# iamgiddyaboutgit/globalign

Hardware: AMD Instinct MI355X
Metric: DP cells/s (matrix fill) + alignment score bit-exact vs ref (higher is better)
Workload: dtype int32; 1 GPU; C3: 100k x 100k DNA (SplitMix64 seeds 1,2), match 2 / mismatch -3 / open -5 / ext -1, full traceback; m=100000, n=100000, traceback=True, parallelism=single GPU, cost=245432, oracle_cost=245432, cost_matches_oracle=True

## Files before the change

globalign_amd/csrc/ga_host.cpp:

```cpp
#include <hip/hip_runtime.h>
#include <unistd.h>

#include <algorithm>
#include <condition_variable>
#include <map>
#include <mutex>
#include <thread>
#include <chrono>
#include <cstdint>
#include <cstdio>
#include <cstring>
#include <string>
#include <vector>

#include "../../include/globalign_amd.h"
#include "ga_device.h"
#include "ga_lane.h"
#include "ga_check.h"
#include "ga_rng.h"

namespace {

thread_local std::string g_err;

// ... 333 lines not shown
#ifdef GA_EXPERIMENTS
constexpr bool kRcJumpDefault = false;
#endif
inline size_t rc_cache_bytes(bool jump, int TD, int CB) {
    return jump ? (size_t)ga::RC_CACHE_I * ga::RC_CACHE_S * 4 * TD * 6144 + 65536
                : (size_t)ga::RC_CACHE_I * ga::RC_CACHE_S * TD * 64 * 64 * CB + (size_t)64 * 64 * 4 * 4;
}
inline bool rc_jump_requested(const ga_ctx* c) {
#ifdef GA_EXPERIMENTS
    const char* e = c->xknob("GA_RC_JUMP");
    return e ? atoi(e) != 0 : kRcJumpDefault;
#else
    (void)c;
    return false;
#endif
}

int enqueue_fill(ga_ctx* c, int32_t flags, const Band& bd = Band()) {
    int every = bd.rc_every > 0 ? bd.rc_every : 64;
    if (!c->loaded) return fail(GA_E_STATE, "no problem loaded");
    const bool tb = (flags & (GA_FILL_TRACEBACK | GA_FILL_FULL)) != 0;
    const bool full = (flags & GA_FILL_FULL) != 0;
    const int64_t m = bd.band ? bd.mb : c->m, n = bd.band && bd.nc > 0 ? bd.nc : c->n;
    c->TC = (int)((m + ga::FROWS - 1) / ga::FROWS) * c->CB;
    int qrows = c->qrows;
    c->diag = false;
    c->lane = false;
    if (bd.rc) {
        if (tb || full || !lane_geometry(c, n, &qrows, false)) return fail(GA_E_STATE, "recompute fill needs the lane kernel");
        if (c->nwc == 8 && c->T == 8 && !lane_geometry(c, n, &qrows, false, 8, 4)) return fail(GA_E_STATE, "recompute fill geometry");
        constexpr int kRcLds = 256 * 256 * 2;
        if (!c->lane_T_req) {
            const char* nw = c->knob("GA_RC_NARROW");
            const bool td2 = nw && atoi(nw) && !c->slab && c->K <= 8 && (n + 127) / 128 <= 4 * (int64_t)c->num_cu;
            if (td2 && lane_geometry(c, n, &qrows, false, 2, 4)) {
            } else if (c->T > 4) {
                if (!lane_geometry(c, n, &qrows, false, 4, 4)) return fail(GA_E_STATE, "recompute fill geometry");
            } else if (c->T < 4) {
                (void)lane_geometry(c, n, &qrows, false, 4, 4);
            }
        }
        int64_t budget = (int64_t)96 << 30;
        if (const char* e = c->knob("GA_RC_BUDGET_MB")) budget = atoll(e) << 20;
        const int64_t dev_avail = dev_avail_bytes(c, (int64_t)c->stck.cap + (int64_t)c->colck.cap + (int64_t)c->rc_tb.cap);
        auto ck_bytes = [&](int e) {
            const int64_t nck = std::max<int64_t>((m - 1) / e, 1);
            return nck * c->nstripes * (c->T + 1) * 512;
        };
        auto other_bytes = [&]() {
            return (int64_t)c->nstripes * (m + 1) * 8 +
                   (int64_t)rc_cache_bytes(rc_jump_requested(c) && c->T <= 4, c->T, c->CB) +
                   ((int64_t)64 << 20);
        };
        auto fits = [&](int e) {
            return ck_bytes(e) <= std::min(budget, dev_avail - other_bytes()) &&
                   1024 + ga::rc_worker_bytes(c->T, c->CB, e) <= kRcLds;
        };
        for (;;) {
            if (bd.rc_every > 0) every = bd.rc_every;
            else
                for (every = 64; every < 4096 && !fits(every); every *= 2) {}
            if (1024 + ga::rc_worker_bytes(c->T, c->CB, every) <= kRcLds) break;
            if (c->T == 1) {
                if (1024 + ga::rc_worker_bytes(1, c->CB, 64) <= kRcLds)
                    return fail(GA_E_NOMEM, "recompute walk: the checkpoints do not fit the budget / free device memory");
                return fail(GA_E_RANGE, "recompute walk: a block's codes do not fit LDS");
            }
// ... 1998 lines not shown
```

globalign_amd/csrc/ga_lane.hip:

```cpp
#include <hip/hip_runtime.h>
#include <stdint.h>

#include <algorithm>
#include <cstdlib>
#include <type_traits>

#include "ga_device.h"
#include "ga_lane.h"
#include "ga_lane_asm.h"
#include "ga_sync.h"

#ifndef GA_LANE_LE
#define GA_LANE_LE 13
#endif

namespace ga {

__device__ unsigned lane_slab(const FillArgs& p) {
    unsigned* F = p.ticket;
    if (!p.xcd_map) return atomicAdd(F, 1u);
    const unsigned x = (unsigned)__builtin_amdgcn_s_getreg((15 << 11) | 20) & 7u;
    const unsigned rk = __hip_atomic_fetch_add(F + 4 + x, 1u, __ATOMIC_RELAXED, AGENT);
    const unsigned arr = __hip_atomic_fetch_add(F, 1u, __ATOMIC_ACQ_REL, AGENT);
    unsigned mode = 0;
// ... 349 lines not shown
    auto dbg_rows = [&](int r0) {
        if (r0 == 64) t_rows[4] = __builtin_amdgcn_s_memrealtime();
        if (r0 == 128) t_rows[5] = __builtin_amdgcn_s_memrealtime();
        if (r0 == 256) t_rows[0] = __builtin_amdgcn_s_memrealtime();
        if (r0 == 1024) t_rows[1] = __builtin_amdgcn_s_memrealtime();
        if (r0 == 4096) t_rows[2] = __builtin_amdgcn_s_memrealtime();
        if (r0 == 16384) t_rows[3] = __builtin_amdgcn_s_memrealtime();
    };
    auto wait_ge = [&](unsigned* ctr, unsigned add, unsigned& cached, int target, int kind) {
        unsigned spins = 0;
        cached = sgpr_u(cached);
        unsigned long long t0 = 0;
        if (DBG && (int)cached < target) t0 = __builtin_amdgcn_s_memtime();
        while ((int)cached < target && !aborted) {
            cached = lds_ldu(ctr) + add;
            if ((int)cached >= target) break;
            if (!spin_ok_lds(spins, p.spin_limit, abort_sh)) aborted = true;
        }
        if (DBG && t0) wcyc[kind] += __builtin_amdgcn_s_memtime() - t0;
        __atomic_signal_fence(__ATOMIC_SEQ_CST);
    };
    constexpr int NE = SUB / 2;
    constexpr int NQ = SUB / 4;
    int4 A[NE], B[NE];
    uint32_t qA[TD][NQ], qB[TD][NQ];
    wait_ge(prod_in, 0, avail, SUB, 0);
    unsigned long long w_first = 0, t_first = 0;
    if (DBG) {
        w_first = wcyc[0];
        t_first = __builtin_amdgcn_s_memrealtime();
    }
    const int4* const ezero = reinterpret_cast<const int4*>(smem + LK_ZERO_OFF);
    const unsigned ca_lds = lds_addr(prod_in);
    const unsigned pq_lds = lds_addr(pq);
    const unsigned scr_lds = lds_addr(smem + LK_SCR_OFF);
    unsigned q4[TD], ea_m, ea_b, wa_m, wa_b, wb_m, wb_b;
    {
#pragma unroll
        for (int k = 0; k < TD; k++) q4[k] = pq_lds + 4u * qb[k];
        const unsigned scr = scr_lds + 8u * (unsigned)lane, rout_l = lds_addr(rin + RING);
        const bool hi = lane >= 48;
        ea_m = lane == 0 ? ~0u : 0u;
        ea_b = lane == 0 ? 0u : lds_addr(ezero);
        wa_m = hi && (lane & 4) ? 8u * RMASK : 0u;
        wa_b = hi && (lane & 4) ? rout_l : scr;
        wb_m = hi && !(lane & 4) ? 8u * RMASK : 0u;
        wb_b = hi && !(lane & 4) ? rout_l : scr;
    }
    {
        const int4* src = lane == 0 ? reinterpret_cast<const int4*>(rin) : ezero;
#pragma unroll
        for (int k = 0; k < NE; k++) A[k] = src[k];
    }
    wait_ge(&cnt[LK_PRODQ], 0, qavail, SUB, 1);
    {
        const unsigned idx = (unsigned)(-lane) & qmask;
#pragma unroll
        for (int k = 0; k < TD; k++)
#pragma unroll
            for (int d = 0; d < NQ; d++) qA[k][d] = pq[qb[k] + idx + 4 * d];
    }
    unsigned pnext = *prod_in;
    int next_ck = CKP ? p.ckpt_rows : 0x7fffffff;
    constexpr int LE = (CB == 0 && !CKP && SUB == 16 && LATE) ? GA_LANE_LE : 0;

    auto sub_chunk = [&](int r0, int4 (&C)[NE], int4 (&Nx)[NE], uint32_t (&qc)[TD][NQ], uint32_t (&qx)[TD][NQ],
                         auto HALF, auto LEANT) {
        constexpr int HB = decltype(HALF)::value * SUB;
        constexpr bool LEAN = decltype(LEANT)::value;
        if (!LE) {
            avail = sgpr_u(max(avail, pnext));
            if ((int)avail < r0 + 2 * SUB) wait_ge(prod_in, 0, avail, r0 + 2 * SUB, 0);
        }
        if ((int)qavail < r0 + 2 * SUB) wait_ge(&cnt[LK_PRODQ], 0, qavail, r0 + 2 * SUB, 1);
        int eh[SUB], ex[SUB];
#pragma unroll
        for (int k = 0; k < NE; k++) {
            eh[2 * k] = C[k].x; ex[2 * k] = C[k].y; eh[2 * k + 1] = C[k].z; ex[2 * k + 1] = C[k].w;
        }
        auto qloads = [&]() {
            asm volatile("" ::: "memory");
            const unsigned idx = (unsigned)(r0 + SUB - lane) & qmask;
#pragma unroll
            for (int k = 0; k < TD; k++)
#pragma unroll
                for (int d = 0; d < NQ; d++) qx[k][d] = pq[qb[k] + idx + 4 * d];
            asm volatile("" ::: "memory");
        };
        auto eloads = [&]() {
            asm volatile("" ::: "memory");
            if (LE) {
                avail = sgpr_u(max(avail, pnext));
                if ((int)avail < r0 + 2 * SUB) wait_ge(prod_in, 0, avail, r0 + 2 * SUB, 0);
            }
            {
                const int4* src = lane == 0 ? reinterpret_cast<const int4*>(rin + ((r0 + SUB) & RMASK)) : ezero;
#pragma unroll
                for (int k = 0; k < NE; k++) Nx[k] = src[k];
            }
            pnext = __hip_atomic_load(prod_in, RLX, WGS);
            asm volatile("" ::: "memory");
        };
        const int row0 = r0 - lane + 1;
        const bool capl = lane == cn / TD;
        int cku = -1;
        int2* ckr = nullptr;
        auto ck_find = [&]() {
// ... 20 lines not shown
                            if (jl + k + 1 <= p.n) ckr[jl + k + 1] = make_int2(H[k], Y[k]);
                    }
                }
            };
            one(std::integral_constant<int, 0>{});
            qloads();
            if constexpr (LE > 0) {
                LkUnroll<1, LE>::run(one);
                eloads();
                LkUnroll<LE, SUB>::run(one);
            } else {
                eloads();
                LkUnroll<1, SUB>::run(one);
            }
        };
        const bool ckw = CKP && next_ck <= r0 + SUB;
        if (ckw) ck_find();
        if (CKP && next_ck < r0 + SUB - 62) next_ck += p.ckpt_rows;
        if constexpr (CKP) {
            if (r0 < 64 || (unsigned)(tm - r0) < (unsigned)SUB) {
                if (ckw) steps(std::true_type{}, std::true_type{});
                else steps(std::true_type{}, std::false_type{});
            } else if (ckw) {
                steps(std::false_type{}, std::true_type{});
            } else {
                steps(std::false_type{}, std::false_type{});
            }
        } else {
            const bool masked = !LEAN && ((r0 < 64 && !(p.lean0 && use_asm)) || (unsigned)(tm - r0) < (unsigned)SUB);
            if constexpr (ASMOK) {
                if (LEAN || (use_asm && !masked && !hand_direct)) {
                    const int rlo = r0 - 62;
                    outfree = sgpr_u(outfree);
                    if ((int)outfree < rlo + SUB - 1) wait_ge(cons_out, RING, outfree, rlo + SUB - 1, 2);
                    lk_v4i Ev[NE];
#pragma unroll
                    for (int k = 0; k < NE; k++) Ev[k] = lk_v4i{C[k].x, C[k].y, C[k].z, C[k].w};
                    unsigned ea, qi4, wt, wa, wb, qbv[TD];
                    const unsigned ea_s = lds_addr(rin) + 8u * ((unsigned)(r0 + SUB) & RMASK);
                    asm volatile("v_and_or_b32 %0, %1, %2, %3" : "=v"(ea) : "s"(ea_s), "v"(ea_m), "v"(ea_b));
                    asm volatile("v_sub_u32 %0, %1, %2" : "=v"(qi4) : "s"(4u * (unsigned)(r0 + SUB)), "v"(4u * (unsigned)lane));
                    qi4 &= 4u * qmask;
#pragma unroll
                    for (int k = 0; k < TD; k++) asm volatile("v_add_u32 %0, %1, %2" : "=v"(qbv[k]) : "v"(q4[k]), "v"(qi4));
                    asm volatile("v_add_u32 %0, %1, %2" : "=v"(wt) : "s"(8u * (unsigned)(rlo - 49)), "v"(8u * (unsigned)lane));
                    wa = (wt & wa_m) + wa_b;
                    wb = (wt & wb_m) + wb_b;
                    const unsigned wc = lane == 0 ? pc_lds : scr_lds + 8u * (unsigned)lane;
                    const bool hi = lane >= 48;
                    const lk_v2u cp = {(unsigned)(r0 + 2 * SUB), (unsigned)max(rlo + SUB - 1, 0)};
                    unsigned cv;
                    lk_v4i En[NE];
                    lk_v2u qn[TD][2];
                    int R[4];
                    LaneSub<TD, LE ? 12 : 0>::run(H, Y, Xl, HLp, Ev, qc, o, ca_lds, ea, qbv, wa, wb, wc, cp, cv, En, qn, R);
                    Hl = H[TD - 1];
                    if (DBG && rlo <= m / 2 && m / 2 < rlo + SUB) t_pub = __builtin_amdgcn_s_memrealtime();
                    const int need = min(r0 + 2 * SUB, m);
                    if ((int)sgpr_u(cv) < need) {
                        wait_ge(prod_in, 0, avail, need, 0);
                        asm volatile("" ::: "memory");
                        const int4* src = lane == 0 ? reinterpret_cast<const int4*>(rin + ((r0 + SUB) & RMASK)) : ezero;
#pragma unroll
                        for (int k = 0; k < NE; k++) Nx[k] = src[k];
#pragma unroll
                        for (int k = 0; k < NE; k++) asm volatile("" ::"v"(Nx[k].x), "v"(Nx[k].y), "v"(Nx[k].z), "v"(Nx[k].w));
                    } else {
#pragma unroll
                        for (int k = 0; k < NE; k++) Nx[k] = make_int4(En[k].x, En[k].y, En[k].z, En[k].w);
                    }
                    if (DBG && r0 + SUB < m / 2 && m / 2 <= r0 + 2 * SUB) t_avail = __builtin_amdgcn_s_memrealtime();
#pragma unroll
                    for (int k = 0; k < TD; k++) {
                        qx[k][0] = qn[k][0].x;
                        qx[k][1] = qn[k][0].y;
                        qx[k][2] = qn[k][1].x;
                        qx[k][3] = qn[k][1].y;
                    }
                    if (RC && LEAN) {
                        const lk_v2u vv = (lane & 4) ? lk_v2u{(unsigned)R[0], (unsigned)R[1]} : lk_v2u{(unsigned)R[2], (unsigned)R[3]};
                        const unsigned off = ck_cb + sgpr_u(8u * (unsigned)rlo);
                        asm volatile("buffer_store_dwordx2 %1, %0, %2, 0 offen" ::"v"(off), "v"(vv), "s"(ck_rsrc) : "memory");
                    } else if (RC && p.colck != nullptr) {
                        const int row = rlo + lane - 48;
                        const int2 v = (lane & 4) ? make_int2(R[0], R[1]) : make_int2(R[2], R[3]);
                        int2* const cdst = hi && row <= m ? colck_s + row : colck_x;
                        const lk_v2u vv = {(unsigned)v.x, (unsigned)v.y};
                        asm volatile("global_store_dwordx2 %0, %1, off" ::"v"(cdst), "v"(vv) : "memory");
                    }
                    return;
                }
            }
// ... 240 lines not shown
```

globalign_amd/csrc/ga_lane_asm.h:

```cpp
#pragma once
#include <hip/hip_runtime.h>
#include <stdint.h>

#include "ga_lane.h"

namespace ga {

template <int TD, int U0, int N>
struct LaneAsm;
typedef int lk_v4i __attribute__((ext_vector_type(4)));
template <int TD, int RS>
struct LaneSub;

template <>
struct LaneAsm<1, 0, 1> {
    __device__ __forceinline__ static void run(int (&H)[1], int (&Y)[1], int& Xl, int& HLp, const int* eh,
                                               const int* ex, const uint32_t (&q)[1], int o, int* oh, int* ox) {
        int X[1], HLn[1], hn[1], T, M[1];
        asm volatile(
        "v_add_u32_sdwa %[M0], sext(%[q0]), %[HLp] dst_sel:DWORD dst_unused:UNUSED_PAD src0_sel:BYTE_0 src1_sel:DWORD\n\t"
        "s_nop 0\n\t"
        "v_add_u32_dpp %[X0], %[Xl], %[ex0] wave_shr:1 row_mask:0xf bank_mask:0xf bound_ctrl:1\n\t"
        "v_add_u32_dpp %[HLn0], %[Hlast], %[eh0] wave_shr:1 row_mask:0xf bank_mask:0xf bound_ctrl:1\n\t"
        "v_min3_i32 %[hn0], %[M0], %[X0], %[Y0]\n\t"
// ... 2393 lines not shown
        "v_min_i32 %[Y4], %[Y4], %[T]\n\t"
        "v_min3_i32 %[H5], %[M5], %[X0], %[Y5]\n\t"
        "v_add_u32 %[T], %[o], %[H5]\n\t"
        "v_min_i32 %[X0], %[X0], %[T]\n\t"
        "v_min_i32 %[Y5], %[Y5], %[T]\n\t"
        "v_min3_i32 %[H6], %[M6], %[X0], %[Y6]\n\t"
        "v_add_u32 %[T], %[o], %[H6]\n\t"
        "v_min_i32 %[X0], %[X0], %[T]\n\t"
        "v_min_i32 %[Y6], %[Y6], %[T]\n\t"
        "v_min3_i32 %[hn0], %[M7], %[X0], %[Y7]\n\t"
        "v_add_u32 %[T], %[o], %[hn0]\n\t"
        "v_min_i32 %[X0], %[X0], %[T]\n\t"
        "v_min_i32 %[Y7], %[Y7], %[T]"
        : [X0] "=&v"(X[0]), [HLn0] "=&v"(HLn[0]), [hn0] "=&v"(hn[0]), [H0] "+v"(H[0]), [H1] "+v"(H[1]), [H2] "+v"(H[2]), [H3] "+v"(H[3]), [H4] "+v"(H[4]), [H5] "+v"(H[5]), [H6] "+v"(H[6]), [Y0] "+v"(Y[0]), [Y1] "+v"(Y[1]), [Y2] "+v"(Y[2]), [Y3] "+v"(Y[3]), [Y4] "+v"(Y[4]), [Y5] "+v"(Y[5]), [Y6] "+v"(Y[6]), [Y7] "+v"(Y[7]), [T] "=&v"(T), [M0] "=&v"(M[0]), [M1] "=&v"(M[1]), [M2] "=&v"(M[2]), [M3] "=&v"(M[3]), [M4] "=&v"(M[4]), [M5] "=&v"(M[5]), [M6] "=&v"(M[6]), [M7] "=&v"(M[7])
        : [Xl] "v"(Xl), [HLp] "v"(HLp), [Hlast] "v"(H[7]), [ex0] "v"(ex[0]), [eh0] "v"(eh[0]), [q0] "v"(q[0]), [q1] "v"(q[1]), [q2] "v"(q[2]), [q3] "v"(q[3]), [q4] "v"(q[4]), [q5] "v"(q[5]), [q6] "v"(q[6]), [q7] "v"(q[7]), [o] "s"(o));
        H[7] = hn[0];
        Xl = X[0];
        HLp = HLn[0];
#pragma unroll
        for (int s = 0; s < 1; s++) {
            oh[s] = hn[s];
            ox[s] = X[s];
        }
    }
};

template <>
struct LaneSub<1, 0> {
    __device__ __forceinline__ static void run(int (&H)[1], int (&Y)[1], int& Xl, int& HLp, const lk_v4i (&E)[8],
                                               const uint32_t (&q)[1][4], int o, unsigned ca, unsigned ea,
                                               const unsigned (&qb)[1], unsigned wa, unsigned wb, unsigned wc, lk_v2u cp,
                                               unsigned& cv, lk_v4i (&En)[8], lk_v2u (&qn)[1][2], int (&R)[4]) {
        int X[16], hn[16], HLn[2], T, M[1];
        asm volatile(
        "v_add_u32_sdwa %[M0], sext(%[q0_0]), %[HLp] dst_sel:DWORD dst_unused:UNUSED_PAD src0_sel:BYTE_0 src1_sel:DWORD\n\t"
        "s_nop 1\n\t"
        "v_add_u32_dpp %[X0], %[Xl], %[ex0] wave_shr:1 row_mask:0xf bank_mask:0xf bound_ctrl:1\n\t"
        "v_add_u32_dpp %[HLn0], %[Hlast], %[eh0] wave_shr:1 row_mask:0xf bank_mask:0xf bound_ctrl:1\n\t"
        "v_min3_i32 %[hn0], %[M0], %[X0], %[Y0]\n\t"
        "v_add_u32 %[T], %[o], %[hn0]\n\t"
        "v_min_i32 %[X0], %[X0], %[T]\n\t"
        "v_min_i32 %[Y0], %[Y0], %[T]\n\t"
        "ds_read_b32 %[cv], %[ca]\n\t"
        "ds_read_b128 %[E0], %[ea] offset:0\n\t"
        "ds_read_b128 %[E1], %[ea] offset:16\n\t"
        "ds_read_b128 %[E2], %[ea] offset:32\n\t"
        "ds_read_b128 %[E3], %[ea] offset:48\n\t"
        "ds_read_b128 %[E4], %[ea] offset:64\n\t"
        "ds_read_b128 %[E5], %[ea] offset:80\n\t"
        "ds_read_b128 %[E6], %[ea] offset:96\n\t"
        "ds_read_b128 %[E7], %[ea] offset:112\n\t"
        "v_add_u32_sdwa %[M0], sext(%[q0_0]), %[HLn0] dst_sel:DWORD dst_unused:UNUSED_PAD src0_sel:BYTE_1 src1_sel:DWORD\n\t"
        "v_add_u32_dpp %[X1], %[X0], %[ex1] wave_shr:1 row_mask:0xf bank_mask:0xf bound_ctrl:1\n\t"
        "v_add_u32_dpp %[HLn1], %[hn0], %[eh1] wave_shr:1 row_mask:0xf bank_mask:0xf bound_ctrl:1\n\t"
        "v_min3_i32 %[hn1], %[M0], %[X1], %[Y0]\n\t"
        "v_add_u32 %[T], %[o], %[hn1]\n\t"
        "v_min_i32 %[X1], %[X1], %[T]\n\t"
        "v_min_i32 %[Y0], %[Y0], %[T]\n\t"
        "ds_read2_b32 %[qa0], %[qb0] offset0:0 offset1:4\n\t"
        "ds_read2_b32 %[qc0], %[qb0] offset0:8 offset1:12\n\t"
        "v_add_u32_sdwa %[M0], sext(%[q0_0]), %[HLn1] dst_sel:DWORD dst_unused:UNUSED_PAD src0_sel:BYTE_2 src1_sel:DWORD\n\t"
        "v_add_u32_dpp %[X2], %[X1], %[ex2] wave_shr:1 row_mask:0xf bank_mask:0xf bound_ctrl:1\n\t"
        "v_add_u32_dpp %[HLn0], %[hn1], %[eh2] wave_shr:1 row_mask:0xf bank_mask:0xf bound_ctrl:1\n\t"
        "v_min3_i32 %[hn2], %[M0], %[X2], %[Y0]\n\t"
        "v_add_u32 %[T], %[o], %[hn2]\n\t"
        "v_min_i32 %[X2], %[X2], %[T]\n\t"
// ... 75 lines not shown
        "v_add_u32_dpp %[HLn1], %[hn10], %[eh11] wave_shr:1 row_mask:0xf bank_mask:0xf bound_ctrl:1\n\t"
        "v_min3_i32 %[hn11], %[M0], %[X11], %[Y0]\n\t"
        "v_add_u32 %[T], %[o], %[hn11]\n\t"
        "v_min_i32 %[X11], %[X11], %[T]\n\t"
        "v_min_i32 %[Y0], %[Y0], %[T]\n\t"
        "v_add_u32_sdwa %[M0], sext(%[q0_3]), %[HLn1] dst_sel:DWORD dst_unused:UNUSED_PAD src0_sel:BYTE_0 src1_sel:DWORD\n\t"
        "v_add_u32_dpp %[X12], %[X11], %[ex12] wave_shr:1 row_mask:0xf bank_mask:0xf bound_ctrl:1\n\t"
        "v_add_u32_dpp %[HLn0], %[hn11], %[eh12] wave_shr:1 row_mask:0xf bank_mask:0xf bound_ctrl:1\n\t"
        "v_min3_i32 %[hn12], %[M0], %[X12], %[Y0]\n\t"
        "v_add_u32 %[T], %[o], %[hn12]\n\t"
        "v_min_i32 %[X12], %[X12], %[T]\n\t"
        "v_min_i32 %[Y0], %[Y0], %[T]\n\t"
        "v_add_u32_sdwa %[M0], sext(%[q0_3]), %[HLn0] dst_sel:DWORD dst_unused:UNUSED_PAD src0_sel:BYTE_1 src1_sel:DWORD\n\t"
        "v_add_u32_dpp %[X13], %[X12], %[ex13] wave_shr:1 row_mask:0xf bank_mask:0xf bound_ctrl:1\n\t"
        "v_add_u32_dpp %[HLn1], %[hn12], %[eh13] wave_shr:1 row_mask:0xf bank_mask:0xf bound_ctrl:1\n\t"
        "v_min3_i32 %[hn13], %[M0], %[X13], %[Y0]\n\t"
        "v_add_u32 %[T], %[o], %[hn13]\n\t"
        "v_min_i32 %[X13], %[X13], %[T]\n\t"
        "v_min_i32 %[Y0], %[Y0], %[T]\n\t"
        "v_add_u32_sdwa %[M0], sext(%[q0_3]), %[HLn1] dst_sel:DWORD dst_unused:UNUSED_PAD src0_sel:BYTE_2 src1_sel:DWORD\n\t"
        "v_add_u32_dpp %[X14], %[X13], %[ex14] wave_shr:1 row_mask:0xf bank_mask:0xf bound_ctrl:1\n\t"
        "v_add_u32_dpp %[HLn0], %[hn13], %[eh14] wave_shr:1 row_mask:0xf bank_mask:0xf bound_ctrl:1\n\t"
        "v_min3_i32 %[hn14], %[M0], %[X14], %[Y0]\n\t"
        "v_add_u32 %[T], %[o], %[hn14]\n\t"
        "v_min_i32 %[X14], %[X14], %[T]\n\t"
        "v_min_i32 %[Y0], %[Y0], %[T]\n\t"
        "v_add_u32_sdwa %[M0], sext(%[q0_3]), %[HLn0] dst_sel:DWORD dst_unused:UNUSED_PAD src0_sel:BYTE_3 src1_sel:DWORD\n\t"
        "v_add_u32_dpp %[X15], %[X14], %[ex15] wave_shr:1 row_mask:0xf bank_mask:0xf bound_ctrl:1\n\t"
        "v_add_u32_dpp %[HLn1], %[hn14], %[eh15] wave_shr:1 row_mask:0xf bank_mask:0xf bound_ctrl:1\n\t"
        "v_min3_i32 %[hn15], %[M0], %[X15], %[Y0]\n\t"
        "v_add_u32 %[T], %[o], %[hn15]\n\t"
        "v_min_i32 %[X15], %[X15], %[T]\n\t"
        "v_min_i32 %[Y0], %[Y0], %[T]\n\t"
        "v_mov_b32_dpp %[Rhb], %[hn11] row_shl:4 row_mask:0x8 bank_mask:0x4\n\t"
        "v_mov_b32_dpp %[Rha], %[hn15] quad_perm:[0,1,2,3] row_mask:0x8 bank_mask:0x8\n\t"
        "v_mov_b32_dpp %[Rxb], %[X11] row_shl:4 row_mask:0x8 bank_mask:0x4\n\t"
        "v_mov_b32_dpp %[Rxa], %[X15] quad_perm:[0,1,2,3] row_mask:0x8 bank_mask:0x8\n\t"
        "v_mov_b32_dpp %[Rhb], %[hn10] row_shl:5 row_mask:0x8 bank_mask:0x4\n\t"
        "v_mov_b32_dpp %[Rha], %[hn14] row_shl:1 row_mask:0x8 bank_mask:0x8\n\t"
        "v_mov_b32_dpp %[Rxb], %[X10] row_shl:5 row_mask:0x8 bank_mask:0x4\n\t"
        "v_mov_b32_dpp %[Rxa], %[X14] row_shl:1 row_mask:0x8 bank_mask:0x8\n\t"
        "v_mov_b32_dpp %[Rhb], %[hn9] row_shl:6 row_mask:0x8 bank_mask:0x4\n\t"
        "v_mov_b32_dpp %[Rha], %[hn13] row_shl:2 row_mask:0x8 bank_mask:0x8\n\t"
        "v_mov_b32_dpp %[Rxb], %[X9] row_shl:6 row_mask:0x8 bank_mask:0x4\n\t"
        "v_mov_b32_dpp %[Rxa], %[X13] row_shl:2 row_mask:0x8 bank_mask:0x8\n\t"
        "v_mov_b32_dpp %[Rhb], %[hn8] row_shl:7 row_mask:0x8 bank_mask:0x4\n\t"
        "v_mov_b32_dpp %[Rha], %[hn12] row_shl:3 row_mask:0x8 bank_mask:0x8\n\t"
        "v_mov_b32_dpp %[Rxb], %[X8] row_shl:7 row_mask:0x8 bank_mask:0x4\n\t"
        "v_mov_b32_dpp %[Rxa], %[X12] row_shl:3 row_mask:0x8 bank_mask:0x8\n\t"
        "ds_write2_b32 %[wa], %[Rha], %[Rxa] offset1:1\n\t"
        "ds_write2_b32 %[wb], %[Rhb], %[Rxb] offset1:1\n\t"
        "ds_write_b64 %[wc], %[cp]\n\t"
        "s_waitcnt lgkmcnt(3)"
        : [X0] "=&v"(X[0]), [X1] "=&v"(X[1]), [X2] "=&v"(X[2]), [X3] "=&v"(X[3]), [X4] "=&v"(X[4]), [X5] "=&v"(X[5]), [X6] "=&v"(X[6]), [X7] "=&v"(X[7]), [X8] "=&v"(X[8]), [X9] "=&v"(X[9]), [X10] "=&v"(X[10]), [X11] "=&v"(X[11]), [X12] "=&v"(X[12]), [X13] "=&v"(X[13]), [X14] "=&v"(X[14]), [X15] "=&v"(X[15]), [hn0] "=&v"(hn[0]), [hn1] "=&v"(hn[1]), [hn2] "=&v"(hn[2]), [hn3] "=&v"(hn[3]), [hn4] "=&v"(hn[4]), [hn5] "=&v"(hn[5]), [hn6] "=&v"(hn[6]), [hn7] "=&v"(hn[7]), [hn8] "=&v"(hn[8]), [hn9] "=&v"(hn[9]), [hn10] "=&v"(hn[10]), [hn11] "=&v"(hn[11]), [hn12] "=&v"(hn[12]), [hn13] "=&v"(hn[13]), [hn14] "=&v"(hn[14]), [hn15] "=&v"(hn[15]), [HLn0] "=&v"(HLn[0]), [HLn1] "=&v"(HLn[1]), [Y0] "+v"(Y[0]), [T] "=&v"(T), [M0] "=&v"(M[0]), [Rha] "=&v"(R[0]), [Rxa] "=&v"(R[1]), [Rhb] "=&v"(R[2]), [Rxb] "=&v"(R[3]), [cv] "=&v"(cv), [E0] "=&v"(En[0]), [E1] "=&v"(En[1]), [E2] "=&v"(En[2]), [E3] "=&v"(En[3]), [E4] "=&v"(En[4]), [E5] "=&v"(En[5]), [E6] "=&v"(En[6]), [E7] "=&v"(En[7]), [qa0] "=&v"(qn[0][0]), [qc0] "=&v"(qn[0][1])
        : [Xl] "v"(Xl), [HLp] "v"(HLp), [Hlast] "v"(H[0]), [o] "s"(o), [ex0] "v"(E[0][1]), [ex1] "v"(E[0][3]), [ex2] "v"(E[1][1]), [ex3] "v"(E[1][3]), [ex4] "v"(E[2][1]), [ex5] "v"(E[2][3]), [ex6] "v"(E[3][1]), [ex7] "v"(E[3][3]), [ex8] "v"(E[4][1]), [ex9] "v"(E[4][3]), [ex10] "v"(E[5][1]), [ex11] "v"(E[5][3]), [ex12] "v"(E[6][1]), [ex13] "v"(E[6][3]), [ex14] "v"(E[7][1]), [ex15] "v"(E[7][3]), [eh0] "v"(E[0][0]), [eh1] "v"(E[0][2]), [eh2] "v"(E[1][0]), [eh3] "v"(E[1][2]), [eh4] "v"(E[2][0]), [eh5] "v"(E[2][2]), [eh6] "v"(E[3][0]), [eh7] "v"(E[3][2]), [eh8] "v"(E[4][0]), [eh9] "v"(E[4][2]), [eh10] "v"(E[5][0]), [eh11] "v"(E[5][2]), [eh12] "v"(E[6][0]), [eh13] "v"(E[6][2]), [eh14] "v"(E[7][0]), [eh15] "v"(E[7][2]), [q0_0] "v"(q[0][0]), [q0_1] "v"(q[0][1]), [q0_2] "v"(q[0][2]), [q0_3] "v"(q[0][3]), [ca] "v"(ca), [ea] "v"(ea), [wa] "v"(wa), [wb] "v"(wb), [wc] "v"(wc), [cp] "v"(cp), [qb0] "v"(qb[0])
        : "memory");
        H[0] = hn[15];
        Xl = X[15];
        HLp = HLn[1];
    }
};

template <>
struct LaneSub<1, 12> {
    __device__ __forceinline__ static void run(int (&H)[1], int (&Y)[1], int& Xl, int& HLp, const lk_v4i (&E)[8],
                                               const uint32_t (&q)[1][4], int o, unsigned ca, unsigned ea,
                                               const unsigned (&qb)[1], unsigned wa, unsigned wb, unsigned wc, lk_v2u cp,
                                               unsigned& cv, lk_v4i (&En)[8], lk_v2u (&qn)[1][2], int (&R)[4]) {
        int X[16], hn[16], HLn[2], T, M[1];
        asm volatile(
        "v_add_u32_sdwa %[M0], sext(%[q0_0]), %[HLp] dst_sel:DWORD dst_unused:UNUSED_PAD src0_sel:BYTE_0 src1_sel:DWORD\n\t"
        "s_nop 1\n\t"
        "v_add_u32_dpp %[X0], %[Xl], %[ex0] wave_shr:1 row_mask:0xf bank_mask:0xf bound_ctrl:1\n\t"
        "v_add_u32_dpp %[HLn0], %[Hlast], %[eh0] wave_shr:1 row_mask:0xf bank_mask:0xf bound_ctrl:1\n\t"
        "v_min3_i32 %[hn0], %[M0], %[X0], %[Y0]\n\t"
        "v_add_u32 %[T], %[o], %[hn0]\n\t"
        "v_min_i32 %[X0], %[X0], %[T]\n\t"
        "v_min_i32 %[Y0], %[Y0], %[T]\n\t"
        "v_add_u32_sdwa %[M0], sext(%[q0_0]), %[HLn0] dst_sel:DWORD dst_unused:UNUSED_PAD src0_sel:BYTE_1 src1_sel:DWORD\n\t"
        "v_add_u32_dpp %[X1], %[X0], %[ex1] wave_shr:1 row_mask:0xf bank_mask:0xf bound_ctrl:1\n\t"
        "v_add_u32_dpp %[HLn1], %[hn0], %[eh1] wave_shr:1 row_mask:0xf bank_mask:0xf bound_ctrl:1\n\t"
        "v_min3_i32 %[hn1], %[M0], %[X1], %[Y0]\n\t"
        "v_add_u32 %[T], %[o], %[hn1]\n\t"
        "v_min_i32 %[X1], %[X1], %[T]\n\t"
        "v_min_i32 %[Y0], %[Y0], %[T]\n\t"
        "ds_read2_b32 %[qa0], %[qb0] offset0:0 offset1:4\n\t"
        "ds_read2_b32 %[qc0], %[qb0] offset0:8 offset1:12\n\t"
        "v_add_u32_sdwa %[M0], sext(%[q0_0]), %[HLn1] dst_sel:DWORD dst_unused:UNUSED_PAD src0_sel:BYTE_2 src1_sel:DWORD\n\t"
        "v_add_u32_dpp %[X2], %[X1], %[ex2] wave_shr:1 row_mask:0xf bank_mask:0xf bound_ctrl:1\n\t"
        "v_add_u32_dpp %[HLn0], %[hn1], %[eh2] wave_shr:1 row_mask:0xf bank_mask:0xf bound_ctrl:1\n\t"
        "v_min3_i32 %[hn2], %[M0], %[X2], %[Y0]\n\t"
        "v_add_u32 %[T], %[o], %[hn2]\n\t"
        "v_min_i32 %[X2], %[X2], %[T]\n\t"
        "v_min_i32 %[Y0], %[Y0], %[T]\n\t"
        "v_add_u32_sdwa %[M0], sext(%[q0_0]), %[HLn0] dst_sel:DWORD dst_unused:UNUSED_PAD src0_sel:BYTE_3 src1_sel:DWORD\n\t"
        "v_add_u32_dpp %[X3], %[X2], %[ex3] wave_shr:1 row_mask:0xf bank_mask:0xf bound_ctrl:1\n\t"
        "v_add_u32_dpp %[HLn1], %[hn2], %[eh3] wave_shr:1 row_mask:0xf bank_mask:0xf bound_ctrl:1\n\t"
        "v_min3_i32 %[hn3], %[M0], %[X3], %[Y0]\n\t"
        "v_add_u32 %[T], %[o], %[hn3]\n\t"
        "v_min_i32 %[X3], %[X3], %[T]\n\t"
        "v_min_i32 %[Y0], %[Y0], %[T]\n\t"
        "v_add_u32_sdwa %[M0], sext(%[q0_1]), %[HLn1] dst_sel:DWORD dst_unused:UNUSED_PAD src0_sel:BYTE_0 src1_sel:DWORD\n\t"
// ... 75 lines not shown
        "v_add_u32 %[T], %[o], %[hn12]\n\t"
        "v_min_i32 %[X12], %[X12], %[T]\n\t"
        "v_min_i32 %[Y0], %[Y0], %[T]\n\t"
        "ds_read_b32 %[cv], %[ca]\n\t"
        "ds_read_b128 %[E0], %[ea] offset:0\n\t"
        "ds_read_b128 %[E1], %[ea] offset:16\n\t"
        "ds_read_b128 %[E2], %[ea] offset:32\n\t"
        "ds_read_b128 %[E3], %[ea] offset:48\n\t"
        "ds_read_b128 %[E4], %[ea] offset:64\n\t"
        "ds_read_b128 %[E5], %[ea] offset:80\n\t"
        "ds_read_b128 %[E6], %[ea] offset:96\n\t"
        "ds_read_b128 %[E7], %[ea] offset:112\n\t"
        "v_add_u32_sdwa %[M0], sext(%[q0_3]), %[HLn0] dst_sel:DWORD dst_unused:UNUSED_PAD src0_sel:BYTE_1 src1_sel:DWORD\n\t"
        "v_add_u32_dpp %[X13], %[X12], %[ex13] wave_shr:1 row_mask:0xf bank_mask:0xf bound_ctrl:1\n\t"
        "v_add_u32_dpp %[HLn1], %[hn12], %[eh13] wave_shr:1 row_mask:0xf bank_mask:0xf bound_ctrl:1\n\t"
        "v_min3_i32 %[hn13], %[M0], %[X13], %[Y0]\n\t"
        "v_add_u32 %[T], %[o], %[hn13]\n\t"
        "v_min_i32 %[X13], %[X13], %[T]\n\t"
        "v_min_i32 %[Y0], %[Y0], %[T]\n\t"
        "v_add_u32_sdwa %[M0], sext(%[q0_3]), %[HLn1] dst_sel:DWORD dst_unused:UNUSED_PAD src0_sel:BYTE_2 src1_sel:DWORD\n\t"
        "v_add_u32_dpp %[X14], %[X13], %[ex14] wave_shr:1 row_mask:0xf bank_mask:0xf bound_ctrl:1\n\t"
        "v_add_u32_dpp %[HLn0], %[hn13], %[eh14] wave_shr:1 row_mask:0xf bank_mask:0xf bound_ctrl:1\n\t"
        "v_min3_i32 %[hn14], %[M0], %[X14], %[Y0]\n\t"
        "v_add_u32 %[T], %[o], %[hn14]\n\t"
        "v_min_i32 %[X14], %[X14], %[T]\n\t"
        "v_min_i32 %[Y0], %[Y0], %[T]\n\t"
        "v_add_u32_sdwa %[M0], sext(%[q0_3]), %[HLn0] dst_sel:DWORD dst_unused:UNUSED_PAD src0_sel:BYTE_3 src1_sel:DWORD\n\t"
        "v_add_u32_dpp %[X15], %[X14], %[ex15] wave_shr:1 row_mask:0xf bank_mask:0xf bound_ctrl:1\n\t"
        "v_add_u32_dpp %[HLn1], %[hn14], %[eh15] wave_shr:1 row_mask:0xf bank_mask:0xf bound_ctrl:1\n\t"
        "v_min3_i32 %[hn15], %[M0], %[X15], %[Y0]\n\t"
        "v_add_u32 %[T], %[o], %[hn15]\n\t"
        "v_min_i32 %[X15], %[X15], %[T]\n\t"
        "v_min_i32 %[Y0], %[Y0], %[T]\n\t"
        "v_mov_b32_dpp %[Rhb], %[hn11] row_shl:4 row_mask:0x8 bank_mask:0x4\n\t"
        "v_mov_b32_dpp %[Rha], %[hn15] quad_perm:[0,1,2,3] row_mask:0x8 bank_mask:0x8\n\t"
        "v_mov_b32_dpp %[Rxb], %[X11] row_shl:4 row_mask:0x8 bank_mask:0x4\n\t"
        "v_mov_b32_dpp %[Rxa], %[X15] quad_perm:[0,1,2,3] row_mask:0x8 bank_mask:0x8\n\t"
        "v_mov_b32_dpp %[Rhb], %[hn10] row_shl:5 row_mask:0x8 bank_mask:0x4\n\t"
        "v_mov_b32_dpp %[Rha], %[hn14] row_shl:1 row_mask:0x8 bank_mask:0x8\n\t"
        "v_mov_b32_dpp %[Rxb], %[X10] row_shl:5 row_mask:0x8 bank_mask:0x4\n\t"
        "v_mov_b32_dpp %[Rxa], %[X14] row_shl:1 row_mask:0x8 bank_mask:0x8\n\t"
        "v_mov_b32_dpp %[Rhb], %[hn9] row_shl:6 row_mask:0x8 bank_mask:0x4\n\t"
        "v_mov_b32_dpp %[Rha], %[hn13] row_shl:2 row_mask:0x8 bank_mask:0x8\n\t"
        "v_mov_b32_dpp %[Rxb], %[X9] row_shl:6 row_mask:0x8 bank_mask:0x4\n\t"
        "v_mov_b32_dpp %[Rxa], %[X13] row_shl:2 row_mask:0x8 bank_mask:0x8\n\t"
        "v_mov_b32_dpp %[Rhb], %[hn8] row_shl:7 row_mask:0x8 bank_mask:0x4\n\t"
        "v_mov_b32_dpp %[Rha], %[hn12] row_shl:3 row_mask:0x8 bank_mask:0x8\n\t"
        "v_mov_b32_dpp %[Rxb], %[X8] row_shl:7 row_mask:0x8 bank_mask:0x4\n\t"
        "v_mov_b32_dpp %[Rxa], %[X12] row_shl:3 row_mask:0x8 bank_mask:0x8\n\t"
        "ds_write2_b32 %[wa], %[Rha], %[Rxa] offset1:1\n\t"
        "ds_write2_b32 %[wb], %[Rhb], %[Rxb] offset1:1\n\t"
        "ds_write_b64 %[wc], %[cp]\n\t"
        "s_waitcnt lgkmcnt(3)"
        : [X0] "=&v"(X[0]), [X1] "=&v"(X[1]), [X2] "=&v"(X[2]), [X3] "=&v"(X[3]), [X4] "=&v"(X[4]), [X5] "=&v"(X[5]), [X6] "=&v"(X[6]), [X7] "=&v"(X[7]), [X8] "=&v"(X[8]), [X9] "=&v"(X[9]), [X10] "=&v"(X[10]), [X11] "=&v"(X[11]), [X12] "=&v"(X[12]), [X13] "=&v"(X[13]), [X14] "=&v"(X[14]), [X15] "=&v"(X[15]), [hn0] "=&v"(hn[0]), [hn1] "=&v"(hn[1]), [hn2] "=&v"(hn[2]), [hn3] "=&v"(hn[3]), [hn4] "=&v"(hn[4]), [hn5] "=&v"(hn[5]), [hn6] "=&v"(hn[6]), [hn7] "=&v"(hn[7]), [hn8] "=&v"(hn[8]), [hn9] "=&v"(hn[9]), [hn10] "=&v"(hn[10]), [hn11] "=&v"(hn[11]), [hn12] "=&v"(hn[12]), [hn13] "=&v"(hn[13]), [hn14] "=&v"(hn[14]), [hn15] "=&v"(hn[15]), [HLn0] "=&v"(HLn[0]), [HLn1] "=&v"(HLn[1]), [Y0] "+v"(Y[0]), [T] "=&v"(T), [M0] "=&v"(M[0]), [Rha] "=&v"(R[0]), [Rxa] "=&v"(R[1]), [Rhb] "=&v"(R[2]), [Rxb] "=&v"(R[3]), [cv] "=&v"(cv), [E0] "=&v"(En[0]), [E1] "=&v"(En[1]), [E2] "=&v"(En[2]), [E3] "=&v"(En[3]), [E4] "=&v"(En[4]), [E5] "=&v"(En[5]), [E6] "=&v"(En[6]), [E7] "=&v"(En[7]), [qa0] "=&v"(qn[0][0]), [qc0] "=&v"(qn[0][1])
        : [Xl] "v"(Xl), [HLp] "v"(HLp), [Hlast] "v"(H[0]), [o] "s"(o), [ex0] "v"(E[0][1]), [ex1] "v"(E[0][3]), [ex2] "v"(E[1][1]), [ex3] "v"(E[1][3]), [ex4] "v"(E[2][1]), [ex5] "v"(E[2][3]), [ex6] "v"(E[3][1]), [ex7] "v"(E[3][3]), [ex8] "v"(E[4][1]), [ex9] "v"(E[4][3]), [ex10] "v"(E[5][1]), [ex11] "v"(E[5][3]), [ex12] "v"(E[6][1]), [ex13] "v"(E[6][3]), [ex14] "v"(E[7][1]), [ex15] "v"(E[7][3]), [eh0] "v"(E[0][0]), [eh1] "v"(E[0][2]), [eh2] "v"(E[1][0]), [eh3] "v"(E[1][2]), [eh4] "v"(E[2][0]), [eh5] "v"(E[2][2]), [eh6] "v"(E[3][0]), [eh7] "v"(E[3][2]), [eh8] "v"(E[4][0]), [eh9] "v"(E[4][2]), [eh10] "v"(E[5][0]), [eh11] "v"(E[5][2]), [eh12] "v"(E[6][0]), [eh13] "v"(E[6][2]), [eh14] "v"(E[7][0]), [eh15] "v"(E[7][2]), [q0_0] "v"(q[0][0]), [q0_1] "v"(q[0][1]), [q0_2] "v"(q[0][2]), [q0_3] "v"(q[0][3]), [ca] "v"(ca), [ea] "v"(ea), [wa] "v"(wa), [wb] "v"(wb), [wc] "v"(wc), [cp] "v"(cp), [qb0] "v"(qb[0])
        : "memory");
        H[0] = hn[15];
        Xl = X[15];
        HLp = HLn[1];
    }
};

template <>
struct LaneSub<2, 0> {
    __device__ __forceinline__ static void run(int (&H)[2], int (&Y)[2], int& Xl, int& HLp, const lk_v4i (&E)[8],
                                               const uint32_t (&q)[2][4], int o, unsigned ca, unsigned ea,
                                               const unsigned (&qb)[2], unsigned wa, unsigned wb, unsigned wc, lk_v2u cp,
                                               unsigned& cv, lk_v4i (&En)[8], lk_v2u (&qn)[2][2], int (&R)[4]) {
        int X[16], hn[16], HLn[2], T, M[2];
        asm volatile(
        "v_add_u32_sdwa %[M0], sext(%[q0_0]), %[HLp] dst_sel:DWORD dst_unused:UNUSED_PAD src0_sel:BYTE_0 src1_sel:DWORD\n\t"
        "v_add_u32_sdwa %[M1], sext(%[q1_0]), %[H0] dst_sel:DWORD dst_unused:UNUSED_PAD src0_sel:BYTE_0 src1_sel:DWORD\n\t"
        "v_add_u32_dpp %[X0], %[Xl], %[ex0] wave_shr:1 row_mask:0xf bank_mask:0xf bound_ctrl:1\n\t"
        "v_add_u32_dpp %[HLn0], %[Hlast], %[eh0] wave_shr:1 row_mask:0xf bank_mask:0xf bound_ctrl:1\n\t"
        "v_min3_i32 %[H0], %[M0], %[X0], %[Y0]\n\t"
        "v_add_u32 %[T], %[o], %[H0]\n\t"
        "v_min_i32 %[X0], %[X0], %[T]\n\t"
        "v_min_i32 %[Y0], %[Y0], %[T]\n\t"
        "v_min3_i32 %[hn0], %[M1], %[X0], %[Y1]\n\t"
        "v_add_u32 %[T], %[o], %[hn0]\n\t"
        "v_min_i32 %[X0], %[X0], %[T]\n\t"
        "v_min_i32 %[Y1], %[Y1], %[T]\n\t"
        "ds_read_b32 %[cv], %[ca]\n\t"
        "ds_read_b128 %[E0], %[ea] offset:0\n\t"
        "ds_read_b128 %[E1], %[ea] offset:16\n\t"
        "ds_read_b128 %[E2], %[ea] offset:32\n\t"
        "ds_read_b128 %[E3], %[ea] offset:48\n\t"
        "ds_read_b128 %[E4], %[ea] offset:64\n\t"
        "ds_read_b128 %[E5], %[ea] offset:80\n\t"
        "ds_read_b128 %[E6], %[ea] offset:96\n\t"
        "ds_read_b128 %[E7], %[ea] offset:112\n\t"
        "v_add_u32_sdwa %[M0], sext(%[q0_0]), %[HLn0] dst_sel:DWORD dst_unused:UNUSED_PAD src0_sel:BYTE_1 src1_sel:DWORD\n\t"
        "v_add_u32_sdwa %[M1], sext(%[q1_0]), %[H0] dst_sel:DWORD dst_unused:UNUSED_PAD src0_sel:BYTE_1 src1_sel:DWORD\n\t"
        "v_add_u32_dpp %[X1], %[X0], %[ex1] wave_shr:1 row_mask:0xf bank_mask:0xf bound_ctrl:1\n\t"
        "v_add_u32_dpp %[HLn1], %[hn0], %[eh1] wave_shr:1 row_mask:0xf bank_mask:0xf bound_ctrl:1\n\t"
        "v_min3_i32 %[H0], %[M0], %[X1], %[Y0]\n\t"
        "v_add_u32 %[T], %[o], %[H0]\n\t"
        "v_min_i32 %[X1], %[X1], %[T]\n\t"
        "v_min_i32 %[Y0], %[Y0], %[T]\n\t"
        "v_min3_i32 %[hn1], %[M1], %[X1], %[Y1]\n\t"
        "v_add_u32 %[T], %[o], %[hn1]\n\t"
        "v_min_i32 %[X1], %[X1], %[T]\n\t"
// ... 156 lines not shown
        "v_add_u32_dpp %[HLn1], %[hn12], %[eh13] wave_shr:1 row_mask:0xf bank_mask:0xf bound_ctrl:1\n\t"
        "v_min3_i32 %[H0], %[M0], %[X13], %[Y0]\n\t"
        "v_add_u32 %[T], %[o], %[H0]\n\t"
        "v_min_i32 %[X13], %[X13], %[T]\n\t"
        "v_min_i32 %[Y0], %[Y0], %[T]\n\t"
        "v_min3_i32 %[hn13], %[M1], %[X13], %[Y1]\n\t"
        "v_add_u32 %[T], %[o], %[hn13]\n\t"
        "v_min_i32 %[X13], %[X13], %[T]\n\t"
        "v_min_i32 %[Y1], %[Y1], %[T]\n\t"
        "v_add_u32_sdwa %[M0], sext(%[q0_3]), %[HLn1] dst_sel:DWORD dst_unused:UNUSED_PAD src0_sel:BYTE_2 src1_sel:DWORD\n\t"
        "v_add_u32_sdwa %[M1], sext(%[q1_3]), %[H0] dst_sel:DWORD dst_unused:UNUSED_PAD src0_sel:BYTE_2 src1_sel:DWORD\n\t"
        "v_add_u32_dpp %[X14], %[X13], %[ex14] wave_shr:1 row_mask:0xf bank_mask:0xf bound_ctrl:1\n\t"
        "v_add_u32_dpp %[HLn0], %[hn13], %[eh14] wave_shr:1 row_mask:0xf bank_mask:0xf bound_ctrl:1\n\t"
        "v_min3_i32 %[H0], %[M0], %[X14], %[Y0]\n\t"
        "v_add_u32 %[T], %[o], %[H0]\n\t"
        "v_min_i32 %[X14], %[X14], %[T]\n\t"
        "v_min_i32 %[Y0], %[Y0], %[T]\n\t"
        "v_min3_i32 %[hn14], %[M1], %[X14], %[Y1]\n\t"
        "v_add_u32 %[T], %[o], %[hn14]\n\t"
        "v_min_i32 %[X14], %[X14], %[T]\n\t"
        "v_min_i32 %[Y1], %[Y1], %[T]\n\t"
        "v_add_u32_sdwa %[M0], sext(%[q0_3]), %[HLn0] dst_sel:DWORD dst_unused:UNUSED_PAD src0_sel:BYTE_3 src1_sel:DWORD\n\t"
        "v_add_u32_sdwa %[M1], sext(%[q1_3]), %[H0] dst_sel:DWORD dst_unused:UNUSED_PAD src0_sel:BYTE_3 src1_sel:DWORD\n\t"
        "v_add_u32_dpp %[X15], %[X14], %[ex15] wave_shr:1 row_mask:0xf bank_mask:0xf bound_ctrl:1\n\t"
        "v_add_u32_dpp %[HLn1], %[hn14], %[eh15] wave_shr:1 row_mask:0xf bank_mask:0xf bound_ctrl:1\n\t"
        "v_min3_i32 %[H0], %[M0], %[X15], %[Y0]\n\t"
        "v_add_u32 %[T], %[o], %[H0]\n\t"
        "v_min_i32 %[X15], %[X15], %[T]\n\t"
        "v_min_i32 %[Y0], %[Y0], %[T]\n\t"
        "v_min3_i32 %[hn15], %[M1], %[X15], %[Y1]\n\t"
        "v_add_u32 %[T], %[o], %[hn15]\n\t"
        "v_min_i32 %[X15], %[X15], %[T]\n\t"
        "v_min_i32 %[Y1], %[Y1], %[T]\n\t"
        "v_mov_b32_dpp %[Rhb], %[hn11] row_shl:4 row_mask:0x8 bank_mask:0x4\n\t"
        "v_mov_b32_dpp %[Rha], %[hn15] quad_perm:[0,1,2,3] row_mask:0x8 bank_mask:0x8\n\t"
        "v_mov_b32_dpp %[Rxb], %[X11] row_shl:4 row_mask:0x8 bank_mask:0x4\n\t"
        "v_mov_b32_dpp %[Rxa], %[X15] quad_perm:[0,1,2,3] row_mask:0x8 bank_mask:0x8\n\t"
        "v_mov_b32_dpp %[Rhb], %[hn10] row_shl:5 row_mask:0x8 bank_mask:0x4\n\t"
        "v_mov_b32_dpp %[Rha], %[hn14] row_shl:1 row_mask:0x8 bank_mask:0x8\n\t"
        "v_mov_b32_dpp %[Rxb], %[X10] row_shl:5 row_mask:0x8 bank_mask:0x4\n\t"
        "v_mov_b32_dpp %[Rxa], %[X14] row_shl:1 row_mask:0x8 bank_mask:0x8\n\t"
        "v_mov_b32_dpp %[Rhb], %[hn9] row_shl:6 row_mask:0x8 bank_mask:0x4\n\t"
        "v_mov_b32_dpp %[Rha], %[hn13] row_shl:2 row_mask:0x8 bank_mask:0x8\n\t"
        "v_mov_b32_dpp %[Rxb], %[X9] row_shl:6 row_mask:0x8 bank_mask:0x4\n\t"
        "v_mov_b32_dpp %[Rxa], %[X13] row_shl:2 row_mask:0x8 bank_mask:0x8\n\t"
        "v_mov_b32_dpp %[Rhb], %[hn8] row_shl:7 row_mask:0x8 bank_mask:0x4\n\t"
        "v_mov_b32_dpp %[Rha], %[hn12] row_shl:3 row_mask:0x8 bank_mask:0x8\n\t"
        "v_mov_b32_dpp %[Rxb], %[X8] row_shl:7 row_mask:0x8 bank_mask:0x4\n\t"
        "v_mov_b32_dpp %[Rxa], %[X12] row_shl:3 row_mask:0x8 bank_mask:0x8\n\t"
        "ds_write2_b32 %[wa], %[Rha], %[Rxa] offset1:1\n\t"
        "ds_write2_b32 %[wb], %[Rhb], %[Rxb] offset1:1\n\t"
        "ds_write_b64 %[wc], %[cp]\n\t"
        "s_waitcnt lgkmcnt(3)"
        : [X0] "=&v"(X[0]), [X1] "=&v"(X[1]), [X2] "=&v"(X[2]), [X3] "=&v"(X[3]), [X4] "=&v"(X[4]), [X5] "=&v"(X[5]), [X6] "=&v"(X[6]), [X7] "=&v"(X[7]), [X8] "=&v"(X[8]), [X9] "=&v"(X[9]), [X10] "=&v"(X[10]), [X11] "=&v"(X[11]), [X12] "=&v"(X[12]), [X13] "=&v"(X[13]), [X14] "=&v"(X[14]), [X15] "=&v"(X[15]), [hn0] "=&v"(hn[0]), [hn1] "=&v"(hn[1]), [hn2] "=&v"(hn[2]), [hn3] "=&v"(hn[3]), [hn4] "=&v"(hn[4]), [hn5] "=&v"(hn[5]), [hn6] "=&v"(hn[6]), [hn7] "=&v"(hn[7]), [hn8] "=&v"(hn[8]), [hn9] "=&v"(hn[9]), [hn10] "=&v"(hn[10]), [hn11] "=&v"(hn[11]), [hn12] "=&v"(hn[12]), [hn13] "=&v"(hn[13]), [hn14] "=&v"(hn[14]), [hn15] "=&v"(hn[15]), [HLn0] "=&v"(HLn[0]), [HLn1] "=&v"(HLn[1]), [H0] "+v"(H[0]), [Y0] "+v"(Y[0]), [Y1] "+v"(Y[1]), [T] "=&v"(T), [M0] "=&v"(M[0]), [M1] "=&v"(M[1]), [Rha] "=&v"(R[0]), [Rxa] "=&v"(R[1]), [Rhb] "=&v"(R[2]), [Rxb] "=&v"(R[3]), [cv] "=&v"(cv), [E0] "=&v"(En[0]), [E1] "=&v"(En[1]), [E2] "=&v"(En[2]), [E3] "=&v"(En[3]), [E4] "=&v"(En[4]), [E5] "=&v"(En[5]), [E6] "=&v"(En[6]), [E7] "=&v"(En[7]), [qa0] "=&v"(qn[0][0]), [qa1] "=&v"(qn[1][0]), [qc0] "=&v"(qn[0][1]), [qc1] "=&v"(qn[1][1])
        : [Xl] "v"(Xl), [HLp] "v"(HLp), [Hlast] "v"(H[1]), [o] "s"(o), [ex0] "v"(E[0][1]), [ex1] "v"(E[0][3]), [ex2] "v"(E[1][1]), [ex3] "v"(E[1][3]), [ex4] "v"(E[2][1]), [ex5] "v"(E[2][3]), [ex6] "v"(E[3][1]), [ex7] "v"(E[3][3]), [ex8] "v"(E[4][1]), [ex9] "v"(E[4][3]), [ex10] "v"(E[5][1]), [ex11] "v"(E[5][3]), [ex12] "v"(E[6][1]), [ex13] "v"(E[6][3]), [ex14] "v"(E[7][1]), [ex15] "v"(E[7][3]), [eh0] "v"(E[0][0]), [eh1] "v"(E[0][2]), [eh2] "v"(E[1][0]), [eh3] "v"(E[1][2]), [eh4] "v"(E[2][0]), [eh5] "v"(E[2][2]), [eh6] "v"(E[3][0]), [eh7] "v"(E[3][2]), [eh8] "v"(E[4][0]), [eh9] "v"(E[4][2]), [eh10] "v"(E[5][0]), [eh11] "v"(E[5][2]), [eh12] "v"(E[6][0]), [eh13] "v"(E[6][2]), [eh14] "v"(E[7][0]), [eh15] "v"(E[7][2]), [q0_0] "v"(q[0][0]), [q0_1] "v"(q[0][1]), [q0_2] "v"(q[0][2]), [q0_3] "v"(q[0][3]), [q1_0] "v"(q[1][0]), [q1_1] "v"(q[1][1]), [q1_2] "v"(q[1][2]), [q1_3] "v"(q[1][3]), [ca] "v"(ca), [ea] "v"(ea), [wa] "v"(wa), [wb] "v"(wb), [wc] "v"(wc), [cp] "v"(cp), [qb0] "v"(qb[0]), [qb1] "v"(qb[1])
        : "memory");
        H[1] = hn[15];
        Xl = X[15];
        HLp = HLn[1];
    }
};

template <>
struct LaneSub<2, 12> {
    __device__ __forceinline__ static void run(int (&H)[2], int (&Y)[2], int& Xl, int& HLp, const lk_v4i (&E)[8],
                                               const uint32_t (&q)[2][4], int o, unsigned ca, unsigned ea,
                                               const unsigned (&qb)[2], unsigned wa, unsigned wb, unsigned wc, lk_v2u cp,
                                               unsigned& cv, lk_v4i (&En)[8], lk_v2u (&qn)[2][2], int (&R)[4]) {
        int X[16], hn[16], HLn[2], T, M[2];
        asm volatile(
        "v_add_u32_sdwa %[M0], sext(%[q0_0]), %[HLp] dst_sel:DWORD dst_unused:UNUSED_PAD src0_sel:BYTE_0 src1_sel:DWORD\n\t"
        "v_add_u32_sdwa %[M1], sext(%[q1_0]), %[H0] dst_sel:DWORD dst_unused:UNUSED_PAD src0_sel:BYTE_0 src1_sel:DWORD\n\t"
        "v_add_u32_dpp %[X0], %[Xl], %[ex0] wave_shr:1 row_mask:0xf bank_mask:0xf bound_ctrl:1\n\t"
        "v_add_u32_dpp %[HLn0], %[Hlast], %[eh0] wave_shr:1 row_mask:0xf bank_mask:0xf bound_ctrl:1\n\t"
        "v_min3_i32 %[H0], %[M0], %[X0], %[Y0]\n\t"
        "v_add_u32 %[T], %[o], %[H0]\n\t"
        "v_min_i32 %[X0], %[X0], %[T]\n\t"
        "v_min_i32 %[Y0], %[Y0], %[T]\n\t"
        "v_min3_i32 %[hn0], %[M1], %[X0], %[Y1]\n\t"
        "v_add_u32 %[T], %[o], %[hn0]\n\t"
        "v_min_i32 %[X0], %[X0], %[T]\n\t"
        "v_min_i32 %[Y1], %[Y1], %[T]\n\t"
        "v_add_u32_sdwa %[M0], sext(%[q0_0]), %[HLn0] dst_sel:DWORD dst_unused:UNUSED_PAD src0_sel:BYTE_1 src1_sel:DWORD\n\t"
        "v_add_u32_sdwa %[M1], sext(%[q1_0]), %[H0] dst_sel:DWORD dst_unused:UNUSED_PAD src0_sel:BYTE_1 src1_sel:DWORD\n\t"
        "v_add_u32_dpp %[X1], %[X0], %[ex1] wave_shr:1 row_mask:0xf bank_mask:0xf bound_ctrl:1\n\t"
        "v_add_u32_dpp %[HLn1], %[hn0], %[eh1] wave_shr:1 row_mask:0xf bank_mask:0xf bound_ctrl:1\n\t"
        "v_min3_i32 %[H0], %[M0], %[X1], %[Y0]\n\t"
        "v_add_u32 %[T], %[o], %[H0]\n\t"
        "v_min_i32 %[X1], %[X1], %[T]\n\t"
        "v_min_i32 %[Y0], %[Y0], %[T]\n\t"
        "v_min3_i32 %[hn1], %[M1], %[X1], %[Y1]\n\t"
        "v_add_u32 %[T], %[o], %[hn1]\n\t"
        "v_min_i32 %[X1], %[X1], %[T]\n\t"
        "v_min_i32 %[Y1], %[Y1], %[T]\n\t"
        "ds_read2_b32 %[qa0], %[qb0] offset0:0 offset1:4\n\t"
        "ds_read2_b32 %[qc0], %[qb0] offset0:8 offset1:12\n\t"
        "ds_read2_b32 %[qa1], %[qb1] offset0:0 offset1:4\n\t"
        "ds_read2_b32 %[qc1], %[qb1] offset0:8 offset1:12\n\t"
        "v_add_u32_sdwa %[M0], sext(%[q0_0]), %[HLn1] dst_sel:DWORD dst_unused:UNUSED_PAD src0_sel:BYTE_2 src1_sel:DWORD\n\t"
        "v_add_u32_sdwa %[M1], sext(%[q1_0]), %[H0] dst_sel:DWORD dst_unused:UNUSED_PAD src0_sel:BYTE_2 src1_sel:DWORD\n\t"
        "v_add_u32_dpp %[X2], %[X1], %[ex2] wave_shr:1 row_mask:0xf bank_mask:0xf bound_ctrl:1\n\t"
        "v_add_u32_dpp %[HLn0], %[hn1], %[eh2] wave_shr:1 row_mask:0xf bank_mask:0xf bound_ctrl:1\n\t"
// ... 156 lines not shown
        "v_add_u32_dpp %[HLn1], %[hn12], %[eh13] wave_shr:1 row_mask:0xf bank_mask:0xf bound_ctrl:1\n\t"
        "v_min3_i32 %[H0], %[M0], %[X13], %[Y0]\n\t"
        "v_add_u32 %[T], %[o], %[H0]\n\t"
        "v_min_i32 %[X13], %[X13], %[T]\n\t"
        "v_min_i32 %[Y0], %[Y0], %[T]\n\t"
        "v_min3_i32 %[hn13], %[M1], %[X13], %[Y1]\n\t"
        "v_add_u32 %[T], %[o], %[hn13]\n\t"
        "v_min_i32 %[X13], %[X13], %[T]\n\t"
        "v_min_i32 %[Y1], %[Y1], %[T]\n\t"
        "v_add_u32_sdwa %[M0], sext(%[q0_3]), %[HLn1] dst_sel:DWORD dst_unused:UNUSED_PAD src0_sel:BYTE_2 src1_sel:DWORD\n\t"
        "v_add_u32_sdwa %[M1], sext(%[q1_3]), %[H0] dst_sel:DWORD dst_unused:UNUSED_PAD src0_sel:BYTE_2 src1_sel:DWORD\n\t"
        "v_add_u32_dpp %[X14], %[X13], %[ex14] wave_shr:1 row_mask:0xf bank_mask:0xf bound_ctrl:1\n\t"
        "v_add_u32_dpp %[HLn0], %[hn13], %[eh14] wave_shr:1 row_mask:0xf bank_mask:0xf bound_ctrl:1\n\t"
        "v_min3_i32 %[H0], %[M0], %[X14], %[Y0]\n\t"
        "v_add_u32 %[T], %[o], %[H0]\n\t"
        "v_min_i32 %[X14], %[X14], %[T]\n\t"
        "v_min_i32 %[Y0], %[Y0], %[T]\n\t"
        "v_min3_i32 %[hn14], %[M1], %[X14], %[Y1]\n\t"
        "v_add_u32 %[T], %[o], %[hn14]\n\t"
        "v_min_i32 %[X14], %[X14], %[T]\n\t"
        "v_min_i32 %[Y1], %[Y1], %[T]\n\t"
        "v_add_u32_sdwa %[M0], sext(%[q0_3]), %[HLn0] dst_sel:DWORD dst_unused:UNUSED_PAD src0_sel:BYTE_3 src1_sel:DWORD\n\t"
        "v_add_u32_sdwa %[M1], sext(%[q1_3]), %[H0] dst_sel:DWORD dst_unused:UNUSED_PAD src0_sel:BYTE_3 src1_sel:DWORD\n\t"
        "v_add_u32_dpp %[X15], %[X14], %[ex15] wave_shr:1 row_mask:0xf bank_mask:0xf bound_ctrl:1\n\t"
        "v_add_u32_dpp %[HLn1], %[hn14], %[eh15] wave_shr:1 row_mask:0xf bank_mask:0xf bound_ctrl:1\n\t"
        "v_min3_i32 %[H0], %[M0], %[X15], %[Y0]\n\t"
        "v_add_u32 %[T], %[o], %[H0]\n\t"
        "v_min_i32 %[X15], %[X15], %[T]\n\t"
        "v_min_i32 %[Y0], %[Y0], %[T]\n\t"
        "v_min3_i32 %[hn15], %[M1], %[X15], %[Y1]\n\t"
        "v_add_u32 %[T], %[o], %[hn15]\n\t"
        "v_min_i32 %[X15], %[X15], %[T]\n\t"
        "v_min_i32 %[Y1], %[Y1], %[T]\n\t"
        "v_mov_b32_dpp %[Rhb], %[hn11] row_shl:4 row_mask:0x8 bank_mask:0x4\n\t"
        "v_mov_b32_dpp %[Rha], %[hn15] quad_perm:[0,1,2,3] row_mask:0x8 bank_mask:0x8\n\t"
        "v_mov_b32_dpp %[Rxb], %[X11] row_shl:4 row_mask:0x8 bank_mask:0x4\n\t"
        "v_mov_b32_dpp %[Rxa], %[X15] quad_perm:[0,1,2,3] row_mask:0x8 bank_mask:0x8\n\t"
        "v_mov_b32_dpp %[Rhb], %[hn10] row_shl:5 row_mask:0x8 bank_mask:0x4\n\t"
        "v_mov_b32_dpp %[Rha], %[hn14] row_shl:1 row_mask:0x8 bank_mask:0x8\n\t"
        "v_mov_b32_dpp %[Rxb], %[X10] row_shl:5 row_mask:0x8 bank_mask:0x4\n\t"
        "v_mov_b32_dpp %[Rxa], %[X14] row_shl:1 row_mask:0x8 bank_mask:0x8\n\t"
        "v_mov_b32_dpp %[Rhb], %[hn9] row_shl:6 row_mask:0x8 bank_mask:0x4\n\t"
        "v_mov_b32_dpp %[Rha], %[hn13] row_shl:2 row_mask:0x8 bank_mask:0x8\n\t"
        "v_mov_b32_dpp %[Rxb], %[X9] row_shl:6 row_mask:0x8 bank_mask:0x4\n\t"
        "v_mov_b32_dpp %[Rxa], %[X13] row_shl:2 row_mask:0x8 bank_mask:0x8\n\t"
        "v_mov_b32_dpp %[Rhb], %[hn8] row_shl:7 row_mask:0x8 bank_mask:0x4\n\t"
        "v_mov_b32_dpp %[Rha], %[hn12] row_shl:3 row_mask:0x8 bank_mask:0x8\n\t"
        "v_mov_b32_dpp %[Rxb], %[X8] row_shl:7 row_mask:0x8 bank_mask:0x4\n\t"
        "v_mov_b32_dpp %[Rxa], %[X12] row_shl:3 row_mask:0x8 bank_mask:0x8\n\t"
        "ds_write2_b32 %[wa], %[Rha], %[Rxa] offset1:1\n\t"
        "ds_write2_b32 %[wb], %[Rhb], %[Rxb] offset1:1\n\t"
        "ds_write_b64 %[wc], %[cp]\n\t"
        "s_waitcnt lgkmcnt(3)"
        : [X0] "=&v"(X[0]), [X1] "=&v"(X[1]), [X2] "=&v"(X[2]), [X3] "=&v"(X[3]), [X4] "=&v"(X[4]), [X5] "=&v"(X[5]), [X6] "=&v"(X[6]), [X7] "=&v"(X[7]), [X8] "=&v"(X[8]), [X9] "=&v"(X[9]), [X10] "=&v"(X[10]), [X11] "=&v"(X[11]), [X12] "=&v"(X[12]), [X13] "=&v"(X[13]), [X14] "=&v"(X[14]), [X15] "=&v"(X[15]), [hn0] "=&v"(hn[0]), [hn1] "=&v"(hn[1]), [hn2] "=&v"(hn[2]), [hn3] "=&v"(hn[3]), [hn4] "=&v"(hn[4]), [hn5] "=&v"(hn[5]), [hn6] "=&v"(hn[6]), [hn7] "=&v"(hn[7]), [hn8] "=&v"(hn[8]), [hn9] "=&v"(hn[9]), [hn10] "=&v"(hn[10]), [hn11] "=&v"(hn[11]), [hn12] "=&v"(hn[12]), [hn13] "=&v"(hn[13]), [hn14] "=&v"(hn[14]), [hn15] "=&v"(hn[15]), [HLn0] "=&v"(HLn[0]), [HLn1] "=&v"(HLn[1]), [H0] "+v"(H[0]), [Y0] "+v"(Y[0]), [Y1] "+v"(Y[1]), [T] "=&v"(T), [M0] "=&v"(M[0]), [M1] "=&v"(M[1]), [Rha] "=&v"(R[0]), [Rxa] "=&v"(R[1]), [Rhb] "=&v"(R[2]), [Rxb] "=&v"(R[3]), [cv] "=&v"(cv), [E0] "=&v"(En[0]), [E1] "=&v"(En[1]), [E2] "=&v"(En[2]), [E3] "=&v"(En[3]), [E4] "=&v"(En[4]), [E5] "=&v"(En[5]), [E6] "=&v"(En[6]), [E7] "=&v"(En[7]), [qa0] "=&v"(qn[0][0]), [qa1] "=&v"(qn[1][0]), [qc0] "=&v"(qn[0][1]), [qc1] "=&v"(qn[1][1])
        : [Xl] "v"(Xl), [HLp] "v"(HLp), [Hlast] "v"(H[1]), [o] "s"(o), [ex0] "v"(E[0][1]), [ex1] "v"(E[0][3]), [ex2] "v"(E[1][1]), [ex3] "v"(E[1][3]), [ex4] "v"(E[2][1]), [ex5] "v"(E[2][3]), [ex6] "v"(E[3][1]), [ex7] "v"(E[3][3]), [ex8] "v"(E[4][1]), [ex9] "v"(E[4][3]), [ex10] "v"(E[5][1]), [ex11] "v"(E[5][3]), [ex12] "v"(E[6][1]), [ex13] "v"(E[6][3]), [ex14] "v"(E[7][1]), [ex15] "v"(E[7][3]), [eh0] "v"(E[0][0]), [eh1] "v"(E[0][2]), [eh2] "v"(E[1][0]), [eh3] "v"(E[1][2]), [eh4] "v"(E[2][0]), [eh5] "v"(E[2][2]), [eh6] "v"(E[3][0]), [eh7] "v"(E[3][2]), [eh8] "v"(E[4][0]), [eh9] "v"(E[4][2]), [eh10] "v"(E[5][0]), [eh11] "v"(E[5][2]), [eh12] "v"(E[6][0]), [eh13] "v"(E[6][2]), [eh14] "v"(E[7][0]), [eh15] "v"(E[7][2]), [q0_0] "v"(q[0][0]), [q0_1] "v"(q[0][1]), [q0_2] "v"(q[0][2]), [q0_3] "v"(q[0][3]), [q1_0] "v"(q[1][0]), [q1_1] "v"(q[1][1]), [q1_2] "v"(q[1][2]), [q1_3] "v"(q[1][3]), [ca] "v"(ca), [ea] "v"(ea), [wa] "v"(wa), [wb] "v"(wb), [wc] "v"(wc), [cp] "v"(cp), [qb0] "v"(qb[0]), [qb1] "v"(qb[1])
        : "memory");
        H[1] = hn[15];
        Xl = X[15];
        HLp = HLn[1];
    }
};

template <>
struct LaneSub<4, 0> {
    __device__ __forceinline__ static void run(int (&H)[4], int (&Y)[4], int& Xl, int& HLp, const lk_v4i (&E)[8],
                                               const uint32_t (&q)[4][4], int o, unsigned ca, unsigned ea,
                                               const unsigned (&qb)[4], unsigned wa, unsigned wb, unsigned wc, lk_v2u cp,
                                               unsigned& cv, lk_v4i (&En)[8], lk_v2u (&qn)[4][2], int (&R)[4]) {
        int X[16], hn[16], HLn[2], T, M[4];
        asm volatile(
        "v_add_u32_sdwa %[M0], sext(%[q0_0]), %[HLp] dst_sel:DWORD dst_unused:UNUSED_PAD src0_sel:BYTE_0 src1_sel:DWORD\n\t"
        "v_add_u32_sdwa %[M1], sext(%[q1_0]), %[H0] dst_sel:DWORD dst_unused:UNUSED_PAD src0_sel:BYTE_0 src1_sel:DWORD\n\t"
        "v_add_u32_sdwa %[M2], sext(%[q2_0]), %[H1] dst_sel:DWORD dst_unused:UNUSED_PAD src0_sel:BYTE_0 src1_sel:DWORD\n\t"
        "v_add_u32_sdwa %[M3], sext(%[q3_0]), %[H2] dst_sel:DWORD dst_unused:UNUSED_PAD src0_sel:BYTE_0 src1_sel:DWORD\n\t"
        "v_add_u32_dpp %[X0], %[Xl], %[ex0] wave_shr:1 row_mask:0xf bank_mask:0xf bound_ctrl:1\n\t"
        "v_add_u32_dpp %[HLn0], %[Hlast], %[eh0] wave_shr:1 row_mask:0xf bank_mask:0xf bound_ctrl:1\n\t"
        "v_min3_i32 %[H0], %[M0], %[X0], %[Y0]\n\t"
        "v_add_u32 %[T], %[o], %[H0]\n\t"
        "v_min_i32 %[X0], %[X0], %[T]\n\t"
        "v_min_i32 %[Y0], %[Y0], %[T]\n\t"
        "v_min3_i32 %[H1], %[M1], %[X0], %[Y1]\n\t"
        "v_add_u32 %[T], %[o], %[H1]\n\t"
        "v_min_i32 %[X0], %[X0], %[T]\n\t"
        "v_min_i32 %[Y1], %[Y1], %[T]\n\t"
        "v_min3_i32 %[H2], %[M2], %[X0], %[Y2]\n\t"
        "v_add_u32 %[T], %[o], %[H2]\n\t"
        "v_min_i32 %[X0], %[X0], %[T]\n\t"
        "v_min_i32 %[Y2], %[Y2], %[T]\n\t"
        "v_min3_i32 %[hn0], %[M3], %[X0], %[Y3]\n\t"
        "v_add_u32 %[T], %[o], %[hn0]\n\t"
        "v_min_i32 %[X0], %[X0], %[T]\n\t"
        "v_min_i32 %[Y3], %[Y3], %[T]\n\t"
        "ds_read_b32 %[cv], %[ca]\n\t"
        "ds_read_b128 %[E0], %[ea] offset:0\n\t"
        "ds_read_b128 %[E1], %[ea] offset:16\n\t"
        "ds_read_b128 %[E2], %[ea] offset:32\n\t"
        "ds_read_b128 %[E3], %[ea] offset:48\n\t"
        "ds_read_b128 %[E4], %[ea] offset:64\n\t"
        "ds_read_b128 %[E5], %[ea] offset:80\n\t"
        "ds_read_b128 %[E6], %[ea] offset:96\n\t"
        "ds_read_b128 %[E7], %[ea] offset:112\n\t"
        "v_add_u32_sdwa %[M0], sext(%[q0_0]), %[HLn0] dst_sel:DWORD dst_unused:UNUSED_PAD src0_sel:BYTE_1 src1_sel:DWORD\n\t"
// ... 320 lines not shown
        "v_add_u32 %[T], %[o], %[H1]\n\t"
        "v_min_i32 %[X14], %[X14], %[T]\n\t"
        "v_min_i32 %[Y1], %[Y1], %[T]\n\t"
        "v_min3_i32 %[H2], %[M2], %[X14], %[Y2]\n\t"
        "v_add_u32 %[T], %[o], %[H2]\n\t"
        "v_min_i32 %[X14], %[X14], %[T]\n\t"
        "v_min_i32 %[Y2], %[Y2], %[T]\n\t"
        "v_min3_i32 %[hn14], %[M3], %[X14], %[Y3]\n\t"
        "v_add_u32 %[T], %[o], %[hn14]\n\t"
        "v_min_i32 %[X14], %[X14], %[T]\n\t"
        "v_min_i32 %[Y3], %[Y3], %[T]\n\t"
        "v_add_u32_sdwa %[M0], sext(%[q0_3]), %[HLn0] dst_sel:DWORD dst_unused:UNUSED_PAD src0_sel:BYTE_3 src1_sel:DWORD\n\t"
        "v_add_u32_sdwa %[M1], sext(%[q1_3]), %[H0] dst_sel:DWORD dst_unused:UNUSED_PAD src0_sel:BYTE_3 src1_sel:DWORD\n\t"
        "v_add_u32_sdwa %[M2], sext(%[q2_3]), %[H1] dst_sel:DWORD dst_unused:UNUSED_PAD src0_sel:BYTE_3 src1_sel:DWORD\n\t"
        "v_add_u32_sdwa %[M3], sext(%[q3_3]), %[H2] dst_sel:DWORD dst_unused:UNUSED_PAD src0_sel:BYTE_3 src1_sel:DWORD\n\t"
        "v_add_u32_dpp %[X15], %[X14], %[ex15] wave_shr:1 row_mask:0xf bank_mask:0xf bound_ctrl:1\n\t"
        "v_add_u32_dpp %[HLn1], %[hn14], %[eh15] wave_shr:1 row_mask:0xf bank_mask:0xf bound_ctrl:1\n\t"
        "v_min3_i32 %[H0], %[M0], %[X15], %[Y0]\n\t"
        "v_add_u32 %[T], %[o], %[H0]\n\t"
        "v_min_i32 %[X15], %[X15], %[T]\n\t"
        "v_min_i32 %[Y0], %[Y0], %[T]\n\t"
        "v_min3_i32 %[H1], %[M1], %[X15], %[Y1]\n\t"
        "v_add_u32 %[T], %[o], %[H1]\n\t"
        "v_min_i32 %[X15], %[X15], %[T]\n\t"
        "v_min_i32 %[Y1], %[Y1], %[T]\n\t"
        "v_min3_i32 %[H2], %[M2], %[X15], %[Y2]\n\t"
        "v_add_u32 %[T], %[o], %[H2]\n\t"
        "v_min_i32 %[X15], %[X15], %[T]\n\t"
        "v_min_i32 %[Y2], %[Y2], %[T]\n\t"
        "v_min3_i32 %[hn15], %[M3], %[X15], %[Y3]\n\t"
        "v_add_u32 %[T], %[o], %[hn15]\n\t"
        "v_min_i32 %[X15], %[X15], %[T]\n\t"
        "v_min_i32 %[Y3], %[Y3], %[T]\n\t"
        "v_mov_b32_dpp %[Rhb], %[hn11] row_shl:4 row_mask:0x8 bank_mask:0x4\n\t"
        "v_mov_b32_dpp %[Rha], %[hn15] quad_perm:[0,1,2,3] row_mask:0x8 bank_mask:0x8\n\t"
        "v_mov_b32_dpp %[Rxb], %[X11] row_shl:4 row_mask:0x8 bank_mask:0x4\n\t"
        "v_mov_b32_dpp %[Rxa], %[X15] quad_perm:[0,1,2,3] row_mask:0x8 bank_mask:0x8\n\t"
        "v_mov_b32_dpp %[Rhb], %[hn10] row_shl:5 row_mask:0x8 bank_mask:0x4\n\t"
        "v_mov_b32_dpp %[Rha], %[hn14] row_shl:1 row_mask:0x8 bank_mask:0x8\n\t"
        "v_mov_b32_dpp %[Rxb], %[X10] row_shl:5 row_mask:0x8 bank_mask:0x4\n\t"
        "v_mov_b32_dpp %[Rxa], %[X14] row_shl:1 row_mask:0x8 bank_mask:0x8\n\t"
        "v_mov_b32_dpp %[Rhb], %[hn9] row_shl:6 row_mask:0x8 bank_mask:0x4\n\t"
        "v_mov_b32_dpp %[Rha], %[hn13] row_shl:2 row_mask:0x8 bank_mask:0x8\n\t"
        "v_mov_b32_dpp %[Rxb], %[X9] row_shl:6 row_mask:0x8 bank_mask:0x4\n\t"
        "v_mov_b32_dpp %[Rxa], %[X13] row_shl:2 row_mask:0x8 bank_mask:0x8\n\t"
        "v_mov_b32_dpp %[Rhb], %[hn8] row_shl:7 row_mask:0x8 bank_mask:0x4\n\t"
        "v_mov_b32_dpp %[Rha], %[hn12] row_shl:3 row_mask:0x8 bank_mask:0x8\n\t"
        "v_mov_b32_dpp %[Rxb], %[X8] row_shl:7 row_mask:0x8 bank_mask:0x4\n\t"
        "v_mov_b32_dpp %[Rxa], %[X12] row_shl:3 row_mask:0x8 bank_mask:0x8\n\t"
        "ds_write2_b32 %[wa], %[Rha], %[Rxa] offset1:1\n\t"
        "ds_write2_b32 %[wb], %[Rhb], %[Rxb] offset1:1\n\t"
        "ds_write_b64 %[wc], %[cp]\n\t"
        "s_waitcnt lgkmcnt(3)"
        : [X0] "=&v"(X[0]), [X1] "=&v"(X[1]), [X2] "=&v"(X[2]), [X3] "=&v"(X[3]), [X4] "=&v"(X[4]), [X5] "=&v"(X[5]), [X6] "=&v"(X[6]), [X7] "=&v"(X[7]), [X8] "=&v"(X[8]), [X9] "=&v"(X[9]), [X10] "=&v"(X[10]), [X11] "=&v"(X[11]), [X12] "=&v"(X[12]), [X13] "=&v"(X[13]), [X14] "=&v"(X[14]), [X15] "=&v"(X[15]), [hn0] "=&v"(hn[0]), [hn1] "=&v"(hn[1]), [hn2] "=&v"(hn[2]), [hn3] "=&v"(hn[3]), [hn4] "=&v"(hn[4]), [hn5] "=&v"(hn[5]), [hn6] "=&v"(hn[6]), [hn7] "=&v"(hn[7]), [hn8] "=&v"(hn[8]), [hn9] "=&v"(hn[9]), [hn10] "=&v"(hn[10]), [hn11] "=&v"(hn[11]), [hn12] "=&v"(hn[12]), [hn13] "=&v"(hn[13]), [hn14] "=&v"(hn[14]), [hn15] "=&v"(hn[15]), [HLn0] "=&v"(HLn[0]), [HLn1] "=&v"(HLn[1]), [H0] "+v"(H[0]), [H1] "+v"(H[1]), [H2] "+v"(H[2]), [Y0] "+v"(Y[0]), [Y1] "+v"(Y[1]), [Y2] "+v"(Y[2]), [Y3] "+v"(Y[3]), [T] "=&v"(T), [M0] "=&v"(M[0]), [M1] "=&v"(M[1]), [M2] "=&v"(M[2]), [M3] "=&v"(M[3]), [Rha] "=&v"(R[0]), [Rxa] "=&v"(R[1]), [Rhb] "=&v"(R[2]), [Rxb] "=&v"(R[3]), [cv] "=&v"(cv), [E0] "=&v"(En[0]), [E1] "=&v"(En[1]), [E2] "=&v"(En[2]), [E3] "=&v"(En[3]), [E4] "=&v"(En[4]), [E5] "=&v"(En[5]), [E6] "=&v"(En[6]), [E7] "=&v"(En[7]), [qa0] "=&v"(qn[0][0]), [qa1] "=&v"(qn[1][0]), [qa2] "=&v"(qn[2][0]), [qa3] "=&v"(qn[3][0]), [qc0] "=&v"(qn[0][1]), [qc1] "=&v"(qn[1][1]), [qc2] "=&v"(qn[2][1]), [qc3] "=&v"(qn[3][1])
        : [Xl] "v"(Xl), [HLp] "v"(HLp), [Hlast] "v"(H[3]), [o] "s"(o), [ex0] "v"(E[0][1]), [ex1] "v"(E[0][3]), [ex2] "v"(E[1][1]), [ex3] "v"(E[1][3]), [ex4] "v"(E[2][1]), [ex5] "v"(E[2][3]), [ex6] "v"(E[3][1]), [ex7] "v"(E[3][3]), [ex8] "v"(E[4][1]), [ex9] "v"(E[4][3]), [ex10] "v"(E[5][1]), [ex11] "v"(E[5][3]), [ex12] "v"(E[6][1]), [ex13] "v"(E[6][3]), [ex14] "v"(E[7][1]), [ex15] "v"(E[7][3]), [eh0] "v"(E[0][0]), [eh1] "v"(E[0][2]), [eh2] "v"(E[1][0]), [eh3] "v"(E[1][2]), [eh4] "v"(E[2][0]), [eh5] "v"(E[2][2]), [eh6] "v"(E[3][0]), [eh7] "v"(E[3][2]), [eh8] "v"(E[4][0]), [eh9] "v"(E[4][2]), [eh10] "v"(E[5][0]), [eh11] "v"(E[5][2]), [eh12] "v"(E[6][0]), [eh13] "v"(E[6][2]), [eh14] "v"(E[7][0]), [eh15] "v"(E[7][2]), [q0_0] "v"(q[0][0]), [q0_1] "v"(q[0][1]), [q0_2] "v"(q[0][2]), [q0_3] "v"(q[0][3]), [q1_0] "v"(q[1][0]), [q1_1] "v"(q[1][1]), [q1_2] "v"(q[1][2]), [q1_3] "v"(q[1][3]), [q2_0] "v"(q[2][0]), [q2_1] "v"(q[2][1]), [q2_2] "v"(q[2][2]), [q2_3] "v"(q[2][3]), [q3_0] "v"(q[3][0]), [q3_1] "v"(q[3][1]), [q3_2] "v"(q[3][2]), [q3_3] "v"(q[3][3]), [ca] "v"(ca), [ea] "v"(ea), [wa] "v"(wa), [wb] "v"(wb), [wc] "v"(wc), [cp] "v"(cp), [qb0] "v"(qb[0]), [qb1] "v"(qb[1]), [qb2] "v"(qb[2]), [qb3] "v"(qb[3])
        : "memory");
        H[3] = hn[15];
        Xl = X[15];
        HLp = HLn[1];
    }
};

template <>
struct LaneSub<4, 12> {
    __device__ __forceinline__ static void run(int (&H)[4], int (&Y)[4], int& Xl, int& HLp, const lk_v4i (&E)[8],
                                               const uint32_t (&q)[4][4], int o, unsigned ca, unsigned ea,
                                               const unsigned (&qb)[4], unsigned wa, unsigned wb, unsigned wc, lk_v2u cp,
                                               unsigned& cv, lk_v4i (&En)[8], lk_v2u (&qn)[4][2], int (&R)[4]) {
        int X[16], hn[16], HLn[2], T, M[4];
        asm volatile(
        "v_add_u32_sdwa %[M0], sext(%[q0_0]), %[HLp] dst_sel:DWORD dst_unused:UNUSED_PAD src0_sel:BYTE_0 src1_sel:DWORD\n\t"
        "v_add_u32_sdwa %[M1], sext(%[q1_0]), %[H0] dst_sel:DWORD dst_unused:UNUSED_PAD src0_sel:BYTE_0 src1_sel:DWORD\n\t"
        "v_add_u32_sdwa %[M2], sext(%[q2_0]), %[H1] dst_sel:DWORD dst_unused:UNUSED_PAD src0_sel:BYTE_0 src1_sel:DWORD\n\t"
        "v_add_u32_sdwa %[M3], sext(%[q3_0]), %[H2] dst_sel:DWORD dst_unused:UNUSED_PAD src0_sel:BYTE_0 src1_sel:DWORD\n\t"
        "v_add_u32_dpp %[X0], %[Xl], %[ex0] wave_shr:1 row_mask:0xf bank_mask:0xf bound_ctrl:1\n\t"
        "v_add_u32_dpp %[HLn0], %[Hlast], %[eh0] wave_shr:1 row_mask:0xf bank_mask:0xf bound_ctrl:1\n\t"
        "v_min3_i32 %[H0], %[M0], %[X0], %[Y0]\n\t"
        "v_add_u32 %[T], %[o], %[H0]\n\t"
        "v_min_i32 %[X0], %[X0], %[T]\n\t"
        "v_min_i32 %[Y0], %[Y0], %[T]\n\t"
        "v_min3_i32 %[H1], %[M1], %[X0], %[Y1]\n\t"
        "v_add_u32 %[T], %[o], %[H1]\n\t"
        "v_min_i32 %[X0], %[X0], %[T]\n\t"
        "v_min_i32 %[Y1], %[Y1], %[T]\n\t"
        "v_min3_i32 %[H2], %[M2], %[X0], %[Y2]\n\t"
        "v_add_u32 %[T], %[o], %[H2]\n\t"
        "v_min_i32 %[X0], %[X0], %[T]\n\t"
        "v_min_i32 %[Y2], %[Y2], %[T]\n\t"
        "v_min3_i32 %[hn0], %[M3], %[X0], %[Y3]\n\t"
        "v_add_u32 %[T], %[o], %[hn0]\n\t"
        "v_min_i32 %[X0], %[X0], %[T]\n\t"
        "v_min_i32 %[Y3], %[Y3], %[T]\n\t"
        "v_add_u32_sdwa %[M0], sext(%[q0_0]), %[HLn0] dst_sel:DWORD dst_unused:UNUSED_PAD src0_sel:BYTE_1 src1_sel:DWORD\n\t"
        "v_add_u32_sdwa %[M1], sext(%[q1_0]), %[H0] dst_sel:DWORD dst_unused:UNUSED_PAD src0_sel:BYTE_1 src1_sel:DWORD\n\t"
        "v_add_u32_sdwa %[M2], sext(%[q2_0]), %[H1] dst_sel:DWORD dst_unused:UNUSED_PAD src0_sel:BYTE_1 src1_sel:DWORD\n\t"
        "v_add_u32_sdwa %[M3], sext(%[q3_0]), %[H2] dst_sel:DWORD dst_unused:UNUSED_PAD src0_sel:BYTE_1 src1_sel:DWORD\n\t"
        "v_add_u32_dpp %[X1], %[X0], %[ex1] wave_shr:1 row_mask:0xf bank_mask:0xf bound_ctrl:1\n\t"
        "v_add_u32_dpp %[HLn1], %[hn0], %[eh1] wave_shr:1 row_mask:0xf bank_mask:0xf bound_ctrl:1\n\t"
        "v_min3_i32 %[H0], %[M0], %[X1], %[Y0]\n\t"
        "v_add_u32 %[T], %[o], %[H0]\n\t"
        "v_min_i32 %[X1], %[X1], %[T]\n\t"
        "v_min_i32 %[Y0], %[Y0], %[T]\n\t"
// ... 320 lines not shown
        "v_add_u32 %[T], %[o], %[H1]\n\t"
        "v_min_i32 %[X14], %[X14], %[T]\n\t"
        "v_min_i32 %[Y1], %[Y1], %[T]\n\t"
        "v_min3_i32 %[H2], %[M2], %[X14], %[Y2]\n\t"
        "v_add_u32 %[T], %[o], %[H2]\n\t"
        "v_min_i32 %[X14], %[X14], %[T]\n\t"
        "v_min_i32 %[Y2], %[Y2], %[T]\n\t"
        "v_min3_i32 %[hn14], %[M3], %[X14], %[Y3]\n\t"
        "v_add_u32 %[T], %[o], %[hn14]\n\t"
        "v_min_i32 %[X14], %[X14], %[T]\n\t"
        "v_min_i32 %[Y3], %[Y3], %[T]\n\t"
        "v_add_u32_sdwa %[M0], sext(%[q0_3]), %[HLn0] dst_sel:DWORD dst_unused:UNUSED_PAD src0_sel:BYTE_3 src1_sel:DWORD\n\t"
        "v_add_u32_sdwa %[M1], sext(%[q1_3]), %[H0] dst_sel:DWORD dst_unused:UNUSED_PAD src0_sel:BYTE_3 src1_sel:DWORD\n\t"
        "v_add_u32_sdwa %[M2], sext(%[q2_3]), %[H1] dst_sel:DWORD dst_unused:UNUSED_PAD src0_sel:BYTE_3 src1_sel:DWORD\n\t"
        "v_add_u32_sdwa %[M3], sext(%[q3_3]), %[H2] dst_sel:DWORD dst_unused:UNUSED_PAD src0_sel:BYTE_3 src1_sel:DWORD\n\t"
        "v_add_u32_dpp %[X15], %[X14], %[ex15] wave_shr:1 row_mask:0xf bank_mask:0xf bound_ctrl:1\n\t"
        "v_add_u32_dpp %[HLn1], %[hn14], %[eh15] wave_shr:1 row_mask:0xf bank_mask:0xf bound_ctrl:1\n\t"
        "v_min3_i32 %[H0], %[M0], %[X15], %[Y0]\n\t"
        "v_add_u32 %[T], %[o], %[H0]\n\t"
        "v_min_i32 %[X15], %[X15], %[T]\n\t"
        "v_min_i32 %[Y0], %[Y0], %[T]\n\t"
        "v_min3_i32 %[H1], %[M1], %[X15], %[Y1]\n\t"
        "v_add_u32 %[T], %[o], %[H1]\n\t"
        "v_min_i32 %[X15], %[X15], %[T]\n\t"
        "v_min_i32 %[Y1], %[Y1], %[T]\n\t"
        "v_min3_i32 %[H2], %[M2], %[X15], %[Y2]\n\t"
        "v_add_u32 %[T], %[o], %[H2]\n\t"
        "v_min_i32 %[X15], %[X15], %[T]\n\t"
        "v_min_i32 %[Y2], %[Y2], %[T]\n\t"
        "v_min3_i32 %[hn15], %[M3], %[X15], %[Y3]\n\t"
        "v_add_u32 %[T], %[o], %[hn15]\n\t"
        "v_min_i32 %[X15], %[X15], %[T]\n\t"
        "v_min_i32 %[Y3], %[Y3], %[T]\n\t"
        "v_mov_b32_dpp %[Rhb], %[hn11] row_shl:4 row_mask:0x8 bank_mask:0x4\n\t"
        "v_mov_b32_dpp %[Rha], %[hn15] quad_perm:[0,1,2,3] row_mask:0x8 bank_mask:0x8\n\t"
        "v_mov_b32_dpp %[Rxb], %[X11] row_shl:4 row_mask:0x8 bank_mask:0x4\n\t"
        "v_mov_b32_dpp %[Rxa], %[X15] quad_perm:[0,1,2,3] row_mask:0x8 bank_mask:0x8\n\t"
        "v_mov_b32_dpp %[Rhb], %[hn10] row_shl:5 row_mask:0x8 bank_mask:0x4\n\t"
        "v_mov_b32_dpp %[Rha], %[hn14] row_shl:1 row_mask:0x8 bank_mask:0x8\n\t"
        "v_mov_b32_dpp %[Rxb], %[X10] row_shl:5 row_mask:0x8 bank_mask:0x4\n\t"
        "v_mov_b32_dpp %[Rxa], %[X14] row_shl:1 row_mask:0x8 bank_mask:0x8\n\t"
        "v_mov_b32_dpp %[Rhb], %[hn9] row_shl:6 row_mask:0x8 bank_mask:0x4\n\t"
        "v_mov_b32_dpp %[Rha], %[hn13] row_shl:2 row_mask:0x8 bank_mask:0x8\n\t"
        "v_mov_b32_dpp %[Rxb], %[X9] row_shl:6 row_mask:0x8 bank_mask:0x4\n\t"
        "v_mov_b32_dpp %[Rxa], %[X13] row_shl:2 row_mask:0x8 bank_mask:0x8\n\t"
        "v_mov_b32_dpp %[Rhb], %[hn8] row_shl:7 row_mask:0x8 bank_mask:0x4\n\t"
        "v_mov_b32_dpp %[Rha], %[hn12] row_shl:3 row_mask:0x8 bank_mask:0x8\n\t"
        "v_mov_b32_dpp %[Rxb], %[X8] row_shl:7 row_mask:0x8 bank_mask:0x4\n\t"
        "v_mov_b32_dpp %[Rxa], %[X12] row_shl:3 row_mask:0x8 bank_mask:0x8\n\t"
        "ds_write2_b32 %[wa], %[Rha], %[Rxa] offset1:1\n\t"
        "ds_write2_b32 %[wb], %[Rhb], %[Rxb] offset1:1\n\t"
        "ds_write_b64 %[wc], %[cp]\n\t"
        "s_waitcnt lgkmcnt(3)"
        : [X0] "=&v"(X[0]), [X1] "=&v"(X[1]), [X2] "=&v"(X[2]), [X3] "=&v"(X[3]), [X4] "=&v"(X[4]), [X5] "=&v"(X[5]), [X6] "=&v"(X[6]), [X7] "=&v"(X[7]), [X8] "=&v"(X[8]), [X9] "=&v"(X[9]), [X10] "=&v"(X[10]), [X11] "=&v"(X[11]), [X12] "=&v"(X[12]), [X13] "=&v"(X[13]), [X14] "=&v"(X[14]), [X15] "=&v"(X[15]), [hn0] "=&v"(hn[0]), [hn1] "=&v"(hn[1]), [hn2] "=&v"(hn[2]), [hn3] "=&v"(hn[3]), [hn4] "=&v"(hn[4]), [hn5] "=&v"(hn[5]), [hn6] "=&v"(hn[6]), [hn7] "=&v"(hn[7]), [hn8] "=&v"(hn[8]), [hn9] "=&v"(hn[9]), [hn10] "=&v"(hn[10]), [hn11] "=&v"(hn[11]), [hn12] "=&v"(hn[12]), [hn13] "=&v"(hn[13]), [hn14] "=&v"(hn[14]), [hn15] "=&v"(hn[15]), [HLn0] "=&v"(HLn[0]), [HLn1] "=&v"(HLn[1]), [H0] "+v"(H[0]), [H1] "+v"(H[1]), [H2] "+v"(H[2]), [Y0] "+v"(Y[0]), [Y1] "+v"(Y[1]), [Y2] "+v"(Y[2]), [Y3] "+v"(Y[3]), [T] "=&v"(T), [M0] "=&v"(M[0]), [M1] "=&v"(M[1]), [M2] "=&v"(M[2]), [M3] "=&v"(M[3]), [Rha] "=&v"(R[0]), [Rxa] "=&v"(R[1]), [Rhb] "=&v"(R[2]), [Rxb] "=&v"(R[3]), [cv] "=&v"(cv), [E0] "=&v"(En[0]), [E1] "=&v"(En[1]), [E2] "=&v"(En[2]), [E3] "=&v"(En[3]), [E4] "=&v"(En[4]), [E5] "=&v"(En[5]), [E6] "=&v"(En[6]), [E7] "=&v"(En[7]), [qa0] "=&v"(qn[0][0]), [qa1] "=&v"(qn[1][0]), [qa2] "=&v"(qn[2][0]), [qa3] "=&v"(qn[3][0]), [qc0] "=&v"(qn[0][1]), [qc1] "=&v"(qn[1][1]), [qc2] "=&v"(qn[2][1]), [qc3] "=&v"(qn[3][1])
        : [Xl] "v"(Xl), [HLp] "v"(HLp), [Hlast] "v"(H[3]), [o] "s"(o), [ex0] "v"(E[0][1]), [ex1] "v"(E[0][3]), [ex2] "v"(E[1][1]), [ex3] "v"(E[1][3]), [ex4] "v"(E[2][1]), [ex5] "v"(E[2][3]), [ex6] "v"(E[3][1]), [ex7] "v"(E[3][3]), [ex8] "v"(E[4][1]), [ex9] "v"(E[4][3]), [ex10] "v"(E[5][1]), [ex11] "v"(E[5][3]), [ex12] "v"(E[6][1]), [ex13] "v"(E[6][3]), [ex14] "v"(E[7][1]), [ex15] "v"(E[7][3]), [eh0] "v"(E[0][0]), [eh1] "v"(E[0][2]), [eh2] "v"(E[1][0]), [eh3] "v"(E[1][2]), [eh4] "v"(E[2][0]), [eh5] "v"(E[2][2]), [eh6] "v"(E[3][0]), [eh7] "v"(E[3][2]), [eh8] "v"(E[4][0]), [eh9] "v"(E[4][2]), [eh10] "v"(E[5][0]), [eh11] "v"(E[5][2]), [eh12] "v"(E[6][0]), [eh13] "v"(E[6][2]), [eh14] "v"(E[7][0]), [eh15] "v"(E[7][2]), [q0_0] "v"(q[0][0]), [q0_1] "v"(q[0][1]), [q0_2] "v"(q[0][2]), [q0_3] "v"(q[0][3]), [q1_0] "v"(q[1][0]), [q1_1] "v"(q[1][1]), [q1_2] "v"(q[1][2]), [q1_3] "v"(q[1][3]), [q2_0] "v"(q[2][0]), [q2_1] "v"(q[2][1]), [q2_2] "v"(q[2][2]), [q2_3] "v"(q[2][3]), [q3_0] "v"(q[3][0]), [q3_1] "v"(q[3][1]), [q3_2] "v"(q[3][2]), [q3_3] "v"(q[3][3]), [ca] "v"(ca), [ea] "v"(ea), [wa] "v"(wa), [wb] "v"(wb), [wc] "v"(wc), [cp] "v"(cp), [qb0] "v"(qb[0]), [qb1] "v"(qb[1]), [qb2] "v"(qb[2]), [qb3] "v"(qb[3])
        : "memory");
        H[3] = hn[15];
        Xl = X[15];
        HLp = HLn[1];
    }
};

template <>
struct LaneSub<8, 0> {
    __device__ __forceinline__ static void run(int (&H)[8], int (&Y)[8], int& Xl, int& HLp, const lk_v4i (&E)[8],
                                               const uint32_t (&q)[8][4], int o, unsigned ca, unsigned ea,
                                               const unsigned (&qb)[8], unsigned wa, unsigned wb, unsigned wc, lk_v2u cp,
                                               unsigned& cv, lk_v4i (&En)[8], lk_v2u (&qn)[8][2], int (&R)[4]) {
        int X[16], hn[16], HLn[2], T, M[8];
        asm volatile(
        "v_add_u32_sdwa %[M0], sext(%[q0_0]), %[HLp] dst_sel:DWORD dst_unused:UNUSED_PAD src0_sel:BYTE_0 src1_sel:DWORD\n\t"
        "v_add_u32_sdwa %[M1], sext(%[q1_0]), %[H0] dst_sel:DWORD dst_unused:UNUSED_PAD src0_sel:BYTE_0 src1_sel:DWORD\n\t"
        "v_add_u32_sdwa %[M2], sext(%[q2_0]), %[H1] dst_sel:DWORD dst_unused:UNUSED_PAD src0_sel:BYTE_0 src1_sel:DWORD\n\t"
        "v_add_u32_sdwa %[M3], sext(%[q3_0]), %[H2] dst_sel:DWORD dst_unused:UNUSED_PAD src0_sel:BYTE_0 src1_sel:DWORD\n\t"
        "v_add_u32_sdwa %[M4], sext(%[q4_0]), %[H3] dst_sel:DWORD dst_unused:UNUSED_PAD src0_sel:BYTE_0 src1_sel:DWORD\n\t"
        "v_add_u32_sdwa %[M5], sext(%[q5_0]), %[H4] dst_sel:DWORD dst_unused:UNUSED_PAD src0_sel:BYTE_0 src1_sel:DWORD\n\t"
        "v_add_u32_sdwa %[M6], sext(%[q6_0]), %[H5] dst_sel:DWORD dst_unused:UNUSED_PAD src0_sel:BYTE_0 src1_sel:DWORD\n\t"
        "v_add_u32_sdwa %[M7], sext(%[q7_0]), %[H6] dst_sel:DWORD dst_unused:UNUSED_PAD src0_sel:BYTE_0 src1_sel:DWORD\n\t"
        "v_add_u32_dpp %[X0], %[Xl], %[ex0] wave_shr:1 row_mask:0xf bank_mask:0xf bound_ctrl:1\n\t"
        "v_add_u32_dpp %[HLn0], %[Hlast], %[eh0] wave_shr:1 row_mask:0xf bank_mask:0xf bound_ctrl:1\n\t"
        "v_min3_i32 %[H0], %[M0], %[X0], %[Y0]\n\t"
        "v_add_u32 %[T], %[o], %[H0]\n\t"
        "v_min_i32 %[X0], %[X0], %[T]\n\t"
        "v_min_i32 %[Y0], %[Y0], %[T]\n\t"
        "v_min3_i32 %[H1], %[M1], %[X0], %[Y1]\n\t"
        "v_add_u32 %[T], %[o], %[H1]\n\t"
        "v_min_i32 %[X0], %[X0], %[T]\n\t"
        "v_min_i32 %[Y1], %[Y1], %[T]\n\t"
        "v_min3_i32 %[H2], %[M2], %[X0], %[Y2]\n\t"
        "v_add_u32 %[T], %[o], %[H2]\n\t"
        "v_min_i32 %[X0], %[X0], %[T]\n\t"
        "v_min_i32 %[Y2], %[Y2], %[T]\n\t"
        "v_min3_i32 %[H3], %[M3], %[X0], %[Y3]\n\t"
        "v_add_u32 %[T], %[o], %[H3]\n\t"
        "v_min_i32 %[X0], %[X0], %[T]\n\t"
        "v_min_i32 %[Y3], %[Y3], %[T]\n\t"
        "v_min3_i32 %[H4], %[M4], %[X0], %[Y4]\n\t"
        "v_add_u32 %[T], %[o], %[H4]\n\t"
        "v_min_i32 %[X0], %[X0], %[T]\n\t"
        "v_min_i32 %[Y4], %[Y4], %[T]\n\t"
        "v_min3_i32 %[H5], %[M5], %[X0], %[Y5]\n\t"
        "v_add_u32 %[T], %[o], %[H5]\n\t"
// ... 648 lines not shown
        "v_add_u32_dpp %[HLn1], %[hn14], %[eh15] wave_shr:1 row_mask:0xf bank_mask:0xf bound_ctrl:1\n\t"
        "v_min3_i32 %[H0], %[M0], %[X15], %[Y0]\n\t"
        "v_add_u32 %[T], %[o], %[H0]\n\t"
        "v_min_i32 %[X15], %[X15], %[T]\n\t"
        "v_min_i32 %[Y0], %[Y0], %[T]\n\t"
        "v_min3_i32 %[H1], %[M1], %[X15], %[Y1]\n\t"
        "v_add_u32 %[T], %[o], %[H1]\n\t"
        "v_min_i32 %[X15], %[X15], %[T]\n\t"
        "v_min_i32 %[Y1], %[Y1], %[T]\n\t"
        "v_min3_i32 %[H2], %[M2], %[X15], %[Y2]\n\t"
        "v_add_u32 %[T], %[o], %[H2]\n\t"
        "v_min_i32 %[X15], %[X15], %[T]\n\t"
        "v_min_i32 %[Y2], %[Y2], %[T]\n\t"
        "v_min3_i32 %[H3], %[M3], %[X15], %[Y3]\n\t"
        "v_add_u32 %[T], %[o], %[H3]\n\t"
        "v_min_i32 %[X15], %[X15], %[T]\n\t"
        "v_min_i32 %[Y3], %[Y3], %[T]\n\t"
        "v_min3_i32 %[H4], %[M4], %[X15], %[Y4]\n\t"
        "v_add_u32 %[T], %[o], %[H4]\n\t"
        "v_min_i32 %[X15], %[X15], %[T]\n\t"
        "v_min_i32 %[Y4], %[Y4], %[T]\n\t"
        "v_min3_i32 %[H5], %[M5], %[X15], %[Y5]\n\t"
        "v_add_u32 %[T], %[o], %[H5]\n\t"
        "v_min_i32 %[X15], %[X15], %[T]\n\t"
        "v_min_i32 %[Y5], %[Y5], %[T]\n\t"
        "v_min3_i32 %[H6], %[M6], %[X15], %[Y6]\n\t"
        "v_add_u32 %[T], %[o], %[H6]\n\t"
        "v_min_i32 %[X15], %[X15], %[T]\n\t"
        "v_min_i32 %[Y6], %[Y6], %[T]\n\t"
        "v_min3_i32 %[hn15], %[M7], %[X15], %[Y7]\n\t"
        "v_add_u32 %[T], %[o], %[hn15]\n\t"
        "v_min_i32 %[X15], %[X15], %[T]\n\t"
        "v_min_i32 %[Y7], %[Y7], %[T]\n\t"
        "v_mov_b32_dpp %[Rhb], %[hn11] row_shl:4 row_mask:0x8 bank_mask:0x4\n\t"
        "v_mov_b32_dpp %[Rha], %[hn15] quad_perm:[0,1,2,3] row_mask:0x8 bank_mask:0x8\n\t"
        "v_mov_b32_dpp %[Rxb], %[X11] row_shl:4 row_mask:0x8 bank_mask:0x4\n\t"
        "v_mov_b32_dpp %[Rxa], %[X15] quad_perm:[0,1,2,3] row_mask:0x8 bank_mask:0x8\n\t"
        "v_mov_b32_dpp %[Rhb], %[hn10] row_shl:5 row_mask:0x8 bank_mask:0x4\n\t"
        "v_mov_b32_dpp %[Rha], %[hn14] row_shl:1 row_mask:0x8 bank_mask:0x8\n\t"
        "v_mov_b32_dpp %[Rxb], %[X10] row_shl:5 row_mask:0x8 bank_mask:0x4\n\t"
        "v_mov_b32_dpp %[Rxa], %[X14] row_shl:1 row_mask:0x8 bank_mask:0x8\n\t"
        "v_mov_b32_dpp %[Rhb], %[hn9] row_shl:6 row_mask:0x8 bank_mask:0x4\n\t"
        "v_mov_b32_dpp %[Rha], %[hn13] row_shl:2 row_mask:0x8 bank_mask:0x8\n\t"
        "v_mov_b32_dpp %[Rxb], %[X9] row_shl:6 row_mask:0x8 bank_mask:0x4\n\t"
        "v_mov_b32_dpp %[Rxa], %[X13] row_shl:2 row_mask:0x8 bank_mask:0x8\n\t"
        "v_mov_b32_dpp %[Rhb], %[hn8] row_shl:7 row_mask:0x8 bank_mask:0x4\n\t"
        "v_mov_b32_dpp %[Rha], %[hn12] row_shl:3 row_mask:0x8 bank_mask:0x8\n\t"
        "v_mov_b32_dpp %[Rxb], %[X8] row_shl:7 row_mask:0x8 bank_mask:0x4\n\t"
        "v_mov_b32_dpp %[Rxa], %[X12] row_shl:3 row_mask:0x8 bank_mask:0x8\n\t"
        "ds_write2_b32 %[wa], %[Rha], %[Rxa] offset1:1\n\t"
        "ds_write2_b32 %[wb], %[Rhb], %[Rxb] offset1:1\n\t"
        "ds_write_b64 %[wc], %[cp]\n\t"
        "s_waitcnt lgkmcnt(3)"
        : [X0] "=&v"(X[0]), [X1] "=&v"(X[1]), [X2] "=&v"(X[2]), [X3] "=&v"(X[3]), [X4] "=&v"(X[4]), [X5] "=&v"(X[5]), [X6] "=&v"(X[6]), [X7] "=&v"(X[7]), [X8] "=&v"(X[8]), [X9] "=&v"(X[9]), [X10] "=&v"(X[10]), [X11] "=&v"(X[11]), [X12] "=&v"(X[12]), [X13] "=&v"(X[13]), [X14] "=&v"(X[14]), [X15] "=&v"(X[15]), [hn0] "=&v"(hn[0]), [hn1] "=&v"(hn[1]), [hn2] "=&v"(hn[2]), [hn3] "=&v"(hn[3]), [hn4] "=&v"(hn[4]), [hn5] "=&v"(hn[5]), [hn6] "=&v"(hn[6]), [hn7] "=&v"(hn[7]), [hn8] "=&v"(hn[8]), [hn9] "=&v"(hn[9]), [hn10] "=&v"(hn[10]), [hn11] "=&v"(hn[11]), [hn12] "=&v"(hn[12]), [hn13] "=&v"(hn[13]), [hn14] "=&v"(hn[14]), [hn15] "=&v"(hn[15]), [HLn0] "=&v"(HLn[0]), [HLn1] "=&v"(HLn[1]), [H0] "+v"(H[0]), [H1] "+v"(H[1]), [H2] "+v"(H[2]), [H3] "+v"(H[3]), [H4] "+v"(H[4]), [H5] "+v"(H[5]), [H6] "+v"(H[6]), [Y0] "+v"(Y[0]), [Y1] "+v"(Y[1]), [Y2] "+v"(Y[2]), [Y3] "+v"(Y[3]), [Y4] "+v"(Y[4]), [Y5] "+v"(Y[5]), [Y6] "+v"(Y[6]), [Y7] "+v"(Y[7]), [T] "=&v"(T), [M0] "=&v"(M[0]), [M1] "=&v"(M[1]), [M2] "=&v"(M[2]), [M3] "=&v"(M[3]), [M4] "=&v"(M[4]), [M5] "=&v"(M[5]), [M6] "=&v"(M[6]), [M7] "=&v"(M[7]), [Rha] "=&v"(R[0]), [Rxa] "=&v"(R[1]), [Rhb] "=&v"(R[2]), [Rxb] "=&v"(R[3]), [cv] "=&v"(cv), [E0] "=&v"(En[0]), [E1] "=&v"(En[1]), [E2] "=&v"(En[2]), [E3] "=&v"(En[3]), [E4] "=&v"(En[4]), [E5] "=&v"(En[5]), [E6] "=&v"(En[6]), [E7] "=&v"(En[7]), [qa0] "=&v"(qn[0][0]), [qa1] "=&v"(qn[1][0]), [qa2] "=&v"(qn[2][0]), [qa3] "=&v"(qn[3][0]), [qa4] "=&v"(qn[4][0]), [qa5] "=&v"(qn[5][0]), [qa6] "=&v"(qn[6][0]), [qa7] "=&v"(qn[7][0]), [qc0] "=&v"(qn[0][1]), [qc1] "=&v"(qn[1][1]), [qc2] "=&v"(qn[2][1]), [qc3] "=&v"(qn[3][1]), [qc4] "=&v"(qn[4][1]), [qc5] "=&v"(qn[5][1]), [qc6] "=&v"(qn[6][1]), [qc7] "=&v"(qn[7][1])
        : [Xl] "v"(Xl), [HLp] "v"(HLp), [Hlast] "v"(H[7]), [o] "s"(o), [ex0] "v"(E[0][1]), [ex1] "v"(E[0][3]), [ex2] "v"(E[1][1]), [ex3] "v"(E[1][3]), [ex4] "v"(E[2][1]), [ex5] "v"(E[2][3]), [ex6] "v"(E[3][1]), [ex7] "v"(E[3][3]), [ex8] "v"(E[4][1]), [ex9] "v"(E[4][3]), [ex10] "v"(E[5][1]), [ex11] "v"(E[5][3]), [ex12] "v"(E[6][1]), [ex13] "v"(E[6][3]), [ex14] "v"(E[7][1]), [ex15] "v"(E[7][3]), [eh0] "v"(E[0][0]), [eh1] "v"(E[0][2]), [eh2] "v"(E[1][0]), [eh3] "v"(E[1][2]), [eh4] "v"(E[2][0]), [eh5] "v"(E[2][2]), [eh6] "v"(E[3][0]), [eh7] "v"(E[3][2]), [eh8] "v"(E[4][0]), [eh9] "v"(E[4][2]), [eh10] "v"(E[5][0]), [eh11] "v"(E[5][2]), [eh12] "v"(E[6][0]), [eh13] "v"(E[6][2]), [eh14] "v"(E[7][0]), [eh15] "v"(E[7][2]), [q0_0] "v"(q[0][0]), [q0_1] "v"(q[0][1]), [q0_2] "v"(q[0][2]), [q0_3] "v"(q[0][3]), [q1_0] "v"(q[1][0]), [q1_1] "v"(q[1][1]), [q1_2] "v"(q[1][2]), [q1_3] "v"(q[1][3]), [q2_0] "v"(q[2][0]), [q2_1] "v"(q[2][1]), [q2_2] "v"(q[2][2]), [q2_3] "v"(q[2][3]), [q3_0] "v"(q[3][0]), [q3_1] "v"(q[3][1]), [q3_2] "v"(q[3][2]), [q3_3] "v"(q[3][3]), [q4_0] "v"(q[4][0]), [q4_1] "v"(q[4][1]), [q4_2] "v"(q[4][2]), [q4_3] "v"(q[4][3]), [q5_0] "v"(q[5][0]), [q5_1] "v"(q[5][1]), [q5_2] "v"(q[5][2]), [q5_3] "v"(q[5][3]), [q6_0] "v"(q[6][0]), [q6_1] "v"(q[6][1]), [q6_2] "v"(q[6][2]), [q6_3] "v"(q[6][3]), [q7_0] "v"(q[7][0]), [q7_1] "v"(q[7][1]), [q7_2] "v"(q[7][2]), [q7_3] "v"(q[7][3]), [ca] "v"(ca), [ea] "v"(ea), [wa] "v"(wa), [wb] "v"(wb), [wc] "v"(wc), [cp] "v"(cp), [qb0] "v"(qb[0]), [qb1] "v"(qb[1]), [qb2] "v"(qb[2]), [qb3] "v"(qb[3]), [qb4] "v"(qb[4]), [qb5] "v"(qb[5]), [qb6] "v"(qb[6]), [qb7] "v"(qb[7])
        : "memory");
        H[7] = hn[15];
        Xl = X[15];
        HLp = HLn[1];
    }
};

template <>
struct LaneSub<8, 12> {
    __device__ __forceinline__ static void run(int (&H)[8], int (&Y)[8], int& Xl, int& HLp, const lk_v4i (&E)[8],
                                               const uint32_t (&q)[8][4], int o, unsigned ca, unsigned ea,
                                               const unsigned (&qb)[8], unsigned wa, unsigned wb, unsigned wc, lk_v2u cp,
                                               unsigned& cv, lk_v4i (&En)[8], lk_v2u (&qn)[8][2], int (&R)[4]) {
        int X[16], hn[16], HLn[2], T, M[8];
        asm volatile(
        "v_add_u32_sdwa %[M0], sext(%[q0_0]), %[HLp] dst_sel:DWORD dst_unused:UNUSED_PAD src0_sel:BYTE_0 src1_sel:DWORD\n\t"
        "v_add_u32_sdwa %[M1], sext(%[q1_0]), %[H0] dst_sel:DWORD dst_unused:UNUSED_PAD src0_sel:BYTE_0 src1_sel:DWORD\n\t"
        "v_add_u32_sdwa %[M2], sext(%[q2_0]), %[H1] dst_sel:DWORD dst_unused:UNUSED_PAD src0_sel:BYTE_0 src1_sel:DWORD\n\t"
        "v_add_u32_sdwa %[M3], sext(%[q3_0]), %[H2] dst_sel:DWORD dst_unused:UNUSED_PAD src0_sel:BYTE_0 src1_sel:DWORD\n\t"
        "v_add_u32_sdwa %[M4], sext(%[q4_0]), %[H3] dst_sel:DWORD dst_unused:UNUSED_PAD src0_sel:BYTE_0 src1_sel:DWORD\n\t"
        "v_add_u32_sdwa %[M5], sext(%[q5_0]), %[H4] dst_sel:DWORD dst_unused:UNUSED_PAD src0_sel:BYTE_0 src1_sel:DWORD\n\t"
        "v_add_u32_sdwa %[M6], sext(%[q6_0]), %[H5] dst_sel:DWORD dst_unused:UNUSED_PAD src0_sel:BYTE_0 src1_sel:DWORD\n\t"
        "v_add_u32_sdwa %[M7], sext(%[q7_0]), %[H6] dst_sel:DWORD dst_unused:UNUSED_PAD src0_sel:BYTE_0 src1_sel:DWORD\n\t"
        "v_add_u32_dpp %[X0], %[Xl], %[ex0] wave_shr:1 row_mask:0xf bank_mask:0xf bound_ctrl:1\n\t"
        "v_add_u32_dpp %[HLn0], %[Hlast], %[eh0] wave_shr:1 row_mask:0xf bank_mask:0xf bound_ctrl:1\n\t"
        "v_min3_i32 %[H0], %[M0], %[X0], %[Y0]\n\t"
        "v_add_u32 %[T], %[o], %[H0]\n\t"
        "v_min_i32 %[X0], %[X0], %[T]\n\t"
        "v_min_i32 %[Y0], %[Y0], %[T]\n\t"
        "v_min3_i32 %[H1], %[M1], %[X0], %[Y1]\n\t"
        "v_add_u32 %[T], %[o], %[H1]\n\t"
        "v_min_i32 %[X0], %[X0], %[T]\n\t"
        "v_min_i32 %[Y1], %[Y1], %[T]\n\t"
        "v_min3_i32 %[H2], %[M2], %[X0], %[Y2]\n\t"
        "v_add_u32 %[T], %[o], %[H2]\n\t"
        "v_min_i32 %[X0], %[X0], %[T]\n\t"
        "v_min_i32 %[Y2], %[Y2], %[T]\n\t"
        "v_min3_i32 %[H3], %[M3], %[X0], %[Y3]\n\t"
        "v_add_u32 %[T], %[o], %[H3]\n\t"
        "v_min_i32 %[X0], %[X0], %[T]\n\t"
        "v_min_i32 %[Y3], %[Y3], %[T]\n\t"
        "v_min3_i32 %[H4], %[M4], %[X0], %[Y4]\n\t"
        "v_add_u32 %[T], %[o], %[H4]\n\t"
        "v_min_i32 %[X0], %[X0], %[T]\n\t"
        "v_min_i32 %[Y4], %[Y4], %[T]\n\t"
        "v_min3_i32 %[H5], %[M5], %[X0], %[Y5]\n\t"
        "v_add_u32 %[T], %[o], %[H5]\n\t"
// ... 648 lines not shown
        "v_add_u32_dpp %[HLn1], %[hn14], %[eh15] wave_shr:1 row_mask:0xf bank_mask:0xf bound_ctrl:1\n\t"
        "v_min3_i32 %[H0], %[M0], %[X15], %[Y0]\n\t"
        "v_add_u32 %[T], %[o], %[H0]\n\t"
        "v_min_i32 %[X15], %[X15], %[T]\n\t"
        "v_min_i32 %[Y0], %[Y0], %[T]\n\t"
        "v_min3_i32 %[H1], %[M1], %[X15], %[Y1]\n\t"
        "v_add_u32 %[T], %[o], %[H1]\n\t"
        "v_min_i32 %[X15], %[X15], %[T]\n\t"
        "v_min_i32 %[Y1], %[Y1], %[T]\n\t"
        "v_min3_i32 %[H2], %[M2], %[X15], %[Y2]\n\t"
        "v_add_u32 %[T], %[o], %[H2]\n\t"
        "v_min_i32 %[X15], %[X15], %[T]\n\t"
        "v_min_i32 %[Y2], %[Y2], %[T]\n\t"
        "v_min3_i32 %[H3], %[M3], %[X15], %[Y3]\n\t"
        "v_add_u32 %[T], %[o], %[H3]\n\t"
        "v_min_i32 %[X15], %[X15], %[T]\n\t"
        "v_min_i32 %[Y3], %[Y3], %[T]\n\t"
        "v_min3_i32 %[H4], %[M4], %[X15], %[Y4]\n\t"
        "v_add_u32 %[T], %[o], %[H4]\n\t"
        "v_min_i32 %[X15], %[X15], %[T]\n\t"
        "v_min_i32 %[Y4], %[Y4], %[T]\n\t"
        "v_min3_i32 %[H5], %[M5], %[X15], %[Y5]\n\t"
        "v_add_u32 %[T], %[o], %[H5]\n\t"
        "v_min_i32 %[X15], %[X15], %[T]\n\t"
        "v_min_i32 %[Y5], %[Y5], %[T]\n\t"
        "v_min3_i32 %[H6], %[M6], %[X15], %[Y6]\n\t"
        "v_add_u32 %[T], %[o], %[H6]\n\t"
        "v_min_i32 %[X15], %[X15], %[T]\n\t"
        "v_min_i32 %[Y6], %[Y6], %[T]\n\t"
        "v_min3_i32 %[hn15], %[M7], %[X15], %[Y7]\n\t"
        "v_add_u32 %[T], %[o], %[hn15]\n\t"
        "v_min_i32 %[X15], %[X15], %[T]\n\t"
        "v_min_i32 %[Y7], %[Y7], %[T]\n\t"
        "v_mov_b32_dpp %[Rhb], %[hn11] row_shl:4 row_mask:0x8 bank_mask:0x4\n\t"
        "v_mov_b32_dpp %[Rha], %[hn15] quad_perm:[0,1,2,3] row_mask:0x8 bank_mask:0x8\n\t"
        "v_mov_b32_dpp %[Rxb], %[X11] row_shl:4 row_mask:0x8 bank_mask:0x4\n\t"
        "v_mov_b32_dpp %[Rxa], %[X15] quad_perm:[0,1,2,3] row_mask:0x8 bank_mask:0x8\n\t"
        "v_mov_b32_dpp %[Rhb], %[hn10] row_shl:5 row_mask:0x8 bank_mask:0x4\n\t"
        "v_mov_b32_dpp %[Rha], %[hn14] row_shl:1 row_mask:0x8 bank_mask:0x8\n\t"
        "v_mov_b32_dpp %[Rxb], %[X10] row_shl:5 row_mask:0x8 bank_mask:0x4\n\t"
        "v_mov_b32_dpp %[Rxa], %[X14] row_shl:1 row_mask:0x8 bank_mask:0x8\n\t"
        "v_mov_b32_dpp %[Rhb], %[hn9] row_shl:6 row_mask:0x8 bank_mask:0x4\n\t"
        "v_mov_b32_dpp %[Rha], %[hn13] row_shl:2 row_mask:0x8 bank_mask:0x8\n\t"
        "v_mov_b32_dpp %[Rxb], %[X9] row_shl:6 row_mask:0x8 bank_mask:0x4\n\t"
        "v_mov_b32_dpp %[Rxa], %[X13] row_shl:2 row_mask:0x8 bank_mask:0x8\n\t"
        "v_mov_b32_dpp %[Rhb], %[hn8] row_shl:7 row_mask:0x8 bank_mask:0x4\n\t"
        "v_mov_b32_dpp %[Rha], %[hn12] row_shl:3 row_mask:0x8 bank_mask:0x8\n\t"
        "v_mov_b32_dpp %[Rxb], %[X8] row_shl:7 row_mask:0x8 bank_mask:0x4\n\t"
        "v_mov_b32_dpp %[Rxa], %[X12] row_shl:3 row_mask:0x8 bank_mask:0x8\n\t"
        "ds_write2_b32 %[wa], %[Rha], %[Rxa] offset1:1\n\t"
        "ds_write2_b32 %[wb], %[Rhb], %[Rxb] offset1:1\n\t"
        "ds_write_b64 %[wc], %[cp]\n\t"
        "s_waitcnt lgkmcnt(3)"
        : [X0] "=&v"(X[0]), [X1] "=&v"(X[1]), [X2] "=&v"(X[2]), [X3] "=&v"(X[3]), [X4] "=&v"(X[4]), [X5] "=&v"(X[5]), [X6] "=&v"(X[6]), [X7] "=&v"(X[7]), [X8] "=&v"(X[8]), [X9] "=&v"(X[9]), [X10] "=&v"(X[10]), [X11] "=&v"(X[11]), [X12] "=&v"(X[12]), [X13] "=&v"(X[13]), [X14] "=&v"(X[14]), [X15] "=&v"(X[15]), [hn0] "=&v"(hn[0]), [hn1] "=&v"(hn[1]), [hn2] "=&v"(hn[2]), [hn3] "=&v"(hn[3]), [hn4] "=&v"(hn[4]), [hn5] "=&v"(hn[5]), [hn6] "=&v"(hn[6]), [hn7] "=&v"(hn[7]), [hn8] "=&v"(hn[8]), [hn9] "=&v"(hn[9]), [hn10] "=&v"(hn[10]), [hn11] "=&v"(hn[11]), [hn12] "=&v"(hn[12]), [hn13] "=&v"(hn[13]), [hn14] "=&v"(hn[14]), [hn15] "=&v"(hn[15]), [HLn0] "=&v"(HLn[0]), [HLn1] "=&v"(HLn[1]), [H0] "+v"(H[0]), [H1] "+v"(H[1]), [H2] "+v"(H[2]), [H3] "+v"(H[3]), [H4] "+v"(H[4]), [H5] "+v"(H[5]), [H6] "+v"(H[6]), [Y0] "+v"(Y[0]), [Y1] "+v"(Y[1]), [Y2] "+v"(Y[2]), [Y3] "+v"(Y[3]), [Y4] "+v"(Y[4]), [Y5] "+v"(Y[5]), [Y6] "+v"(Y[6]), [Y7] "+v"(Y[7]), [T] "=&v"(T), [M0] "=&v"(M[0]), [M1] "=&v"(M[1]), [M2] "=&v"(M[2]), [M3] "=&v"(M[3]), [M4] "=&v"(M[4]), [M5] "=&v"(M[5]), [M6] "=&v"(M[6]), [M7] "=&v"(M[7]), [Rha] "=&v"(R[0]), [Rxa] "=&v"(R[1]), [Rhb] "=&v"(R[2]), [Rxb] "=&v"(R[3]), [cv] "=&v"(cv), [E0] "=&v"(En[0]), [E1] "=&v"(En[1]), [E2] "=&v"(En[2]), [E3] "=&v"(En[3]), [E4] "=&v"(En[4]), [E5] "=&v"(En[5]), [E6] "=&v"(En[6]), [E7] "=&v"(En[7]), [qa0] "=&v"(qn[0][0]), [qa1] "=&v"(qn[1][0]), [qa2] "=&v"(qn[2][0]), [qa3] "=&v"(qn[3][0]), [qa4] "=&v"(qn[4][0]), [qa5] "=&v"(qn[5][0]), [qa6] "=&v"(qn[6][0]), [qa7] "=&v"(qn[7][0]), [qc0] "=&v"(qn[0][1]), [qc1] "=&v"(qn[1][1]), [qc2] "=&v"(qn[2][1]), [qc3] "=&v"(qn[3][1]), [qc4] "=&v"(qn[4][1]), [qc5] "=&v"(qn[5][1]), [qc6] "=&v"(qn[6][1]), [qc7] "=&v"(qn[7][1])
        : [Xl] "v"(Xl), [HLp] "v"(HLp), [Hlast] "v"(H[7]), [o] "s"(o), [ex0] "v"(E[0][1]), [ex1] "v"(E[0][3]), [ex2] "v"(E[1][1]), [ex3] "v"(E[1][3]), [ex4] "v"(E[2][1]), [ex5] "v"(E[2][3]), [ex6] "v"(E[3][1]), [ex7] "v"(E[3][3]), [ex8] "v"(E[4][1]), [ex9] "v"(E[4][3]), [ex10] "v"(E[5][1]), [ex11] "v"(E[5][3]), [ex12] "v"(E[6][1]), [ex13] "v"(E[6][3]), [ex14] "v"(E[7][1]), [ex15] "v"(E[7][3]), [eh0] "v"(E[0][0]), [eh1] "v"(E[0][2]), [eh2] "v"(E[1][0]), [eh3] "v"(E[1][2]), [eh4] "v"(E[2][0]), [eh5] "v"(E[2][2]), [eh6] "v"(E[3][0]), [eh7] "v"(E[3][2]), [eh8] "v"(E[4][0]), [eh9] "v"(E[4][2]), [eh10] "v"(E[5][0]), [eh11] "v"(E[5][2]), [eh12] "v"(E[6][0]), [eh13] "v"(E[6][2]), [eh14] "v"(E[7][0]), [eh15] "v"(E[7][2]), [q0_0] "v"(q[0][0]), [q0_1] "v"(q[0][1]), [q0_2] "v"(q[0][2]), [q0_3] "v"(q[0][3]), [q1_0] "v"(q[1][0]), [q1_1] "v"(q[1][1]), [q1_2] "v"(q[1][2]), [q1_3] "v"(q[1][3]), [q2_0] "v"(q[2][0]), [q2_1] "v"(q[2][1]), [q2_2] "v"(q[2][2]), [q2_3] "v"(q[2][3]), [q3_0] "v"(q[3][0]), [q3_1] "v"(q[3][1]), [q3_2] "v"(q[3][2]), [q3_3] "v"(q[3][3]), [q4_0] "v"(q[4][0]), [q4_1] "v"(q[4][1]), [q4_2] "v"(q[4][2]), [q4_3] "v"(q[4][3]), [q5_0] "v"(q[5][0]), [q5_1] "v"(q[5][1]), [q5_2] "v"(q[5][2]), [q5_3] "v"(q[5][3]), [q6_0] "v"(q[6][0]), [q6_1] "v"(q[6][1]), [q6_2] "v"(q[6][2]), [q6_3] "v"(q[6][3]), [q7_0] "v"(q[7][0]), [q7_1] "v"(q[7][1]), [q7_2] "v"(q[7][2]), [q7_3] "v"(q[7][3]), [ca] "v"(ca), [ea] "v"(ea), [wa] "v"(wa), [wb] "v"(wb), [wc] "v"(wc), [cp] "v"(cp), [qb0] "v"(qb[0]), [qb1] "v"(qb[1]), [qb2] "v"(qb[2]), [qb3] "v"(qb[3]), [qb4] "v"(qb[4]), [qb5] "v"(qb[5]), [qb6] "v"(qb[6]), [qb7] "v"(qb[7])
        : "memory");
        H[7] = hn[15];
        Xl = X[15];
        HLp = HLn[1];
    }
};

__device__ __forceinline__ void lk_store_rows(unsigned b1, unsigned b2, unsigned pc, lk_v2u cp, const int (&h)[16],
                                              const int (&x)[16]) {
    const unsigned long long m63 = 1ull << 63;
    unsigned long long saved;
    asm volatile(
        "s_mov_b64 %[saved], exec\n\t"
        "s_mov_b64 exec, %[m63]\n\t"
        "ds_write2_b32 %[b1], %[h0], %[x0] offset0:0 offset1:1\n\t"
        "ds_write2_b32 %[b1], %[h1], %[x1] offset0:2 offset1:3\n\t"
        "ds_write2_b32 %[b1], %[h2], %[x2] offset0:4 offset1:5\n\t"
        "ds_write2_b32 %[b1], %[h3], %[x3] offset0:6 offset1:7\n\t"
        "ds_write2_b32 %[b1], %[h4], %[x4] offset0:8 offset1:9\n\t"
        "ds_write2_b32 %[b1], %[h5], %[x5] offset0:10 offset1:11\n\t"
        "ds_write2_b32 %[b1], %[h6], %[x6] offset0:12 offset1:13\n\t"
        "ds_write2_b32 %[b1], %[h7], %[x7] offset0:14 offset1:15\n\t"
        "ds_write2_b32 %[b1], %[h8], %[x8] offset0:16 offset1:17\n\t"
        "ds_write2_b32 %[b1], %[h9], %[x9] offset0:18 offset1:19\n\t"
        "ds_write2_b32 %[b1], %[h10], %[x10] offset0:20 offset1:21\n\t"
        "ds_write2_b32 %[b1], %[h11], %[x11] offset0:22 offset1:23\n\t"
        "ds_write2_b32 %[b1], %[h12], %[x12] offset0:24 offset1:25\n\t"
        "ds_write2_b32 %[b1], %[h13], %[x13] offset0:26 offset1:27\n\t"
        "ds_write2_b32 %[b1], %[h14], %[x14] offset0:28 offset1:29\n\t"
        "ds_write2_b32 %[b2], %[h15], %[x15] offset1:1\n\t"
        "s_mov_b64 exec, 1\n\t"
        "ds_write_b64 %[pc], %[cp]\n\t"
// ... 9 lines not shown
```

Baseline: 776.3 billion cells/s.

## Default to narrow recompute geometry and read producer counter into SGPR inside asm

The narrow TD=2 recompute-fill geometry becomes the default unless GA_RC_NARROW=0, instead of needing opt-in. Inside each LaneSub asm block the producer counter is now moved to a scalar register with an explicit lgkmcnt wait and v_readfirstlane, so the C++ caller no longer issues a separate readfirstlane. The counter address is passed in a VGPR, and the wait branches are marked unlikely. The added lgkmcnt waits could stall on outstanding LDS ops, and the geometry default change alters the work split for all recompute fills.

```diff
diff --git a/globalign_amd/csrc/ga_host.cpp b/globalign_amd/csrc/ga_host.cpp
--- a/globalign_amd/csrc/ga_host.cpp
+++ b/globalign_amd/csrc/ga_host.cpp
@@ -389,7 +389,7 @@
         constexpr int kRcLds = 256 * 256 * 2;
         if (!c->lane_T_req) {
             const char* nw = c->knob("GA_RC_NARROW");
-            const bool td2 = nw && atoi(nw) && !c->slab && c->K <= 8 && (n + 127) / 128 <= 4 * (int64_t)c->num_cu;
+            const bool td2 = (!nw || atoi(nw)) && !c->slab && c->K <= 8 && (n + 127) / 128 <= 4 * (int64_t)c->num_cu;
             if (td2 && lane_geometry(c, n, &qrows, false, 2, 4)) {
             } else if (c->T > 4) {
                 if (!lane_geometry(c, n, &qrows, false, 4, 4)) return fail(GA_E_STATE, "recompute fill geometry");
diff --git a/globalign_amd/csrc/ga_lane.hip b/globalign_amd/csrc/ga_lane.hip
--- a/globalign_amd/csrc/ga_lane.hip
+++ b/globalign_amd/csrc/ga_lane.hip
@@ -405,6 +405,8 @@
     }
     const int4* const ezero = reinterpret_cast<const int4*>(smem + LK_ZERO_OFF);
     const unsigned ca_lds = lds_addr(prod_in);
+    unsigned ca_v;
+    asm volatile("v_mov_b32 %0, %1" : "=v"(ca_v) : "s"(ca_lds));
     const unsigned pq_lds = lds_addr(pq);
     const unsigned scr_lds = lds_addr(smem + LK_SCR_OFF);
     unsigned q4[TD], ea_m, ea_b, wa_m, wa_b, wb_m, wb_b;
@@ -445,7 +447,7 @@
             avail = sgpr_u(max(avail, pnext));
             if ((int)avail < r0 + 2 * SUB) wait_ge(prod_in, 0, avail, r0 + 2 * SUB, 0);
         }
-        if ((int)qavail < r0 + 2 * SUB) wait_ge(&cnt[LK_PRODQ], 0, qavail, r0 + 2 * SUB, 1);
+        if (__builtin_expect((int)qavail < r0 + 2 * SUB, 0)) wait_ge(&cnt[LK_PRODQ], 0, qavail, r0 + 2 * SUB, 1);
         int eh[SUB], ex[SUB];
 #pragma unroll
         for (int k = 0; k < NE; k++) {
@@ -532,7 +534,7 @@
                 if (LEAN || (use_asm && !masked && !hand_direct)) {
                     const int rlo = r0 - 62;
                     outfree = sgpr_u(outfree);
-                    if ((int)outfree < rlo + SUB - 1) wait_ge(cons_out, RING, outfree, rlo + SUB - 1, 2);
+                    if (__builtin_expect((int)outfree < rlo + SUB - 1, 0)) wait_ge(cons_out, RING, outfree, rlo + SUB - 1, 2);
                     lk_v4i Ev[NE];
 #pragma unroll
                     for (int k = 0; k < NE; k++) Ev[k] = lk_v4i{C[k].x, C[k].y, C[k].z, C[k].w};
@@ -553,11 +555,11 @@
                     lk_v4i En[NE];
                     lk_v2u qn[TD][2];
                     int R[4];
-                    LaneSub<TD, LE ? 12 : 0>::run(H, Y, Xl, HLp, Ev, qc, o, ca_lds, ea, qbv, wa, wb, wc, cp, cv, En, qn, R);
+                    LaneSub<TD, LE ? 12 : 0>::run(H, Y, Xl, HLp, Ev, qc, o, ca_v, ea, qbv, wa, wb, wc, cp, cv, En, qn, R);
                     Hl = H[TD - 1];
                     if (DBG && rlo <= m / 2 && m / 2 < rlo + SUB) t_pub = __builtin_amdgcn_s_memrealtime();
                     const int need = min(r0 + 2 * SUB, m);
-                    if ((int)sgpr_u(cv) < need) {
+                    if (__builtin_expect((int)cv < need, 0)) {
                         wait_ge(prod_in, 0, avail, need, 0);
                         asm volatile("" ::: "memory");
                         const int4* src = lane == 0 ? reinterpret_cast<const int4*>(rin + ((r0 + SUB) & RMASK)) : ezero;
diff --git a/globalign_amd/csrc/ga_lane_asm.h b/globalign_amd/csrc/ga_lane_asm.h
--- a/globalign_amd/csrc/ga_lane_asm.h
+++ b/globalign_amd/csrc/ga_lane_asm.h
@@ -2449,6 +2449,7 @@
                                                const unsigned (&qb)[1], unsigned wa, unsigned wb, unsigned wc, lk_v2u cp,
                                                unsigned& cv, lk_v4i (&En)[8], lk_v2u (&qn)[1][2], int (&R)[4]) {
         int X[16], hn[16], HLn[2], T, M[1];
+        unsigned cvt;
         asm volatile(
         "v_add_u32_sdwa %[M0], sext(%[q0_0]), %[HLp] dst_sel:DWORD dst_unused:UNUSED_PAD src0_sel:BYTE_0 src1_sel:DWORD\n\t"
         "s_nop 1\n\t"
@@ -2590,6 +2591,8 @@
         "v_add_u32 %[T], %[o], %[hn15]\n\t"
         "v_min_i32 %[X15], %[X15], %[T]\n\t"
         "v_min_i32 %[Y0], %[Y0], %[T]\n\t"
+        "s_waitcnt lgkmcnt(0)\n\t"
+        "v_readfirstlane_b32 %[cvs], %[cv]\n\t"
         "v_mov_b32_dpp %[Rhb], %[hn11] row_shl:4 row_mask:0x8 bank_mask:0x4\n\t"
         "v_mov_b32_dpp %[Rha], %[hn15] quad_perm:[0,1,2,3] row_mask:0x8 bank_mask:0x8\n\t"
         "v_mov_b32_dpp %[Rxb], %[X11] row_shl:4 row_mask:0x8 bank_mask:0x4\n\t"
@@ -2610,7 +2613,7 @@
         "ds_write2_b32 %[wb], %[Rhb], %[Rxb] offset1:1\n\t"
         "ds_write_b64 %[wc], %[cp]\n\t"
         "s_waitcnt lgkmcnt(3)"
-        : [X0] "=&v"(X[0]), [X1] "=&v"(X[1]), [X2] "=&v"(X[2]), [X3] "=&v"(X[3]), [X4] "=&v"(X[4]), [X5] "=&v"(X[5]), [X6] "=&v"(X[6]), [X7] "=&v"(X[7]), [X8] "=&v"(X[8]), [X9] "=&v"(X[9]), [X10] "=&v"(X[10]), [X11] "=&v"(X[11]), [X12] "=&v"(X[12]), [X13] "=&v"(X[13]), [X14] "=&v"(X[14]), [X15] "=&v"(X[15]), [hn0] "=&v"(hn[0]), [hn1] "=&v"(hn[1]), [hn2] "=&v"(hn[2]), [hn3] "=&v"(hn[3]), [hn4] "=&v"(hn[4]), [hn5] "=&v"(hn[5]), [hn6] "=&v"(hn[6]), [hn7] "=&v"(hn[7]), [hn8] "=&v"(hn[8]), [hn9] "=&v"(hn[9]), [hn10] "=&v"(hn[10]), [hn11] "=&v"(hn[11]), [hn12] "=&v"(hn[12]), [hn13] "=&v"(hn[13]), [hn14] "=&v"(hn[14]), [hn15] "=&v"(hn[15]), [HLn0] "=&v"(HLn[0]), [HLn1] "=&v"(HLn[1]), [Y0] "+v"(Y[0]), [T] "=&v"(T), [M0] "=&v"(M[0]), [Rha] "=&v"(R[0]), [Rxa] "=&v"(R[1]), [Rhb] "=&v"(R[2]), [Rxb] "=&v"(R[3]), [cv] "=&v"(cv), [E0] "=&v"(En[0]), [E1] "=&v"(En[1]), [E2] "=&v"(En[2]), [E3] "=&v"(En[3]), [E4] "=&v"(En[4]), [E5] "=&v"(En[5]), [E6] "=&v"(En[6]), [E7] "=&v"(En[7]), [qa0] "=&v"(qn[0][0]), [qc0] "=&v"(qn[0][1])
+        : [X0] "=&v"(X[0]), [X1] "=&v"(X[1]), [X2] "=&v"(X[2]), [X3] "=&v"(X[3]), [X4] "=&v"(X[4]), [X5] "=&v"(X[5]), [X6] "=&v"(X[6]), [X7] "=&v"(X[7]), [X8] "=&v"(X[8]), [X9] "=&v"(X[9]), [X10] "=&v"(X[10]), [X11] "=&v"(X[11]), [X12] "=&v"(X[12]), [X13] "=&v"(X[13]), [X14] "=&v"(X[14]), [X15] "=&v"(X[15]), [hn0] "=&v"(hn[0]), [hn1] "=&v"(hn[1]), [hn2] "=&v"(hn[2]), [hn3] "=&v"(hn[3]), [hn4] "=&v"(hn[4]), [hn5] "=&v"(hn[5]), [hn6] "=&v"(hn[6]), [hn7] "=&v"(hn[7]), [hn8] "=&v"(hn[8]), [hn9] "=&v"(hn[9]), [hn10] "=&v"(hn[10]), [hn11] "=&v"(hn[11]), [hn12] "=&v"(hn[12]), [hn13] "=&v"(hn[13]), [hn14] "=&v"(hn[14]), [hn15] "=&v"(hn[15]), [HLn0] "=&v"(HLn[0]), [HLn1] "=&v"(HLn[1]), [Y0] "+v"(Y[0]), [T] "=&v"(T), [M0] "=&v"(M[0]), [Rha] "=&v"(R[0]), [Rxa] "=&v"(R[1]), [Rhb] "=&v"(R[2]), [Rxb] "=&v"(R[3]), [cv] "=&v"(cvt), [cvs] "=&s"(cv), [E0] "=&v"(En[0]), [E1] "=&v"(En[1]), [E2] "=&v"(En[2]), [E3] "=&v"(En[3]), [E4] "=&v"(En[4]), [E5] "=&v"(En[5]), [E6] "=&v"(En[6]), [E7] "=&v"(En[7]), [qa0] "=&v"(qn[0][0]), [qc0] "=&v"(qn[0][1])
         : [Xl] "v"(Xl), [HLp] "v"(HLp), [Hlast] "v"(H[0]), [o] "s"(o), [ex0] "v"(E[0][1]), [ex1] "v"(E[0][3]), [ex2] "v"(E[1][1]), [ex3] "v"(E[1][3]), [ex4] "v"(E[2][1]), [ex5] "v"(E[2][3]), [ex6] "v"(E[3][1]), [ex7] "v"(E[3][3]), [ex8] "v"(E[4][1]), [ex9] "v"(E[4][3]), [ex10] "v"(E[5][1]), [ex11] "v"(E[5][3]), [ex12] "v"(E[6][1]), [ex13] "v"(E[6][3]), [ex14] "v"(E[7][1]), [ex15] "v"(E[7][3]), [eh0] "v"(E[0][0]), [eh1] "v"(E[0][2]), [eh2] "v"(E[1][0]), [eh3] "v"(E[1][2]), [eh4] "v"(E[2][0]), [eh5] "v"(E[2][2]), [eh6] "v"(E[3][0]), [eh7] "v"(E[3][2]), [eh8] "v"(E[4][0]), [eh9] "v"(E[4][2]), [eh10] "v"(E[5][0]), [eh11] "v"(E[5][2]), [eh12] "v"(E[6][0]), [eh13] "v"(E[6][2]), [eh14] "v"(E[7][0]), [eh15] "v"(E[7][2]), [q0_0] "v"(q[0][0]), [q0_1] "v"(q[0][1]), [q0_2] "v"(q[0][2]), [q0_3] "v"(q[0][3]), [ca] "v"(ca), [ea] "v"(ea), [wa] "v"(wa), [wb] "v"(wb), [wc] "v"(wc), [cp] "v"(cp), [qb0] "v"(qb[0])
         : "memory");
         H[0] = hn[15];
@@ -2626,6 +2629,7 @@
                                                const unsigned (&qb)[1], unsigned wa, unsigned wb, unsigned wc, lk_v2u cp,
                                                unsigned& cv, lk_v4i (&En)[8], lk_v2u (&qn)[1][2], int (&R)[4]) {
         int X[16], hn[16], HLn[2], T, M[1];
+        unsigned cvt;
         asm volatile(
         "v_add_u32_sdwa %[M0], sext(%[q0_0]), %[HLp] dst_sel:DWORD dst_unused:UNUSED_PAD src0_sel:BYTE_0 src1_sel:DWORD\n\t"
         "s_nop 1\n\t"
@@ -2767,6 +2771,8 @@
         "v_add_u32 %[T], %[o], %[hn15]\n\t"
         "v_min_i32 %[X15], %[X15], %[T]\n\t"
         "v_min_i32 %[Y0], %[Y0], %[T]\n\t"
+        "s_waitcnt lgkmcnt(8)\n\t"
+        "v_readfirstlane_b32 %[cvs], %[cv]\n\t"
         "v_mov_b32_dpp %[Rhb], %[hn11] row_shl:4 row_mask:0x8 bank_mask:0x4\n\t"
         "v_mov_b32_dpp %[Rha], %[hn15] quad_perm:[0,1,2,3] row_mask:0x8 bank_mask:0x8\n\t"
         "v_mov_b32_dpp %[Rxb], %[X11] row_shl:4 row_mask:0x8 bank_mask:0x4\n\t"
@@ -2787,7 +2793,7 @@
         "ds_write2_b32 %[wb], %[Rhb], %[Rxb] offset1:1\n\t"
         "ds_write_b64 %[wc], %[cp]\n\t"
         "s_waitcnt lgkmcnt(3)"
-        : [X0] "=&v"(X[0]), [X1] "=&v"(X[1]), [X2] "=&v"(X[2]), [X3] "=&v"(X[3]), [X4] "=&v"(X[4]), [X5] "=&v"(X[5]), [X6] "=&v"(X[6]), [X7] "=&v"(X[7]), [X8] "=&v"(X[8]), [X9] "=&v"(X[9]), [X10] "=&v"(X[10]), [X11] "=&v"(X[11]), [X12] "=&v"(X[12]), [X13] "=&v"(X[13]), [X14] "=&v"(X[14]), [X15] "=&v"(X[15]), [hn0] "=&v"(hn[0]), [hn1] "=&v"(hn[1]), [hn2] "=&v"(hn[2]), [hn3] "=&v"(hn[3]), [hn4] "=&v"(hn[4]), [hn5] "=&v"(hn[5]), [hn6] "=&v"(hn[6]), [hn7] "=&v"(hn[7]), [hn8] "=&v"(hn[8]), [hn9] "=&v"(hn[9]), [hn10] "=&v"(hn[10]), [hn11] "=&v"(hn[11]), [hn12] "=&v"(hn[12]), [hn13] "=&v"(hn[13]), [hn14] "=&v"(hn[14]), [hn15] "=&v"(hn[15]), [HLn0] "=&v"(HLn[0]), [HLn1] "=&v"(HLn[1]), [Y0] "+v"(Y[0]), [T] "=&v"(T), [M0] "=&v"(M[0]), [Rha] "=&v"(R[0]), [Rxa] "=&v"(R[1]), [Rhb] "=&v"(R[2]), [Rxb] "=&v"(R[3]), [cv] "=&v"(cv), [E0] "=&v"(En[0]), [E1] "=&v"(En[1]), [E2] "=&v"(En[2]), [E3] "=&v"(En[3]), [E4] "=&v"(En[4]), [E5] "=&v"(En[5]), [E6] "=&v"(En[6]), [E7] "=&v"(En[7]), [qa0] "=&v"(qn[0][0]), [qc0] "=&v"(qn[0][1])
+        : [X0] "=&v"(X[0]), [X1] "=&v"(X[1]), [X2] "=&v"(X[2]), [X3] "=&v"(X[3]), [X4] "=&v"(X[4]), [X5] "=&v"(X[5]), [X6] "=&v"(X[6]), [X7] "=&v"(X[7]), [X8] "=&v"(X[8]), [X9] "=&v"(X[9]), [X10] "=&v"(X[10]), [X11] "=&v"(X[11]), [X12] "=&v"(X[12]), [X13] "=&v"(X[13]), [X14] "=&v"(X[14]), [X15] "=&v"(X[15]), [hn0] "=&v"(hn[0]), [hn1] "=&v"(hn[1]), [hn2] "=&v"(hn[2]), [hn3] "=&v"(hn[3]), [hn4] "=&v"(hn[4]), [hn5] "=&v"(hn[5]), [hn6] "=&v"(hn[6]), [hn7] "=&v"(hn[7]), [hn8] "=&v"(hn[8]), [hn9] "=&v"(hn[9]), [hn10] "=&v"(hn[10]), [hn11] "=&v"(hn[11]), [hn12] "=&v"(hn[12]), [hn13] "=&v"(hn[13]), [hn14] "=&v"(hn[14]), [hn15] "=&v"(hn[15]), [HLn0] "=&v"(HLn[0]), [HLn1] "=&v"(HLn[1]), [Y0] "+v"(Y[0]), [T] "=&v"(T), [M0] "=&v"(M[0]), [Rha] "=&v"(R[0]), [Rxa] "=&v"(R[1]), [Rhb] "=&v"(R[2]), [Rxb] "=&v"(R[3]), [cv] "=&v"(cvt), [cvs] "=&s"(cv), [E0] "=&v"(En[0]), [E1] "=&v"(En[1]), [E2] "=&v"(En[2]), [E3] "=&v"(En[3]), [E4] "=&v"(En[4]), [E5] "=&v"(En[5]), [E6] "=&v"(En[6]), [E7] "=&v"(En[7]), [qa0] "=&v"(qn[0][0]), [qc0] "=&v"(qn[0][1])
         : [Xl] "v"(Xl), [HLp] "v"(HLp), [Hlast] "v"(H[0]), [o] "s"(o), [ex0] "v"(E[0][1]), [ex1] "v"(E[0][3]), [ex2] "v"(E[1][1]), [ex3] "v"(E[1][3]), [ex4] "v"(E[2][1]), [ex5] "v"(E[2][3]), [ex6] "v"(E[3][1]), [ex7] "v"(E[3][3]), [ex8] "v"(E[4][1]), [ex9] "v"(E[4][3]), [ex10] "v"(E[5][1]), [ex11] "v"(E[5][3]), [ex12] "v"(E[6][1]), [ex13] "v"(E[6][3]), [ex14] "v"(E[7][1]), [ex15] "v"(E[7][3]), [eh0] "v"(E[0][0]), [eh1] "v"(E[0][2]), [eh2] "v"(E[1][0]), [eh3] "v"(E[1][2]), [eh4] "v"(E[2][0]), [eh5] "v"(E[2][2]), [eh6] "v"(E[3][0]), [eh7] "v"(E[3][2]), [eh8] "v"(E[4][0]), [eh9] "v"(E[4][2]), [eh10] "v"(E[5][0]), [eh11] "v"(E[5][2]), [eh12] "v"(E[6][0]), [eh13] "v"(E[6][2]), [eh14] "v"(E[7][0]), [eh15] "v"(E[7][2]), [q0_0] "v"(q[0][0]), [q0_1] "v"(q[0][1]), [q0_2] "v"(q[0][2]), [q0_3] "v"(q[0][3]), [ca] "v"(ca), [ea] "v"(ea), [wa] "v"(wa), [wb] "v"(wb), [wc] "v"(wc), [cp] "v"(cp), [qb0] "v"(qb[0])
         : "memory");
         H[0] = hn[15];
@@ -2803,6 +2809,7 @@
                                                const unsigned (&qb)[2], unsigned wa, unsigned wb, unsigned wc, lk_v2u cp,
                                                unsigned& cv, lk_v4i (&En)[8], lk_v2u (&qn)[2][2], int (&R)[4]) {
         int X[16], hn[16], HLn[2], T, M[2];
+        unsigned cvt;
         asm volatile(
         "v_add_u32_sdwa %[M0], sext(%[q0_0]), %[HLp] dst_sel:DWORD dst_unused:UNUSED_PAD src0_sel:BYTE_0 src1_sel:DWORD\n\t"
         "v_add_u32_sdwa %[M1], sext(%[q1_0]), %[H0] dst_sel:DWORD dst_unused:UNUSED_PAD src0_sel:BYTE_0 src1_sel:DWORD\n\t"
@@ -3025,6 +3032,8 @@
         "v_add_u32 %[T], %[o], %[hn15]\n\t"
         "v_min_i32 %[X15], %[X15], %[T]\n\t"
         "v_min_i32 %[Y1], %[Y1], %[T]\n\t"
+        "s_waitcnt lgkmcnt(0)\n\t"
+        "v_readfirstlane_b32 %[cvs], %[cv]\n\t"
         "v_mov_b32_dpp %[Rhb], %[hn11] row_shl:4 row_mask:0x8 bank_mask:0x4\n\t"
         "v_mov_b32_dpp %[Rha], %[hn15] quad_perm:[0,1,2,3] row_mask:0x8 bank_mask:0x8\n\t"
         "v_mov_b32_dpp %[Rxb], %[X11] row_shl:4 row_mask:0x8 bank_mask:0x4\n\t"
@@ -3045,7 +3054,7 @@
         "ds_write2_b32 %[wb], %[Rhb], %[Rxb] offset1:1\n\t"
         "ds_write_b64 %[wc], %[cp]\n\t"
         "s_waitcnt lgkmcnt(3)"
-        : [X0] "=&v"(X[0]), [X1] "=&v"(X[1]), [X2] "=&v"(X[2]), [X3] "=&v"(X[3]), [X4] "=&v"(X[4]), [X5] "=&v"(X[5]), [X6] "=&v"(X[6]), [X7] "=&v"(X[7]), [X8] "=&v"(X[8]), [X9] "=&v"(X[9]), [X10] "=&v"(X[10]), [X11] "=&v"(X[11]), [X12] "=&v"(X[12]), [X13] "=&v"(X[13]), [X14] "=&v"(X[14]), [X15] "=&v"(X[15]), [hn0] "=&v"(hn[0]), [hn1] "=&v"(hn[1]), [hn2] "=&v"(hn[2]), [hn3] "=&v"(hn[3]), [hn4] "=&v"(hn[4]), [hn5] "=&v"(hn[5]), [hn6] "=&v"(hn[6]), [hn7] "=&v"(hn[7]), [hn8] "=&v"(hn[8]), [hn9] "=&v"(hn[9]), [hn10] "=&v"(hn[10]), [hn11] "=&v"(hn[11]), [hn12] "=&v"(hn[12]), [hn13] "=&v"(hn[13]), [hn14] "=&v"(hn[14]), [hn15] "=&v"(hn[15]), [HLn0] "=&v"(HLn[0]), [HLn1] "=&v"(HLn[1]), [H0] "+v"(H[0]), [Y0] "+v"(Y[0]), [Y1] "+v"(Y[1]), [T] "=&v"(T), [M0] "=&v"(M[0]), [M1] "=&v"(M[1]), [Rha] "=&v"(R[0]), [Rxa] "=&v"(R[1]), [Rhb] "=&v"(R[2]), [Rxb] "=&v"(R[3]), [cv] "=&v"(cv), [E0] "=&v"(En[0]), [E1] "=&v"(En[1]), [E2] "=&v"(En[2]), [E3] "=&v"(En[3]), [E4] "=&v"(En[4]), [E5] "=&v"(En[5]), [E6] "=&v"(En[6]), [E7] "=&v"(En[7]), [qa0] "=&v"(qn[0][0]), [qa1] "=&v"(qn[1][0]), [qc0] "=&v"(qn[0][1]), [qc1] "=&v"(qn[1][1])
+        : [X0] "=&v"(X[0]), [X1] "=&v"(X[1]), [X2] "=&v"(X[2]), [X3] "=&v"(X[3]), [X4] "=&v"(X[4]), [X5] "=&v"(X[5]), [X6] "=&v"(X[6]), [X7] "=&v"(X[7]), [X8] "=&v"(X[8]), [X9] "=&v"(X[9]), [X10] "=&v"(X[10]), [X11] "=&v"(X[11]), [X12] "=&v"(X[12]), [X13] "=&v"(X[13]), [X14] "=&v"(X[14]), [X15] "=&v"(X[15]), [hn0] "=&v"(hn[0]), [hn1] "=&v"(hn[1]), [hn2] "=&v"(hn[2]), [hn3] "=&v"(hn[3]), [hn4] "=&v"(hn[4]), [hn5] "=&v"(hn[5]), [hn6] "=&v"(hn[6]), [hn7] "=&v"(hn[7]), [hn8] "=&v"(hn[8]), [hn9] "=&v"(hn[9]), [hn10] "=&v"(hn[10]), [hn11] "=&v"(hn[11]), [hn12] "=&v"(hn[12]), [hn13] "=&v"(hn[13]), [hn14] "=&v"(hn[14]), [hn15] "=&v"(hn[15]), [HLn0] "=&v"(HLn[0]), [HLn1] "=&v"(HLn[1]), [H0] "+v"(H[0]), [Y0] "+v"(Y[0]), [Y1] "+v"(Y[1]), [T] "=&v"(T), [M0] "=&v"(M[0]), [M1] "=&v"(M[1]), [Rha] "=&v"(R[0]), [Rxa] "=&v"(R[1]), [Rhb] "=&v"(R[2]), [Rxb] "=&v"(R[3]), [cv] "=&v"(cvt), [cvs] "=&s"(cv), [E0] "=&v"(En[0]), [E1] "=&v"(En[1]), [E2] "=&v"(En[2]), [E3] "=&v"(En[3]), [E4] "=&v"(En[4]), [E5] "=&v"(En[5]), [E6] "=&v"(En[6]), [E7] "=&v"(En[7]), [qa0] "=&v"(qn[0][0]), [qa1] "=&v"(qn[1][0]), [qc0] "=&v"(qn[0][1]), [qc1] "=&v"(qn[1][1])
         : [Xl] "v"(Xl), [HLp] "v"(HLp), [Hlast] "v"(H[1]), [o] "s"(o), [ex0] "v"(E[0][1]), [ex1] "v"(E[0][3]), [ex2] "v"(E[1][1]), [ex3] "v"(E[1][3]), [ex4] "v"(E[2][1]), [ex5] "v"(E[2][3]), [ex6] "v"(E[3][1]), [ex7] "v"(E[3][3]), [ex8] "v"(E[4][1]), [ex9] "v"(E[4][3]), [ex10] "v"(E[5][1]), [ex11] "v"(E[5][3]), [ex12] "v"(E[6][1]), [ex13] "v"(E[6][3]), [ex14] "v"(E[7][1]), [ex15] "v"(E[7][3]), [eh0] "v"(E[0][0]), [eh1] "v"(E[0][2]), [eh2] "v"(E[1][0]), [eh3] "v"(E[1][2]), [eh4] "v"(E[2][0]), [eh5] "v"(E[2][2]), [eh6] "v"(E[3][0]), [eh7] "v"(E[3][2]), [eh8] "v"(E[4][0]), [eh9] "v"(E[4][2]), [eh10] "v"(E[5][0]), [eh11] "v"(E[5][2]), [eh12] "v"(E[6][0]), [eh13] "v"(E[6][2]), [eh14] "v"(E[7][0]), [eh15] "v"(E[7][2]), [q0_0] "v"(q[0][0]), [q0_1] "v"(q[0][1]), [q0_2] "v"(q[0][2]), [q0_3] "v"(q[0][3]), [q1_0] "v"(q[1][0]), [q1_1] "v"(q[1][1]), [q1_2] "v"(q[1][2]), [q1_3] "v"(q[1][3]), [ca] "v"(ca), [ea] "v"(ea), [wa] "v"(wa), [wb] "v"(wb), [wc] "v"(wc), [cp] "v"(cp), [qb0] "v"(qb[0]), [qb1] "v"(qb[1])
         : "memory");
         H[1] = hn[15];
@@ -3061,6 +3070,7 @@
                                                const unsigned (&qb)[2], unsigned wa, unsigned wb, unsigned wc, lk_v2u cp,
                                                unsigned& cv, lk_v4i (&En)[8], lk_v2u (&qn)[2][2], int (&R)[4]) {
         int X[16], hn[16], HLn[2], T, M[2];
+        unsigned cvt;
         asm volatile(
         "v_add_u32_sdwa %[M0], sext(%[q0_0]), %[HLp] dst_sel:DWORD dst_unused:UNUSED_PAD src0_sel:BYTE_0 src1_sel:DWORD\n\t"
         "v_add_u32_sdwa %[M1], sext(%[q1_0]), %[H0] dst_sel:DWORD dst_unused:UNUSED_PAD src0_sel:BYTE_0 src1_sel:DWORD\n\t"
@@ -3283,6 +3293,8 @@
         "v_add_u32 %[T], %[o], %[hn15]\n\t"
         "v_min_i32 %[X15], %[X15], %[T]\n\t"
         "v_min_i32 %[Y1], %[Y1], %[T]\n\t"
+        "s_waitcnt lgkmcnt(8)\n\t"
+        "v_readfirstlane_b32 %[cvs], %[cv]\n\t"
         "v_mov_b32_dpp %[Rhb], %[hn11] row_shl:4 row_mask:0x8 bank_mask:0x4\n\t"
         "v_mov_b32_dpp %[Rha], %[hn15] quad_perm:[0,1,2,3] row_mask:0x8 bank_mask:0x8\n\t"
         "v_mov_b32_dpp %[Rxb], %[X11] row_shl:4 row_mask:0x8 bank_mask:0x4\n\t"
@@ -3303,7 +3315,7 @@
         "ds_write2_b32 %[wb], %[Rhb], %[Rxb] offset1:1\n\t"
         "ds_write_b64 %[wc], %[cp]\n\t"
         "s_waitcnt lgkmcnt(3)"
-        : [X0] "=&v"(X[0]), [X1] "=&v"(X[1]), [X2] "=&v"(X[2]), [X3] "=&v"(X[3]), [X4] "=&v"(X[4]), [X5] "=&v"(X[5]), [X6] "=&v"(X[6]), [X7] "=&v"(X[7]), [X8] "=&v"(X[8]), [X9] "=&v"(X[9]), [X10] "=&v"(X[10]), [X11] "=&v"(X[11]), [X12] "=&v"(X[12]), [X13] "=&v"(X[13]), [X14] "=&v"(X[14]), [X15] "=&v"(X[15]), [hn0] "=&v"(hn[0]), [hn1] "=&v"(hn[1]), [hn2] "=&v"(hn[2]), [hn3] "=&v"(hn[3]), [hn4] "=&v"(hn[4]), [hn5] "=&v"(hn[5]), [hn6] "=&v"(hn[6]), [hn7] "=&v"(hn[7]), [hn8] "=&v"(hn[8]), [hn9] "=&v"(hn[9]), [hn10] "=&v"(hn[10]), [hn11] "=&v"(hn[11]), [hn12] "=&v"(hn[12]), [hn13] "=&v"(hn[13]), [hn14] "=&v"(hn[14]), [hn15] "=&v"(hn[15]), [HLn0] "=&v"(HLn[0]), [HLn1] "=&v"(HLn[1]), [H0] "+v"(H[0]), [Y0] "+v"(Y[0]), [Y1] "+v"(Y[1]), [T] "=&v"(T), [M0] "=&v"(M[0]), [M1] "=&v"(M[1]), [Rha] "=&v"(R[0]), [Rxa] "=&v"(R[1]), [Rhb] "=&v"(R[2]), [Rxb] "=&v"(R[3]), [cv] "=&v"(cv), [E0] "=&v"(En[0]), [E1] "=&v"(En[1]), [E2] "=&v"(En[2]), [E3] "=&v"(En[3]), [E4] "=&v"(En[4]), [E5] "=&v"(En[5]), [E6] "=&v"(En[6]), [E7] "=&v"(En[7]), [qa0] "=&v"(qn[0][0]), [qa1] "=&v"(qn[1][0]), [qc0] "=&v"(qn[0][1]), [qc1] "=&v"(qn[1][1])
+        : [X0] "=&v"(X[0]), [X1] "=&v"(X[1]), [X2] "=&v"(X[2]), [X3] "=&v"(X[3]), [X4] "=&v"(X[4]), [X5] "=&v"(X[5]), [X6] "=&v"(X[6]), [X7] "=&v"(X[7]), [X8] "=&v"(X[8]), [X9] "=&v"(X[9]), [X10] "=&v"(X[10]), [X11] "=&v"(X[11]), [X12] "=&v"(X[12]), [X13] "=&v"(X[13]), [X14] "=&v"(X[14]), [X15] "=&v"(X[15]), [hn0] "=&v"(hn[0]), [hn1] "=&v"(hn[1]), [hn2] "=&v"(hn[2]), [hn3] "=&v"(hn[3]), [hn4] "=&v"(hn[4]), [hn5] "=&v"(hn[5]), [hn6] "=&v"(hn[6]), [hn7] "=&v"(hn[7]), [hn8] "=&v"(hn[8]), [hn9] "=&v"(hn[9]), [hn10] "=&v"(hn[10]), [hn11] "=&v"(hn[11]), [hn12] "=&v"(hn[12]), [hn13] "=&v"(hn[13]), [hn14] "=&v"(hn[14]), [hn15] "=&v"(hn[15]), [HLn0] "=&v"(HLn[0]), [HLn1] "=&v"(HLn[1]), [H0] "+v"(H[0]), [Y0] "+v"(Y[0]), [Y1] "+v"(Y[1]), [T] "=&v"(T), [M0] "=&v"(M[0]), [M1] "=&v"(M[1]), [Rha] "=&v"(R[0]), [Rxa] "=&v"(R[1]), [Rhb] "=&v"(R[2]), [Rxb] "=&v"(R[3]), [cv] "=&v"(cvt), [cvs] "=&s"(cv), [E0] "=&v"(En[0]), [E1] "=&v"(En[1]), [E2] "=&v"(En[2]), [E3] "=&v"(En[3]), [E4] "=&v"(En[4]), [E5] "=&v"(En[5]), [E6] "=&v"(En[6]), [E7] "=&v"(En[7]), [qa0] "=&v"(qn[0][0]), [qa1] "=&v"(qn[1][0]), [qc0] "=&v"(qn[0][1]), [qc1] "=&v"(qn[1][1])
         : [Xl] "v"(Xl), [HLp] "v"(HLp), [Hlast] "v"(H[1]), [o] "s"(o), [ex0] "v"(E[0][1]), [ex1] "v"(E[0][3]), [ex2] "v"(E[1][1]), [ex3] "v"(E[1][3]), [ex4] "v"(E[2][1]), [ex5] "v"(E[2][3]), [ex6] "v"(E[3][1]), [ex7] "v"(E[3][3]), [ex8] "v"(E[4][1]), [ex9] "v"(E[4][3]), [ex10] "v"(E[5][1]), [ex11] "v"(E[5][3]), [ex12] "v"(E[6][1]), [ex13] "v"(E[6][3]), [ex14] "v"(E[7][1]), [ex15] "v"(E[7][3]), [eh0] "v"(E[0][0]), [eh1] "v"(E[0][2]), [eh2] "v"(E[1][0]), [eh3] "v"(E[1][2]), [eh4] "v"(E[2][0]), [eh5] "v"(E[2][2]), [eh6] "v"(E[3][0]), [eh7] "v"(E[3][2]), [eh8] "v"(E[4][0]), [eh9] "v"(E[4][2]), [eh10] "v"(E[5][0]), [eh11] "v"(E[5][2]), [eh12] "v"(E[6][0]), [eh13] "v"(E[6][2]), [eh14] "v"(E[7][0]), [eh15] "v"(E[7][2]), [q0_0] "v"(q[0][0]), [q0_1] "v"(q[0][1]), [q0_2] "v"(q[0][2]), [q0_3] "v"(q[0][3]), [q1_0] "v"(q[1][0]), [q1_1] "v"(q[1][1]), [q1_2] "v"(q[1][2]), [q1_3] "v"(q[1][3]), [ca] "v"(ca), [ea] "v"(ea), [wa] "v"(wa), [wb] "v"(wb), [wc] "v"(wc), [cp] "v"(cp), [qb0] "v"(qb[0]), [qb1] "v"(qb[1])
         : "memory");
         H[1] = hn[15];
@@ -3319,6 +3331,7 @@
                                                const unsigned (&qb)[4], unsigned wa, unsigned wb, unsigned wc, lk_v2u cp,
                                                unsigned& cv, lk_v4i (&En)[8], lk_v2u (&qn)[4][2], int (&R)[4]) {
         int X[16], hn[16], HLn[2], T, M[4];
+        unsigned cvt;
         asm volatile(
         "v_add_u32_sdwa %[M0], sext(%[q0_0]), %[HLp] dst_sel:DWORD dst_unused:UNUSED_PAD src0_sel:BYTE_0 src1_sel:DWORD\n\t"
         "v_add_u32_sdwa %[M1], sext(%[q1_0]), %[H0] dst_sel:DWORD dst_unused:UNUSED_PAD src0_sel:BYTE_0 src1_sel:DWORD\n\t"
@@ -3705,6 +3718,8 @@
         "v_add_u32 %[T], %[o], %[hn15]\n\t"
         "v_min_i32 %[X15], %[X15], %[T]\n\t"
         "v_min_i32 %[Y3], %[Y3], %[T]\n\t"
+        "s_waitcnt lgkmcnt(0)\n\t"
+        "v_readfirstlane_b32 %[cvs], %[cv]\n\t"
         "v_mov_b32_dpp %[Rhb], %[hn11] row_shl:4 row_mask:0x8 bank_mask:0x4\n\t"
         "v_mov_b32_dpp %[Rha], %[hn15] quad_perm:[0,1,2,3] row_mask:0x8 bank_mask:0x8\n\t"
         "v_mov_b32_dpp %[Rxb], %[X11] row_shl:4 row_mask:0x8 bank_mask:0x4\n\t"
@@ -3725,7 +3740,7 @@
         "ds_write2_b32 %[wb], %[Rhb], %[Rxb] offset1:1\n\t"
         "ds_write_b64 %[wc], %[cp]\n\t"
         "s_waitcnt lgkmcnt(3)"
-        : [X0] "=&v"(X[0]), [X1] "=&v"(X[1]), [X2] "=&v"(X[2]), [X3] "=&v"(X[3]), [X4] "=&v"(X[4]), [X5] "=&v"(X[5]), [X6] "=&v"(X[6]), [X7] "=&v"(X[7]), [X8] "=&v"(X[8]), [X9] "=&v"(X[9]), [X10] "=&v"(X[10]), [X11] "=&v"(X[11]), [X12] "=&v"(X[12]), [X13] "=&v"(X[13]), [X14] "=&v"(X[14]), [X15] "=&v"(X[15]), [hn0] "=&v"(hn[0]), [hn1] "=&v"(hn[1]), [hn2] "=&v"(hn[2]), [hn3] "=&v"(hn[3]), [hn4] "=&v"(hn[4]), [hn5] "=&v"(hn[5]), [hn6] "=&v"(hn[6]), [hn7] "=&v"(hn[7]), [hn8] "=&v"(hn[8]), [hn9] "=&v"(hn[9]), [hn10] "=&v"(hn[10]), [hn11] "=&v"(hn[11]), [hn12] "=&v"(hn[12]), [hn13] "=&v"(hn[13]), [hn14] "=&v"(hn[14]), [hn15] "=&v"(hn[15]), [HLn0] "=&v"(HLn[0]), [HLn1] "=&v"(HLn[1]), [H0] "+v"(H[0]), [H1] "+v"(H[1]), [H2] "+v"(H[2]), [Y0] "+v"(Y[0]), [Y1] "+v"(Y[1]), [Y2] "+v"(Y[2]), [Y3] "+v"(Y[3]), [T] "=&v"(T), [M0] "=&v"(M[0]), [M1] "=&v"(M[1]), [M2] "=&v"(M[2]), [M3] "=&v"(M[3]), [Rha] "=&v"(R[0]), [Rxa] "=&v"(R[1]), [Rhb] "=&v"(R[2]), [Rxb] "=&v"(R[3]), [cv] "=&v"(cv), [E0] "=&v"(En[0]), [E1] "=&v"(En[1]), [E2] "=&v"(En[2]), [E3] "=&v"(En[3]), [E4] "=&v"(En[4]), [E5] "=&v"(En[5]), [E6] "=&v"(En[6]), [E7] "=&v"(En[7]), [qa0] "=&v"(qn[0][0]), [qa1] "=&v"(qn[1][0]), [qa2] "=&v"(qn[2][0]), [qa3] "=&v"(qn[3][0]), [qc0] "=&v"(qn[0][1]), [qc1] "=&v"(qn[1][1]), [qc2] "=&v"(qn[2][1]), [qc3] "=&v"(qn[3][1])
+        : [X0] "=&v"(X[0]), [X1] "=&v"(X[1]), [X2] "=&v"(X[2]), [X3] "=&v"(X[3]), [X4] "=&v"(X[4]), [X5] "=&v"(X[5]), [X6] "=&v"(X[6]), [X7] "=&v"(X[7]), [X8] "=&v"(X[8]), [X9] "=&v"(X[9]), [X10] "=&v"(X[10]), [X11] "=&v"(X[11]), [X12] "=&v"(X[12]), [X13] "=&v"(X[13]), [X14] "=&v"(X[14]), [X15] "=&v"(X[15]), [hn0] "=&v"(hn[0]), [hn1] "=&v"(hn[1]), [hn2] "=&v"(hn[2]), [hn3] "=&v"(hn[3]), [hn4] "=&v"(hn[4]), [hn5] "=&v"(hn[5]), [hn6] "=&v"(hn[6]), [hn7] "=&v"(hn[7]), [hn8] "=&v"(hn[8]), [hn9] "=&v"(hn[9]), [hn10] "=&v"(hn[10]), [hn11] "=&v"(hn[11]), [hn12] "=&v"(hn[12]), [hn13] "=&v"(hn[13]), [hn14] "=&v"(hn[14]), [hn15] "=&v"(hn[15]), [HLn0] "=&v"(HLn[0]), [HLn1] "=&v"(HLn[1]), [H0] "+v"(H[0]), [H1] "+v"(H[1]), [H2] "+v"(H[2]), [Y0] "+v"(Y[0]), [Y1] "+v"(Y[1]), [Y2] "+v"(Y[2]), [Y3] "+v"(Y[3]), [T] "=&v"(T), [M0] "=&v"(M[0]), [M1] "=&v"(M[1]), [M2] "=&v"(M[2]), [M3] "=&v"(M[3]), [Rha] "=&v"(R[0]), [Rxa] "=&v"(R[1]), [Rhb] "=&v"(R[2]), [Rxb] "=&v"(R[3]), [cv] "=&v"(cvt), [cvs] "=&s"(cv), [E0] "=&v"(En[0]), [E1] "=&v"(En[1]), [E2] "=&v"(En[2]), [E3] "=&v"(En[3]), [E4] "=&v"(En[4]), [E5] "=&v"(En[5]), [E6] "=&v"(En[6]), [E7] "=&v"(En[7]), [qa0] "=&v"(qn[0][0]), [qa1] "=&v"(qn[1][0]), [qa2] "=&v"(qn[2][0]), [qa3] "=&v"(qn[3][0]), [qc0] "=&v"(qn[0][1]), [qc1] "=&v"(qn[1][1]), [qc2] "=&v"(qn[2][1]), [qc3] "=&v"(qn[3][1])
         : [Xl] "v"(Xl), [HLp] "v"(HLp), [Hlast] "v"(H[3]), [o] "s"(o), [ex0] "v"(E[0][1]), [ex1] "v"(E[0][3]), [ex2] "v"(E[1][1]), [ex3] "v"(E[1][3]), [ex4] "v"(E[2][1]), [ex5] "v"(E[2][3]), [ex6] "v"(E[3][1]), [ex7] "v"(E[3][3]), [ex8] "v"(E[4][1]), [ex9] "v"(E[4][3]), [ex10] "v"(E[5][1]), [ex11] "v"(E[5][3]), [ex12] "v"(E[6][1]), [ex13] "v"(E[6][3]), [ex14] "v"(E[7][1]), [ex15] "v"(E[7][3]), [eh0] "v"(E[0][0]), [eh1] "v"(E[0][2]), [eh2] "v"(E[1][0]), [eh3] "v"(E[1][2]), [eh4] "v"(E[2][0]), [eh5] "v"(E[2][2]), [eh6] "v"(E[3][0]), [eh7] "v"(E[3][2]), [eh8] "v"(E[4][0]), [eh9] "v"(E[4][2]), [eh10] "v"(E[5][0]), [eh11] "v"(E[5][2]), [eh12] "v"(E[6][0]), [eh13] "v"(E[6][2]), [eh14] "v"(E[7][0]), [eh15] "v"(E[7][2]), [q0_0] "v"(q[0][0]), [q0_1] "v"(q[0][1]), [q0_2] "v"(q[0][2]), [q0_3] "v"(q[0][3]), [q1_0] "v"(q[1][0]), [q1_1] "v"(q[1][1]), [q1_2] "v"(q[1][2]), [q1_3] "v"(q[1][3]), [q2_0] "v"(q[2][0]), [q2_1] "v"(q[2][1]), [q2_2] "v"(q[2][2]), [q2_3] "v"(q[2][3]), [q3_0] "v"(q[3][0]), [q3_1] "v"(q[3][1]), [q3_2] "v"(q[3][2]), [q3_3] "v"(q[3][3]), [ca] "v"(ca), [ea] "v"(ea), [wa] "v"(wa), [wb] "v"(wb), [wc] "v"(wc), [cp] "v"(cp), [qb0] "v"(qb[0]), [qb1] "v"(qb[1]), [qb2] "v"(qb[2]), [qb3] "v"(qb[3])
         : "memory");
         H[3] = hn[15];
@@ -3741,6 +3756,7 @@
                                                const unsigned (&qb)[4], unsigned wa, unsigned wb, unsigned wc, lk_v2u cp,
                                                unsigned& cv, lk_v4i (&En)[8], lk_v2u (&qn)[4][2], int (&R)[4]) {
         int X[16], hn[16], HLn[2], T, M[4];
+        unsigned cvt;
         asm volatile(
         "v_add_u32_sdwa %[M0], sext(%[q0_0]), %[HLp] dst_sel:DWORD dst_unused:UNUSED_PAD src0_sel:BYTE_0 src1_sel:DWORD\n\t"
         "v_add_u32_sdwa %[M1], sext(%[q1_0]), %[H0] dst_sel:DWORD dst_unused:UNUSED_PAD src0_sel:BYTE_0 src1_sel:DWORD\n\t"
@@ -4127,6 +4143,8 @@
         "v_add_u32 %[T], %[o], %[hn15]\n\t"
         "v_min_i32 %[X15], %[X15], %[T]\n\t"
         "v_min_i32 %[Y3], %[Y3], %[T]\n\t"
+        "s_waitcnt lgkmcnt(8)\n\t"
+        "v_readfirstlane_b32 %[cvs], %[cv]\n\t"
         "v_mov_b32_dpp %[Rhb], %[hn11] row_shl:4 row_mask:0x8 bank_mask:0x4\n\t"
         "v_mov_b32_dpp %[Rha], %[hn15] quad_perm:[0,1,2,3] row_mask:0x8 bank_mask:0x8\n\t"
         "v_mov_b32_dpp %[Rxb], %[X11] row_shl:4 row_mask:0x8 bank_mask:0x4\n\t"
@@ -4147,7 +4165,7 @@
         "ds_write2_b32 %[wb], %[Rhb], %[Rxb] offset1:1\n\t"
         "ds_write_b64 %[wc], %[cp]\n\t"
         "s_waitcnt lgkmcnt(3)"
-        : [X0] "=&v"(X[0]), [X1] "=&v"(X[1]), [X2] "=&v"(X[2]), [X3] "=&v"(X[3]), [X4] "=&v"(X[4]), [X5] "=&v"(X[5]), [X6] "=&v"(X[6]), [X7] "=&v"(X[7]), [X8] "=&v"(X[8]), [X9] "=&v"(X[9]), [X10] "=&v"(X[10]), [X11] "=&v"(X[11]), [X12] "=&v"(X[12]), [X13] "=&v"(X[13]), [X14] "=&v"(X[14]), [X15] "=&v"(X[15]), [hn0] "=&v"(hn[0]), [hn1] "=&v"(hn[1]), [hn2] "=&v"(hn[2]), [hn3] "=&v"(hn[3]), [hn4] "=&v"(hn[4]), [hn5] "=&v"(hn[5]), [hn6] "=&v"(hn[6]), [hn7] "=&v"(hn[7]), [hn8] "=&v"(hn[8]), [hn9] "=&v"(hn[9]), [hn10] "=&v"(hn[10]), [hn11] "=&v"(hn[11]), [hn12] "=&v"(hn[12]), [hn13] "=&v"(hn[13]), [hn14] "=&v"(hn[14]), [hn15] "=&v"(hn[15]), [HLn0] "=&v"(HLn[0]), [HLn1] "=&v"(HLn[1]), [H0] "+v"(H[0]), [H1] "+v"(H[1]), [H2] "+v"(H[2]), [Y0] "+v"(Y[0]), [Y1] "+v"(Y[1]), [Y2] "+v"(Y[2]), [Y3] "+v"(Y[3]), [T] "=&v"(T), [M0] "=&v"(M[0]), [M1] "=&v"(M[1]), [M2] "=&v"(M[2]), [M3] "=&v"(M[3]), [Rha] "=&v"(R[0]), [Rxa] "=&v"(R[1]), [Rhb] "=&v"(R[2]), [Rxb] "=&v"(R[3]), [cv] "=&v"(cv), [E0] "=&v"(En[0]), [E1] "=&v"(En[1]), [E2] "=&v"(En[2]), [E3] "=&v"(En[3]), [E4] "=&v"(En[4]), [E5] "=&v"(En[5]), [E6] "=&v"(En[6]), [E7] "=&v"(En[7]), [qa0] "=&v"(qn[0][0]), [qa1] "=&v"(qn[1][0]), [qa2] "=&v"(qn[2][0]), [qa3] "=&v"(qn[3][0]), [qc0] "=&v"(qn[0][1]), [qc1] "=&v"(qn[1][1]), [qc2] "=&v"(qn[2][1]), [qc3] "=&v"(qn[3][1])
+        : [X0] "=&v"(X[0]), [X1] "=&v"(X[1]), [X2] "=&v"(X[2]), [X3] "=&v"(X[3]), [X4] "=&v"(X[4]), [X5] "=&v"(X[5]), [X6] "=&v"(X[6]), [X7] "=&v"(X[7]), [X8] "=&v"(X[8]), [X9] "=&v"(X[9]), [X10] "=&v"(X[10]), [X11] "=&v"(X[11]), [X12] "=&v"(X[12]), [X13] "=&v"(X[13]), [X14] "=&v"(X[14]), [X15] "=&v"(X[15]), [hn0] "=&v"(hn[0]), [hn1] "=&v"(hn[1]), [hn2] "=&v"(hn[2]), [hn3] "=&v"(hn[3]), [hn4] "=&v"(hn[4]), [hn5] "=&v"(hn[5]), [hn6] "=&v"(hn[6]), [hn7] "=&v"(hn[7]), [hn8] "=&v"(hn[8]), [hn9] "=&v"(hn[9]), [hn10] "=&v"(hn[10]), [hn11] "=&v"(hn[11]), [hn12] "=&v"(hn[12]), [hn13] "=&v"(hn[13]), [hn14] "=&v"(hn[14]), [hn15] "=&v"(hn[15]), [HLn0] "=&v"(HLn[0]), [HLn1] "=&v"(HLn[1]), [H0] "+v"(H[0]), [H1] "+v"(H[1]), [H2] "+v"(H[2]), [Y0] "+v"(Y[0]), [Y1] "+v"(Y[1]), [Y2] "+v"(Y[2]), [Y3] "+v"(Y[3]), [T] "=&v"(T), [M0] "=&v"(M[0]), [M1] "=&v"(M[1]), [M2] "=&v"(M[2]), [M3] "=&v"(M[3]), [Rha] "=&v"(R[0]), [Rxa] "=&v"(R[1]), [Rhb] "=&v"(R[2]), [Rxb] "=&v"(R[3]), [cv] "=&v"(cvt), [cvs] "=&s"(cv), [E0] "=&v"(En[0]), [E1] "=&v"(En[1]), [E2] "=&v"(En[2]), [E3] "=&v"(En[3]), [E4] "=&v"(En[4]), [E5] "=&v"(En[5]), [E6] "=&v"(En[6]), [E7] "=&v"(En[7]), [qa0] "=&v"(qn[0][0]), [qa1] "=&v"(qn[1][0]), [qa2] "=&v"(qn[2][0]), [qa3] "=&v"(qn[3][0]), [qc0] "=&v"(qn[0][1]), [qc1] "=&v"(qn[1][1]), [qc2] "=&v"(qn[2][1]), [qc3] "=&v"(qn[3][1])
         : [Xl] "v"(Xl), [HLp] "v"(HLp), [Hlast] "v"(H[3]), [o] "s"(o), [ex0] "v"(E[0][1]), [ex1] "v"(E[0][3]), [ex2] "v"(E[1][1]), [ex3] "v"(E[1][3]), [ex4] "v"(E[2][1]), [ex5] "v"(E[2][3]), [ex6] "v"(E[3][1]), [ex7] "v"(E[3][3]), [ex8] "v"(E[4][1]), [ex9] "v"(E[4][3]), [ex10] "v"(E[5][1]), [ex11] "v"(E[5][3]), [ex12] "v"(E[6][1]), [ex13] "v"(E[6][3]), [ex14] "v"(E[7][1]), [ex15] "v"(E[7][3]), [eh0] "v"(E[0][0]), [eh1] "v"(E[0][2]), [eh2] "v"(E[1][0]), [eh3] "v"(E[1][2]), [eh4] "v"(E[2][0]), [eh5] "v"(E[2][2]), [eh6] "v"(E[3][0]), [eh7] "v"(E[3][2]), [eh8] "v"(E[4][0]), [eh9] "v"(E[4][2]), [eh10] "v"(E[5][0]), [eh11] "v"(E[5][2]), [eh12] "v"(E[6][0]), [eh13] "v"(E[6][2]), [eh14] "v"(E[7][0]), [eh15] "v"(E[7][2]), [q0_0] "v"(q[0][0]), [q0_1] "v"(q[0][1]), [q0_2] "v"(q[0][2]), [q0_3] "v"(q[0][3]), [q1_0] "v"(q[1][0]), [q1_1] "v"(q[1][1]), [q1_2] "v"(q[1][2]), [q1_3] "v"(q[1][3]), [q2_0] "v"(q[2][0]), [q2_1] "v"(q[2][1]), [q2_2] "v"(q[2][2]), [q2_3] "v"(q[2][3]), [q3_0] "v"(q[3][0]), [q3_1] "v"(q[3][1]), [q3_2] "v"(q[3][2]), [q3_3] "v"(q[3][3]), [ca] "v"(ca), [ea] "v"(ea), [wa] "v"(wa), [wb] "v"(wb), [wc] "v"(wc), [cp] "v"(cp), [qb0] "v"(qb[0]), [qb1] "v"(qb[1]), [qb2] "v"(qb[2]), [qb3] "v"(qb[3])
         : "memory");
         H[3] = hn[15];
@@ -4163,6 +4181,7 @@
                                                const unsigned (&qb)[8], unsigned wa, unsigned wb, unsigned wc, lk_v2u cp,
                                                unsigned& cv, lk_v4i (&En)[8], lk_v2u (&qn)[8][2], int (&R)[4]) {
         int X[16], hn[16], HLn[2], T, M[8];
+        unsigned cvt;
         asm volatile(
         "v_add_u32_sdwa %[M0], sext(%[q0_0]), %[HLp] dst_sel:DWORD dst_unused:UNUSED_PAD src0_sel:BYTE_0 src1_sel:DWORD\n\t"
         "v_add_u32_sdwa %[M1], sext(%[q1_0]), %[H0] dst_sel:DWORD dst_unused:UNUSED_PAD src0_sel:BYTE_0 src1_sel:DWORD\n\t"
@@ -4877,6 +4896,8 @@
         "v_add_u32 %[T], %[o], %[hn15]\n\t"
         "v_min_i32 %[X15], %[X15], %[T]\n\t"
         "v_min_i32 %[Y7], %[Y7], %[T]\n\t"
+        "s_waitcnt lgkmcnt(0)\n\t"
+        "v_readfirstlane_b32 %[cvs], %[cv]\n\t"
         "v_mov_b32_dpp %[Rhb], %[hn11] row_shl:4 row_mask:0x8 bank_mask:0x4\n\t"
         "v_mov_b32_dpp %[Rha], %[hn15] quad_perm:[0,1,2,3] row_mask:0x8 bank_mask:0x8\n\t"
         "v_mov_b32_dpp %[Rxb], %[X11] row_shl:4 row_mask:0x8 bank_mask:0x4\n\t"
@@ -4897,7 +4918,7 @@
         "ds_write2_b32 %[wb], %[Rhb], %[Rxb] offset1:1\n\t"
         "ds_write_b64 %[wc], %[cp]\n\t"
         "s_waitcnt lgkmcnt(3)"
-        : [X0] "=&v"(X[0]), [X1] "=&v"(X[1]), [X2] "=&v"(X[2]), [X3] "=&v"(X[3]), [X4] "=&v"(X[4]), [X5] "=&v"(X[5]), [X6] "=&v"(X[6]), [X7] "=&v"(X[7]), [X8] "=&v"(X[8]), [X9] "=&v"(X[9]), [X10] "=&v"(X[10]), [X11] "=&v"(X[11]), [X12] "=&v"(X[12]), [X13] "=&v"(X[13]), [X14] "=&v"(X[14]), [X15] "=&v"(X[15]), [hn0] "=&v"(hn[0]), [hn1] "=&v"(hn[1]), [hn2] "=&v"(hn[2]), [hn3] "=&v"(hn[3]), [hn4] "=&v"(hn[4]), [hn5] "=&v"(hn[5]), [hn6] "=&v"(hn[6]), [hn7] "=&v"(hn[7]), [hn8] "=&v"(hn[8]), [hn9] "=&v"(hn[9]), [hn10] "=&v"(hn[10]), [hn11] "=&v"(hn[11]), [hn12] "=&v"(hn[12]), [hn13] "=&v"(hn[13]), [hn14] "=&v"(hn[14]), [hn15] "=&v"(hn[15]), [HLn0] "=&v"(HLn[0]), [HLn1] "=&v"(HLn[1]), [H0] "+v"(H[0]), [H1] "+v"(H[1]), [H2] "+v"(H[2]), [H3] "+v"(H[3]), [H4] "+v"(H[4]), [H5] "+v"(H[5]), [H6] "+v"(H[6]), [Y0] "+v"(Y[0]), [Y1] "+v"(Y[1]), [Y2] "+v"(Y[2]), [Y3] "+v"(Y[3]), [Y4] "+v"(Y[4]), [Y5] "+v"(Y[5]), [Y6] "+v"(Y[6]), [Y7] "+v"(Y[7]), [T] "=&v"(T), [M0] "=&v"(M[0]), [M1] "=&v"(M[1]), [M2] "=&v"(M[2]), [M3] "=&v"(M[3]), [M4] "=&v"(M[4]), [M5] "=&v"(M[5]), [M6] "=&v"(M[6]), [M7] "=&v"(M[7]), [Rha] "=&v"(R[0]), [Rxa] "=&v"(R[1]), [Rhb] "=&v"(R[2]), [Rxb] "=&v"(R[3]), [cv] "=&v"(cv), [E0] "=&v"(En[0]), [E1] "=&v"(En[1]), [E2] "=&v"(En[2]), [E3] "=&v"(En[3]), [E4] "=&v"(En[4]), [E5] "=&v"(En[5]), [E6] "=&v"(En[6]), [E7] "=&v"(En[7]), [qa0] "=&v"(qn[0][0]), [qa1] "=&v"(qn[1][0]), [qa2] "=&v"(qn[2][0]), [qa3] "=&v"(qn[3][0]), [qa4] "=&v"(qn[4][0]), [qa5] "=&v"(qn[5][0]), [qa6] "=&v"(qn[6][0]), [qa7] "=&v"(qn[7][0]), [qc0] "=&v"(qn[0][1]), [qc1] "=&v"(qn[1][1]), [qc2] "=&v"(qn[2][1]), [qc3] "=&v"(qn[3][1]), [qc4] "=&v"(qn[4][1]), [qc5] "=&v"(qn[5][1]), [qc6] "=&v"(qn[6][1]), [qc7] "=&v"(qn[7][1])
+        : [X0] "=&v"(X[0]), [X1] "=&v"(X[1]), [X2] "=&v"(X[2]), [X3] "=&v"(X[3]), [X4] "=&v"(X[4]), [X5] "=&v"(X[5]), [X6] "=&v"(X[6]), [X7] "=&v"(X[7]), [X8] "=&v"(X[8]), [X9] "=&v"(X[9]), [X10] "=&v"(X[10]), [X11] "=&v"(X[11]), [X12] "=&v"(X[12]), [X13] "=&v"(X[13]), [X14] "=&v"(X[14]), [X15] "=&v"(X[15]), [hn0] "=&v"(hn[0]), [hn1] "=&v"(hn[1]), [hn2] "=&v"(hn[2]), [hn3] "=&v"(hn[3]), [hn4] "=&v"(hn[4]), [hn5] "=&v"(hn[5]), [hn6] "=&v"(hn[6]), [hn7] "=&v"(hn[7]), [hn8] "=&v"(hn[8]), [hn9] "=&v"(hn[9]), [hn10] "=&v"(hn[10]), [hn11] "=&v"(hn[11]), [hn12] "=&v"(hn[12]), [hn13] "=&v"(hn[13]), [hn14] "=&v"(hn[14]), [hn15] "=&v"(hn[15]), [HLn0] "=&v"(HLn[0]), [HLn1] "=&v"(HLn[1]), [H0] "+v"(H[0]), [H1] "+v"(H[1]), [H2] "+v"(H[2]), [H3] "+v"(H[3]), [H4] "+v"(H[4]), [H5] "+v"(H[5]), [H6] "+v"(H[6]), [Y0] "+v"(Y[0]), [Y1] "+v"(Y[1]), [Y2] "+v"(Y[2]), [Y3] "+v"(Y[3]), [Y4] "+v"(Y[4]), [Y5] "+v"(Y[5]), [Y6] "+v"(Y[6]), [Y7] "+v"(Y[7]), [T] "=&v"(T), [M0] "=&v"(M[0]), [M1] "=&v"(M[1]), [M2] "=&v"(M[2]), [M3] "=&v"(M[3]), [M4] "=&v"(M[4]), [M5] "=&v"(M[5]), [M6] "=&v"(M[6]), [M7] "=&v"(M[7]), [Rha] "=&v"(R[0]), [Rxa] "=&v"(R[1]), [Rhb] "=&v"(R[2]), [Rxb] "=&v"(R[3]), [cv] "=&v"(cvt), [cvs] "=&s"(cv), [E0] "=&v"(En[0]), [E1] "=&v"(En[1]), [E2] "=&v"(En[2]), [E3] "=&v"(En[3]), [E4] "=&v"(En[4]), [E5] "=&v"(En[5]), [E6] "=&v"(En[6]), [E7] "=&v"(En[7]), [qa0] "=&v"(qn[0][0]), [qa1] "=&v"(qn[1][0]), [qa2] "=&v"(qn[2][0]), [qa3] "=&v"(qn[3][0]), [qa4] "=&v"(qn[4][0]), [qa5] "=&v"(qn[5][0]), [qa6] "=&v"(qn[6][0]), [qa7] "=&v"(qn[7][0]), [qc0] "=&v"(qn[0][1]), [qc1] "=&v"(qn[1][1]), [qc2] "=&v"(qn[2][1]), [qc3] "=&v"(qn[3][1]), [qc4] "=&v"(qn[4][1]), [qc5] "=&v"(qn[5][1]), [qc6] "=&v"(qn[6][1]), [qc7] "=&v"(qn[7][1])
         : [Xl] "v"(Xl), [HLp] "v"(HLp), [Hlast] "v"(H[7]), [o] "s"(o), [ex0] "v"(E[0][1]), [ex1] "v"(E[0][3]), [ex2] "v"(E[1][1]), [ex3] "v"(E[1][3]), [ex4] "v"(E[2][1]), [ex5] "v"(E[2][3]), [ex6] "v"(E[3][1]), [ex7] "v"(E[3][3]), [ex8] "v"(E[4][1]), [ex9] "v"(E[4][3]), [ex10] "v"(E[5][1]), [ex11] "v"(E[5][3]), [ex12] "v"(E[6][1]), [ex13] "v"(E[6][3]), [ex14] "v"(E[7][1]), [ex15] "v"(E[7][3]), [eh0] "v"(E[0][0]), [eh1] "v"(E[0][2]), [eh2] "v"(E[1][0]), [eh3] "v"(E[1][2]), [eh4] "v"(E[2][0]), [eh5] "v"(E[2][2]), [eh6] "v"(E[3][0]), [eh7] "v"(E[3][2]), [eh8] "v"(E[4][0]), [eh9] "v"(E[4][2]), [eh10] "v"(E[5][0]), [eh11] "v"(E[5][2]), [eh12] "v"(E[6][0]), [eh13] "v"(E[6][2]), [eh14] "v"(E[7][0]), [eh15] "v"(E[7][2]), [q0_0] "v"(q[0][0]), [q0_1] "v"(q[0][1]), [q0_2] "v"(q[0][2]), [q0_3] "v"(q[0][3]), [q1_0] "v"(q[1][0]), [q1_1] "v"(q[1][1]), [q1_2] "v"(q[1][2]), [q1_3] "v"(q[1][3]), [q2_0] "v"(q[2][0]), [q2_1] "v"(q[2][1]), [q2_2] "v"(q[2][2]), [q2_3] "v"(q[2][3]), [q3_0] "v"(q[3][0]), [q3_1] "v"(q[3][1]), [q3_2] "v"(q[3][2]), [q3_3] "v"(q[3][3]), [q4_0] "v"(q[4][0]), [q4_1] "v"(q[4][1]), [q4_2] "v"(q[4][2]), [q4_3] "v"(q[4][3]), [q5_0] "v"(q[5][0]), [q5_1] "v"(q[5][1]), [q5_2] "v"(q[5][2]), [q5_3] "v"(q[5][3]), [q6_0] "v"(q[6][0]), [q6_1] "v"(q[6][1]), [q6_2] "v"(q[6][2]), [q6_3] "v"(q[6][3]), [q7_0] "v"(q[7][0]), [q7_1] "v"(q[7][1]), [q7_2] "v"(q[7][2]), [q7_3] "v"(q[7][3]), [ca] "v"(ca), [ea] "v"(ea), [wa] "v"(wa), [wb] "v"(wb), [wc] "v"(wc), [cp] "v"(cp), [qb0] "v"(qb[0]), [qb1] "v"(qb[1]), [qb2] "v"(qb[2]), [qb3] "v"(qb[3]), [qb4] "v"(qb[4]), [qb5] "v"(qb[5]), [qb6] "v"(qb[6]), [qb7] "v"(qb[7])
         : "memory");
         H[7] = hn[15];
@@ -4913,6 +4934,7 @@
                                                const unsigned (&qb)[8], unsigned wa, unsigned wb, unsigned wc, lk_v2u cp,
                                                unsigned& cv, lk_v4i (&En)[8], lk_v2u (&qn)[8][2], int (&R)[4]) {
         int X[16], hn[16], HLn[2], T, M[8];
+        unsigned cvt;
         asm volatile(
         "v_add_u32_sdwa %[M0], sext(%[q0_0]), %[HLp] dst_sel:DWORD dst_unused:UNUSED_PAD src0_sel:BYTE_0 src1_sel:DWORD\n\t"
         "v_add_u32_sdwa %[M1], sext(%[q1_0]), %[H0] dst_sel:DWORD dst_unused:UNUSED_PAD src0_sel:BYTE_0 src1_sel:DWORD\n\t"
@@ -5627,6 +5649,8 @@
         "v_add_u32 %[T], %[o], %[hn15]\n\t"
         "v_min_i32 %[X15], %[X15], %[T]\n\t"
         "v_min_i32 %[Y7], %[Y7], %[T]\n\t"
+        "s_waitcnt lgkmcnt(8)\n\t"
+        "v_readfirstlane_b32 %[cvs], %[cv]\n\t"
         "v_mov_b32_dpp %[Rhb], %[hn11] row_shl:4 row_mask:0x8 bank_mask:0x4\n\t"
         "v_mov_b32_dpp %[Rha], %[hn15] quad_perm:[0,1,2,3] row_mask:0x8 bank_mask:0x8\n\t"
         "v_mov_b32_dpp %[Rxb], %[X11] row_shl:4 row_mask:0x8 bank_mask:0x4\n\t"
@@ -5647,7 +5671,7 @@
         "ds_write2_b32 %[wb], %[Rhb], %[Rxb] offset1:1\n\t"
         "ds_write_b64 %[wc], %[cp]\n\t"
         "s_waitcnt lgkmcnt(3)"
-        : [X0] "=&v"(X[0]), [X1] "=&v"(X[1]), [X2] "=&v"(X[2]), [X3] "=&v"(X[3]), [X4] "=&v"(X[4]), [X5] "=&v"(X[5]), [X6] "=&v"(X[6]), [X7] "=&v"(X[7]), [X8] "=&v"(X[8]), [X9] "=&v"(X[9]), [X10] "=&v"(X[10]), [X11] "=&v"(X[11]), [X12] "=&v"(X[12]), [X13] "=&v"(X[13]), [X14] "=&v"(X[14]), [X15] "=&v"(X[15]), [hn0] "=&v"(hn[0]), [hn1] "=&v"(hn[1]), [hn2] "=&v"(hn[2]), [hn3] "=&v"(hn[3]), [hn4] "=&v"(hn[4]), [hn5] "=&v"(hn[5]), [hn6] "=&v"(hn[6]), [hn7] "=&v"(hn[7]), [hn8] "=&v"(hn[8]), [hn9] "=&v"(hn[9]), [hn10] "=&v"(hn[10]), [hn11] "=&v"(hn[11]), [hn12] "=&v"(hn[12]), [hn13] "=&v"(hn[13]), [hn14] "=&v"(hn[14]), [hn15] "=&v"(hn[15]), [HLn0] "=&v"(HLn[0]), [HLn1] "=&v"(HLn[1]), [H0] "+v"(H[0]), [H1] "+v"(H[1]), [H2] "+v"(H[2]), [H3] "+v"(H[3]), [H4] "+v"(H[4]), [H5] "+v"(H[5]), [H6] "+v"(H[6]), [Y0] "+v"(Y[0]), [Y1] "+v"(Y[1]), [Y2] "+v"(Y[2]), [Y3] "+v"(Y[3]), [Y4] "+v"(Y[4]), [Y5] "+v"(Y[5]), [Y6] "+v"(Y[6]), [Y7] "+v"(Y[7]), [T] "=&v"(T), [M0] "=&v"(M[0]), [M1] "=&v"(M[1]), [M2] "=&v"(M[2]), [M3] "=&v"(M[3]), [M4] "=&v"(M[4]), [M5] "=&v"(M[5]), [M6] "=&v"(M[6]), [M7] "=&v"(M[7]), [Rha] "=&v"(R[0]), [Rxa] "=&v"(R[1]), [Rhb] "=&v"(R[2]), [Rxb] "=&v"(R[3]), [cv] "=&v"(cv), [E0] "=&v"(En[0]), [E1] "=&v"(En[1]), [E2] "=&v"(En[2]), [E3] "=&v"(En[3]), [E4] "=&v"(En[4]), [E5] "=&v"(En[5]), [E6] "=&v"(En[6]), [E7] "=&v"(En[7]), [qa0] "=&v"(qn[0][0]), [qa1] "=&v"(qn[1][0]), [qa2] "=&v"(qn[2][0]), [qa3] "=&v"(qn[3][0]), [qa4] "=&v"(qn[4][0]), [qa5] "=&v"(qn[5][0]), [qa6] "=&v"(qn[6][0]), [qa7] "=&v"(qn[7][0]), [qc0] "=&v"(qn[0][1]), [qc1] "=&v"(qn[1][1]), [qc2] "=&v"(qn[2][1]), [qc3] "=&v"(qn[3][1]), [qc4] "=&v"(qn[4][1]), [qc5] "=&v"(qn[5][1]), [qc6] "=&v"(qn[6][1]), [qc7] "=&v"(qn[7][1])
+        : [X0] "=&v"(X[0]), [X1] "=&v"(X[1]), [X2] "=&v"(X[2]), [X3] "=&v"(X[3]), [X4] "=&v"(X[4]), [X5] "=&v"(X[5]), [X6] "=&v"(X[6]), [X7] "=&v"(X[7]), [X8] "=&v"(X[8]), [X9] "=&v"(X[9]), [X10] "=&v"(X[10]), [X11] "=&v"(X[11]), [X12] "=&v"(X[12]), [X13] "=&v"(X[13]), [X14] "=&v"(X[14]), [X15] "=&v"(X[15]), [hn0] "=&v"(hn[0]), [hn1] "=&v"(hn[1]), [hn2] "=&v"(hn[2]), [hn3] "=&v"(hn[3]), [hn4] "=&v"(hn[4]), [hn5] "=&v"(hn[5]), [hn6] "=&v"(hn[6]), [hn7] "=&v"(hn[7]), [hn8] "=&v"(hn[8]), [hn9] "=&v"(hn[9]), [hn10] "=&v"(hn[10]), [hn11] "=&v"(hn[11]), [hn12] "=&v"(hn[12]), [hn13] "=&v"(hn[13]), [hn14] "=&v"(hn[14]), [hn15] "=&v"(hn[15]), [HLn0] "=&v"(HLn[0]), [HLn1] "=&v"(HLn[1]), [H0] "+v"(H[0]), [H1] "+v"(H[1]), [H2] "+v"(H[2]), [H3] "+v"(H[3]), [H4] "+v"(H[4]), [H5] "+v"(H[5]), [H6] "+v"(H[6]), [Y0] "+v"(Y[0]), [Y1] "+v"(Y[1]), [Y2] "+v"(Y[2]), [Y3] "+v"(Y[3]), [Y4] "+v"(Y[4]), [Y5] "+v"(Y[5]), [Y6] "+v"(Y[6]), [Y7] "+v"(Y[7]), [T] "=&v"(T), [M0] "=&v"(M[0]), [M1] "=&v"(M[1]), [M2] "=&v"(M[2]), [M3] "=&v"(M[3]), [M4] "=&v"(M[4]), [M5] "=&v"(M[5]), [M6] "=&v"(M[6]), [M7] "=&v"(M[7]), [Rha] "=&v"(R[0]), [Rxa] "=&v"(R[1]), [Rhb] "=&v"(R[2]), [Rxb] "=&v"(R[3]), [cv] "=&v"(cvt), [cvs] "=&s"(cv), [E0] "=&v"(En[0]), [E1] "=&v"(En[1]), [E2] "=&v"(En[2]), [E3] "=&v"(En[3]), [E4] "=&v"(En[4]), [E5] "=&v"(En[5]), [E6] "=&v"(En[6]), [E7] "=&v"(En[7]), [qa0] "=&v"(qn[0][0]), [qa1] "=&v"(qn[1][0]), [qa2] "=&v"(qn[2][0]), [qa3] "=&v"(qn[3][0]), [qa4] "=&v"(qn[4][0]), [qa5] "=&v"(qn[5][0]), [qa6] "=&v"(qn[6][0]), [qa7] "=&v"(qn[7][0]), [qc0] "=&v"(qn[0][1]), [qc1] "=&v"(qn[1][1]), [qc2] "=&v"(qn[2][1]), [qc3] "=&v"(qn[3][1]), [qc4] "=&v"(qn[4][1]), [qc5] "=&v"(qn[5][1]), [qc6] "=&v"(qn[6][1]), [qc7] "=&v"(qn[7][1])
         : [Xl] "v"(Xl), [HLp] "v"(HLp), [Hlast] "v"(H[7]), [o] "s"(o), [ex0] "v"(E[0][1]), [ex1] "v"(E[0][3]), [ex2] "v"(E[1][1]), [ex3] "v"(E[1][3]), [ex4] "v"(E[2][1]), [ex5] "v"(E[2][3]), [ex6] "v"(E[3][1]), [ex7] "v"(E[3][3]), [ex8] "v"(E[4][1]), [ex9] "v"(E[4][3]), [ex10] "v"(E[5][1]), [ex11] "v"(E[5][3]), [ex12] "v"(E[6][1]), [ex13] "v"(E[6][3]), [ex14] "v"(E[7][1]), [ex15] "v"(E[7][3]), [eh0] "v"(E[0][0]), [eh1] "v"(E[0][2]), [eh2] "v"(E[1][0]), [eh3] "v"(E[1][2]), [eh4] "v"(E[2][0]), [eh5] "v"(E[2][2]), [eh6] "v"(E[3][0]), [eh7] "v"(E[3][2]), [eh8] "v"(E[4][0]), [eh9] "v"(E[4][2]), [eh10] "v"(E[5][0]), [eh11] "v"(E[5][2]), [eh12] "v"(E[6][0]), [eh13] "v"(E[6][2]), [eh14] "v"(E[7][0]), [eh15] "v"(E[7][2]), [q0_0] "v"(q[0][0]), [q0_1] "v"(q[0][1]), [q0_2] "v"(q[0][2]), [q0_3] "v"(q[0][3]), [q1_0] "v"(q[1][0]), [q1_1] "v"(q[1][1]), [q1_2] "v"(q[1][2]), [q1_3] "v"(q[1][3]), [q2_0] "v"(q[2][0]), [q2_1] "v"(q[2][1]), [q2_2] "v"(q[2][2]), [q2_3] "v"(q[2][3]), [q3_0] "v"(q[3][0]), [q3_1] "v"(q[3][1]), [q3_2] "v"(q[3][2]), [q3_3] "v"(q[3][3]), [q4_0] "v"(q[4][0]), [q4_1] "v"(q[4][1]), [q4_2] "v"(q[4][2]), [q4_3] "v"(q[4][3]), [q5_0] "v"(q[5][0]), [q5_1] "v"(q[5][1]), [q5_2] "v"(q[5][2]), [q5_3] "v"(q[5][3]), [q6_0] "v"(q[6][0]), [q6_1] "v"(q[6][1]), [q6_2] "v"(q[6][2]), [q6_3] "v"(q[6][3]), [q7_0] "v"(q[7][0]), [q7_1] "v"(q[7][1]), [q7_2] "v"(q[7][2]), [q7_3] "v"(q[7][3]), [ca] "v"(ca), [ea] "v"(ea), [wa] "v"(wa), [wb] "v"(wb), [wc] "v"(wc), [cp] "v"(cp), [qb0] "v"(qb[0]), [qb1] "v"(qb[1]), [qb2] "v"(qb[2]), [qb3] "v"(qb[3]), [qb4] "v"(qb[4]), [qb5] "v"(qb[5]), [qb6] "v"(qb[6]), [qb7] "v"(qb[7])
         : "memory");
         H[7] = hn[15];
```

Measured after the change: 832.0 billion cells/s (median of 6 runs). 1.07x the previous value.
